# tczhangzhi/pytorch-distributed

Hardware: AMD Instinct MI355X
Metric: ImageNet images/sec (ResNet-50 train step, whole job) (higher is better)
Workload: dtype bf16; 1 GPU; model=resnet50, global_batch=3072, image_size=224, parallelism=dp1, style=ddp, hip_ext=True, hipgraph=False

## Files before the change

### amdtrain/ops/conv.py

```python

from __future__ import annotations

import os

import torch
import torch.nn as nn

from ._ext import ext_available, require_ext


def _rows(x: torch.Tensor) -> torch.Tensor:
    n, c, h, w = x.shape
    return x.permute(0, 2, 3, 1).reshape(n * h * w, c)


def _fuse_stats_enabled() -> bool:
    return os.environ.get("AMDTRAIN_FUSE_BNSTATS", "1") == "1"


def _stem_s2d_enabled() -> bool:
    return os.environ.get("AMDTRAIN_STEM_S2D", "0") == "1"


def _stem_nt64_enabled() -> bool:
    return os.environ.get("AMDTRAIN_STEM_NT64", "1") == "1"


def _s2parity_enabled() -> bool:
    return os.environ.get("AMDTRAIN_CONV3X3_S2PARITY", "1") == "1"


def _nt64_enabled() -> bool:
    return os.environ.get("AMDTRAIN_CONV3X3_NT64", "1") == "1"


def _wgrad2_enabled() -> bool:
    return os.environ.get("AMDTRAIN_WGRAD2", "1") == "1"


class GradCell:
    __slots__ = ("armed", "g", "compact_ok", "meta")

    def __init__(self):
        self.armed = False
        self.g = None
        self.compact_ok = False
        self.meta = None


def _dsgrad_compact_enabled() -> bool:
    return os.environ.get("AMDTRAIN_DSGRAD_COMPACT", "1") == "1"


class ResidualGradTap(torch.autograd.Function):

    @staticmethod
    def forward(ctx, z: torch.Tensor, cell: "GradCell"):
        ctx.cell = cell
        ctx.set_materialize_grads(False)
        return z.view_as(z)

    @staticmethod
    def backward(ctx, grad):
        if grad is None:
            return None, None
        if ctx.cell.armed:
            ctx.cell.g = grad
            ctx.cell.meta = None
            return None, None
        return grad, None


def tap_residual(x: torch.Tensor, cell: "GradCell") -> torch.Tensor:
    out = ResidualGradTap.apply(x, cell)
    out._amdtrain_tap_cell = cell
    return out


class _Conv1x1(torch.autograd.Function):

    @staticmethod
    @torch.amp.custom_fwd(device_type="cuda", cast_inputs=torch.bfloat16)
    def forward(ctx, x: torch.Tensor, weight: torch.Tensor, stride: int,
                cell=None):
        e = require_ext()
        n, cin, h, w = x.shape
        cout = weight.shape[0]
        xc = x.contiguous(memory_format=torch.channels_last)
        x2d = _rows(xc)
        w2d = weight.reshape(cout, cin)
        stats = None
        ctx.cell = cell
        if stride > 1:
            y2d = e.gemm_bt_strided(x2d, w2d, n, h, w, stride)
            ho = (h + stride - 1) // stride
            wo = (w + stride - 1) // stride
        elif _fuse_stats_enabled():
            y2d, stats = e.gemm_bt_stats(x2d, w2d)
            ho, wo = h, w
        else:
            y2d = e.gemm_bt(x2d, w2d, False)
            ho, wo = h, w
        ctx.save_for_backward(x2d, w2d)
        ctx.meta = (n, cin, h, w, stride, ho, wo, cout)
        y = y2d.view(n, ho, wo, cout).permute(0, 3, 1, 2)
        if stats is None:
            stats = torch.empty(0, device=x.device)
        ctx.mark_non_differentiable(stats)
        return y, stats

    @staticmethod
    @torch.amp.custom_bwd(device_type="cuda")
    def backward(ctx, grad_y: torch.Tensor, _grad_stats=None):
        e = require_ext()
        x2d, w2d = ctx.saved_tensors
        n, cin, h, w, stride, ho, wo, cout = ctx.meta
        gy = grad_y.contiguous(memory_format=torch.channels_last)
        gy2d = _rows(gy).to(torch.bfloat16)
        wT = e.transpose_2d(w2d)
        dx2d = e.gemm_bt(gy2d, wT, False)
        if stride > 1:
            cell = ctx.cell
            if (stride == 2 and cell is not None and cell.armed
                    and cell.compact_ok):
                cell.g = dx2d
                cell.meta = (n, h, w, ho, wo)
                dx = None
            else:
                dx = e.scatter_rows_x2(dx2d, n, h, w, ho, wo)
            dw = e.tn2_wgrad(gy2d, x2d, 1, n, h, w, stride, 1) \
                if _wgrad2_enabled() \
                else e.gemm_tn_strided(gy2d, x2d, n, h, w, stride)
        else:
            dx = dx2d.view(n, ho, wo, cin).permute(0, 3, 1, 2)
            dw = e.tn2_wgrad(gy2d, x2d) if _wgrad2_enabled() \
                else e.gemm_tn(gy2d, x2d, 0)
        return dx, dw.reshape(cout, cin, 1, 1), None, None


def conv1x1_mfma(x: torch.Tensor, weight: torch.Tensor,
                 stride: int = 1) -> torch.Tensor:
    cell = getattr(x, "_amdtrain_tap_cell", None) if stride == 2 else None
    y, stats = _Conv1x1.apply(x, weight, stride, cell)
    if stats.numel():
        y._amdtrain_bn_stats = stats
    return y


class _Conv3x3(torch.autograd.Function):

    @staticmethod
    @torch.amp.custom_fwd(device_type="cuda", cast_inputs=torch.bfloat16)
    def forward(ctx, x: torch.Tensor, weight: torch.Tensor, stride: int):
        e = require_ext()
        n, cin, h, w = x.shape
        cout = weight.shape[0]
        xc = x.contiguous(memory_format=torch.channels_last)
        x2d = _rows(xc)
        w2d = weight.contiguous(memory_format=torch.channels_last) \
            .permute(0, 2, 3, 1).reshape(cout, 9 * cin)
        nt64 = _nt64_enabled()
        if _fuse_stats_enabled():
            y2d, stats = e.conv3x3_fwd_stats(x2d, n, h, w, stride, w2d,
                                             False, nt64)
        else:
            y2d = e.conv3x3_fwd(x2d, n, h, w, stride, w2d, nt64)
            stats = torch.empty(0, device=x.device)
        ctx.save_for_backward(x2d, w2d)
        ctx.meta = (n, cin, h, w, stride, cout)
        ho = (h + 2 - 3) // stride + 1
        wo = (w + 2 - 3) // stride + 1
        y = y2d.view(n, ho, wo, cout).permute(0, 3, 1, 2)
        ctx.mark_non_differentiable(stats)
        return y, stats

    @staticmethod
    @torch.amp.custom_bwd(device_type="cuda")
    def backward(ctx, grad_y: torch.Tensor, _grad_stats=None):
        e = require_ext()
        x2d, w2d = ctx.saved_tensors
        n, cin, h, w, stride, cout = ctx.meta
        gy = grad_y.contiguous(memory_format=torch.channels_last)
        gy2d = _rows(gy).to(torch.bfloat16)
        dx2d = e.conv3x3_dgrad(gy2d, n, h, w, stride, w2d, False,
                               _s2parity_enabled(), _nt64_enabled())
        dx = dx2d.view(n, h, w, cin).permute(0, 3, 1, 2)
        dw2d = e.tn2_wgrad(gy2d, x2d, 9, n, h, w, stride, 2) \
            if _wgrad2_enabled() \
            else e.conv3x3_wgrad(gy2d, x2d, n, h, w, stride)
        dw = dw2d.view(cout, 3, 3, cin).permute(0, 3, 1, 2) \
            .contiguous(memory_format=torch.channels_last)
        return dx, dw, None


def conv3x3_mfma(x: torch.Tensor, weight: torch.Tensor,
                 stride: int = 1) -> torch.Tensor:
    y, stats = _Conv3x3.apply(x, weight, stride)
    if stats.numel():
        y._amdtrain_bn_stats = stats
    return y


class _ConvGrouped3x3(torch.autograd.Function):

    @staticmethod
    @torch.amp.custom_fwd(device_type="cuda", cast_inputs=torch.bfloat16)
    def forward(ctx, x: torch.Tensor, weight: torch.Tensor, stride: int,
                groups: int):
        e = require_ext()
        n, cin, h, w = x.shape
        cout = weight.shape[0]
        sg = cin // groups
        xc = x.contiguous(memory_format=torch.channels_last)
        x2d = _rows(xc)
        sout = cout // groups
        wg = weight.contiguous(memory_format=torch.channels_last) \
            .permute(0, 2, 3, 1).reshape(groups, sout, 3, 3, sg)
        dense = torch.zeros(groups, sout, 3, 3, groups, sg,
                            dtype=wg.dtype, device=wg.device)
        gi = torch.arange(groups, device=wg.device)
        dense[gi, :, :, :, gi, :] = wg
        w2d = dense.reshape(cout, 3, 3, cin).reshape(cout, 9 * cin)
        banded = (cin == cout and cin % 128 == 0)
        if _fuse_stats_enabled():
            y2d, stats = e.conv3x3_fwd_stats(x2d, n, h, w, stride, w2d,
                                             banded, _nt64_enabled())
        else:
            y2d = e.conv3x3_fwd(x2d, n, h, w, stride, w2d, _nt64_enabled())
            stats = torch.empty(0, device=x.device)
        ctx.save_for_backward(x2d, w2d)
        ctx.meta = (n, cin, h, w, stride, cout, groups, banded)
        ho = (h + 2 - 3) // stride + 1
        wo = (w + 2 - 3) // stride + 1
        y = y2d.view(n, ho, wo, cout).permute(0, 3, 1, 2)
        ctx.mark_non_differentiable(stats)
        return y, stats

    @staticmethod
    @torch.amp.custom_bwd(device_type="cuda")
    def backward(ctx, grad_y: torch.Tensor, _grad_stats=None):
        e = require_ext()
        x2d, w2d = ctx.saved_tensors
        n, cin, h, w, stride, cout, groups, banded = ctx.meta
        sg = cin // groups
        sout = cout // groups
        gy = grad_y.contiguous(memory_format=torch.channels_last)
        gy2d = _rows(gy).to(torch.bfloat16)
        dx2d = e.conv3x3_dgrad(gy2d, n, h, w, stride, w2d, banded,
                               _s2parity_enabled(), _nt64_enabled())
        dx = dx2d.view(n, h, w, cin).permute(0, 3, 1, 2)
        if banded and _wgrad2_enabled():
            dwb = e.tn2_wgrad_banded(gy2d, x2d, n, h, w, stride) \
                .view(cout // 128, 128 // sg, sg, 9, 128 // sg, sg)
            bi = torch.arange(cout // 128, device=dwb.device)[:, None]
            gi = torch.arange(128 // sg, device=dwb.device)[None, :]
            dw = dwb[bi, gi, :, :, gi, :].reshape(cout, 9, sg) \
                .view(cout, 3, 3, sg).permute(0, 3, 1, 2) \
                .contiguous(memory_format=torch.channels_last)
            return dx, dw, None, None
        dw2d = e.tn2_wgrad(gy2d, x2d, 9, n, h, w, stride, 2) \
            if _wgrad2_enabled() \
            else e.conv3x3_wgrad(gy2d, x2d, n, h, w, stride)
        dwd = dw2d.view(groups, sout, 3, 3, groups, sg)
        gi = torch.arange(groups, device=dwd.device)
        dw = dwd[gi, :, :, :, gi, :].permute(0, 1, 4, 2, 3) \
            .reshape(cout, sg, 3, 3) \
            .contiguous(memory_format=torch.channels_last)
        return dx, dw, None, None


def conv3x3_grouped_mfma(x: torch.Tensor, weight: torch.Tensor,
                         stride: int, groups: int) -> torch.Tensor:
    y, stats = _ConvGrouped3x3.apply(x, weight, stride, groups)
    if stats.numel():
        y._amdtrain_bn_stats = stats
    return y


def stem_s2d_input(x_nhwc: torch.Tensor) -> torch.Tensor:
    n, h, w, c = x_nhwc.shape
    assert c <= 4 and w % 2 == 0
    x4 = torch.nn.functional.pad(x_nhwc, (0, 4 - c))
    return x4.reshape(n, h, w // 2, 8)


def stem_s2d_weight(weight: torch.Tensor) -> torch.Tensor:
    cout, c, kh, kw = weight.shape
    assert c <= 4 and kh == 7 and kw == 7
    wp = torch.nn.functional.pad(weight, (1, 0, 0, 0, 0, 4 - c))
    return wp.permute(0, 2, 3, 1).reshape(cout, 7, 4, 2, 4)


def stem_s2d_dweight(dw2: torch.Tensor, cin: int) -> torch.Tensor:
    cout = dw2.shape[0]
    return dw2.reshape(cout, 7, 8, 4)[:, :, 1:, :cin].permute(0, 3, 1, 2)


def _stem_s2d_ok(weight: torch.Tensor, w: int, stride: int, pad: int) -> bool:
    return (weight.shape[1] <= 4 and tuple(weight.shape[2:]) == (7, 7)
            and stride == 2 and pad == 3 and w % 2 == 0)


class _ConvGeneric(torch.autograd.Function):

    @staticmethod
    @torch.amp.custom_fwd(device_type="cuda", cast_inputs=torch.bfloat16)
    def forward(ctx, x: torch.Tensor, weight: torch.Tensor, stride: int,
                pad: int, s2d: bool = False, nt64: bool = False):
        e = require_ext()
        n, cin, h, w = x.shape
        cout, _, kh, kw = weight.shape
        xc = x.contiguous(memory_format=torch.channels_last)
        x2d = _rows(xc)
        ho = (h + 2 * pad - kh) // stride + 1
        wo = (w + 2 * pad - kw) // stride + 1
        ctx.s2d = s2d
        if s2d:
            x8 = stem_s2d_input(x2d.view(n, h, w, cin)) \
                .view(n * h * (w // 2), 8)
            w2 = stem_s2d_weight(weight).reshape(cout, 224)
            geom = (n, h, w // 2, 7, 4, 2, 3, w2, 1, 2, ho, wo, True)
            if _fuse_stats_enabled():
                y2d, stats = e.conv_generic_fwd_stats(x8, *geom)
            else:
                y2d = e.conv_generic_fwd(x8, *geom)
                stats = torch.empty(0, device=x.device)
            ctx.save_for_backward(x8, weight)
            ctx.meta = (n, cin, h, w, kh, kw, stride, pad, cout, 224, 8)
            ctx.mark_non_differentiable(stats)
            return y2d.view(n, ho, wo, cout).permute(0, 3, 1, 2), stats
        w4 = weight.contiguous(memory_format=torch.channels_last) \
            .permute(0, 2, 3, 1)
        if cin < 8:
            x2d = torch.nn.functional.pad(x2d, (0, 8 - cin))
            w4 = torch.nn.functional.pad(w4, (0, 8 - cin))
            cin_k = 8
        else:
            cin_k = cin
        k = kh * kw * cin_k
        kpad = (k + 31) // 32 * 32
        w2 = w4.reshape(cout, k)
        if kpad != k:
            w2 = torch.nn.functional.pad(w2, (0, kpad - k))
        y2d = e.conv_generic_fwd(x2d, n, h, w, kh, kw, stride, pad, w2,
                                 0, -1, 0, 0, nt64)
        ctx.save_for_backward(x2d, weight)
        ctx.meta = (n, cin, h, w, kh, kw, stride, pad, cout, k, cin_k)
        stats = torch.empty(0, device=x.device)
        ctx.mark_non_differentiable(stats)
        return y2d.view(n, ho, wo, cout).permute(0, 3, 1, 2), stats

    @staticmethod
    @torch.amp.custom_bwd(device_type="cuda")
    def backward(ctx, grad_y: torch.Tensor, _grad_stats=None):
        e = require_ext()
        x2d, weight = ctx.saved_tensors
        n, cin, h, w, kh, kw, stride, pad, cout, k, cin_k = ctx.meta
        gy2d = _rows(grad_y.contiguous(memory_format=torch.channels_last)) \
            .to(torch.bfloat16)
        dx = None
        if ctx.needs_input_grad[0]:
            k2 = kh * kw * cout
            k2p = (k2 + 31) // 32 * 32
            w2p = weight.to(torch.bfloat16).permute(1, 2, 3, 0) \
                .reshape(cin, k2)
            if k2p != k2:
                w2p = torch.nn.functional.pad(w2p, (0, k2p - k2))
            dx2d = e.conv_generic_dgrad(gy2d, w2p.contiguous(), n, h, w,
                                        kh, kw, stride, pad)
            dx = dx2d.view(n, h, w, cin).permute(0, 3, 1, 2)
        if ctx.s2d:
            ho = (h + 2 * pad - kh) // stride + 1
            wo = (w + 2 * pad - kw) // stride + 1
            dwp = e.tn2_wgrad(gy2d, x2d, 28, n, h, w // 2, 2, 2, 7, 4, 3,
                              1, 2, ho, wo)
            dw = stem_s2d_dweight(dwp, cin) \
                .contiguous(memory_format=torch.channels_last)
        elif _wgrad2_enabled() and cout % 8 == 0:
            dwp = e.tn2_wgrad(gy2d, x2d, kh * kw, n, h, w, stride, 2,
                              kh, kw, pad)
            dw = dwp.view(cout, kh * kw, cin_k)[:, :, :cin] \
                .view(cout, kh, kw, cin).permute(0, 3, 1, 2) \
                .contiguous(memory_format=torch.channels_last)
        else:
            dw2 = e.conv_generic_wgrad(gy2d, x2d, n, h, w, kh, kw, stride,
                                       pad)
            dw = dw2[:, :k].view(cout, kh * kw, cin_k)[:, :, :cin] \
                .reshape(cout, kh, kw, cin).permute(0, 3, 1, 2) \
                .contiguous(memory_format=torch.channels_last)
        return dx, dw, None, None, None, None


def conv_stem_mfma(x: torch.Tensor, weight: torch.Tensor, stride: int,
                   pad: int) -> torch.Tensor:
    s2d = (_stem_s2d_enabled() and _wgrad2_enabled()
           and _stem_s2d_ok(weight, x.shape[3], stride, pad))
    y, stats = _ConvGeneric.apply(x, weight, stride, pad, s2d,
                                  _stem_nt64_enabled())
    if stats.numel():
        y._amdtrain_bn_stats = stats
    return y


def _conv1x1_env_default() -> str:
    return os.environ.get("AMDTRAIN_CONV1X1", "custom")


class AmdConv2d(nn.Conv2d):

    def forward(self, x: torch.Tensor) -> torch.Tensor:
        bf16_ok = (x.dtype == torch.bfloat16
                   or torch.is_autocast_enabled("cuda"))
        if (x.is_cuda and bf16_ok and ext_available()
                and self.bias is None and self.dilation == (1, 1)
                and self.groups > 1):
            if (self.kernel_size == (3, 3) and self.padding == (1, 1)
                    and self.stride[0] in (1, 2)
                    and self.in_channels % 32 == 0
                    and self.out_channels % 16 == 0
                    and self.in_channels % self.groups == 0
                    and os.environ.get("AMDTRAIN_CONV3X3G", "custom")
                    == "custom"):
                return conv3x3_grouped_mfma(x, self.weight, self.stride[0],
                                            self.groups)
            return super().forward(x)
        if (x.is_cuda and bf16_ok and ext_available()
                and self.bias is None and self.groups == 1
                and self.dilation == (1, 1)):
            ch_ok = (self.in_channels % 32 == 0
                     and self.out_channels % 16 == 0)
            if (ch_ok and self.kernel_size == (1, 1)
                    and self.padding == (0, 0)
                    and _conv1x1_env_default() == "custom"):
                return conv1x1_mfma(x, self.weight, self.stride[0])
            if (ch_ok and self.kernel_size == (3, 3)
                    and self.padding == (1, 1)
                    and self.stride[0] in (1, 2)
                    and os.environ.get("AMDTRAIN_CONV3X3", "custom")
                    == "custom"):
                return conv3x3_mfma(x, self.weight, self.stride[0])
            if (self.out_channels % 16 == 0
                    and self.stride[0] == self.stride[1]
                    and self.padding[0] == self.padding[1]
                    and os.environ.get("AMDTRAIN_CONVSTEM", "custom")
                    == "custom"):
                return conv_stem_mfma(x, self.weight, self.stride[0],
                                      self.padding[0])
        return super().forward(x)
```

### amdtrain/ops/csrc/common.h

```cpp
#pragma once

#include <torch/extension.h>
#include <ATen/cuda/CUDAContext.h>
#include <hip/hip_runtime.h>
#include <hip/hip_bf16.h>
#include <hip/hip_fp16.h>

#define AMD_WAVE 64
#define AMD_TPB 256
#define AMD_MAX_BLOCKS 2048

#define CHECK_CUDA_OK()                                                     \
  do {                                                                      \
    hipError_t e = hipGetLastError();                                       \
    TORCH_CHECK(e == hipSuccess, "HIP kernel launch failed: ",              \
                hipGetErrorString(e));                                      \
  } while (0)

static inline int amd_grid(long total, int tpb = AMD_TPB,
                           int cap = AMD_MAX_BLOCKS) {
  long g = (total + tpb - 1) / tpb;
  return (int)std::min<long>(g, cap);
}


template <typename scalar_t> struct DevT { using type = scalar_t; };
template <> struct DevT<at::BFloat16> { using type = __hip_bfloat16; };
template <> struct DevT<at::Half> { using type = __half; };

template <typename T> __device__ __forceinline__ float to_f32(T v);
template <> __device__ __forceinline__ float to_f32<float>(float v) { return v; }
template <> __device__ __forceinline__ float to_f32<__hip_bfloat16>(__hip_bfloat16 v) {
  return __bfloat162float(v);
}
template <> __device__ __forceinline__ float to_f32<__half>(__half v) {
  return __half2float(v);
}
template <> __device__ __forceinline__ float to_f32<double>(double v) {
  return (float)v;
}

template <typename T> __device__ __forceinline__ T from_f32(float v);
template <> __device__ __forceinline__ float from_f32<float>(float v) { return v; }
template <> __device__ __forceinline__ __hip_bfloat16 from_f32<__hip_bfloat16>(float v) {
  return __float2bfloat16(v);
}
template <> __device__ __forceinline__ __half from_f32<__half>(float v) {
  return __float2half(v);
}
template <> __device__ __forceinline__ double from_f32<double>(float v) {
  return (double)v;
}

template <typename T, int N> struct alignas(sizeof(T) * N) Pack {
  T v[N];
};
template <typename T> struct VecWidth {
  static constexpr int value = 16 / sizeof(T);
};


__device__ __forceinline__ float wave_reduce_sum(float v) {
#pragma unroll
  for (int off = AMD_WAVE / 2; off > 0; off >>= 1)
    v += __shfl_down(v, off, AMD_WAVE);
  return v;
}

__device__ __forceinline__ float wave_reduce_max(float v) {
#pragma unroll
  for (int off = AMD_WAVE / 2; off > 0; off >>= 1)
    v = fmaxf(v, __shfl_down(v, off, AMD_WAVE));
  return v;
}

template <int NTE = 128>
__device__ __forceinline__ void conv_epilogue_stats(
    float* __restrict__ stats, const float* acc_flat, long m0, long M,
    long n0, long N, int bm, int wm, int wn, int fr, int fq,
    void* lds_scratch) {
  constexpr int NF = NTE / 32;
  float* srow = stats + (long)bm * 2 * N;
  float s1[NF], s2[NF];
#pragma unroll
  for (int j = 0; j < NF; ++j) {
    s1[j] = 0.f;
    s2[j] = 0.f;
#pragma unroll
    for (int i = 0; i < 4; ++i)
#pragma unroll
      for (int r = 0; r < 4; ++r) {
        long row = m0 + wm + i * 16 + fq * 4 + r;
        float v = (row < M) ? acc_flat[(i * NF + j) * 4 + r] : 0.f;
        s1[j] += v;
        s2[j] += v * v;
      }
  }
#pragma unroll
  for (int j = 0; j < NF; ++j) {
#pragma unroll
    for (int off = 32; off >= 16; off >>= 1) {
      s1[j] += __shfl_down(s1[j], off, AMD_WAVE);
      s2[j] += __shfl_down(s2[j], off, AMD_WAVE);
    }
  }
  float* red = (float*)lds_scratch;
  __syncthreads();
  if (fq == 0) {
#pragma unroll
    for (int j = 0; j < NF; ++j) {
      int col = wn + j * 16 + fr;
      red[(wm ? 1 : 0) * (2 * NTE) + col * 2 + 0] = s1[j];
      red[(wm ? 1 : 0) * (2 * NTE) + col * 2 + 1] = s2[j];
    }
  }
  __syncthreads();
  const int t = threadIdx.x;
  for (int col = t; col < NTE; col += AMD_TPB) {
    long n = n0 + col;
    if (n < N) {
      srow[n] = red[col * 2] + red[2 * NTE + col * 2];
      srow[N + n] = red[col * 2 + 1] + red[2 * NTE + col * 2 + 1];
    }
  }
}


constexpr int MT_TENSORS = 24;
constexpr int MT_BLOCKS = 320;
constexpr long MT_CHUNK = 1 << 16;

struct MTMeta {
  const void* a[MT_TENSORS];
  void* b[MT_TENSORS];
  void* c[MT_TENSORS];
  long sizes[MT_TENSORS];
  short t_for_block[MT_BLOCKS];
  short chunk_for_block[MT_BLOCKS];
};

template <typename LaunchFn>
static void mt_apply(const std::vector<at::Tensor>& A,
                     const std::vector<at::Tensor>* B,
                     const std::vector<at::Tensor>* C, LaunchFn launch) {
  MTMeta meta;
  int t = 0, blk = 0;
  for (size_t i = 0; i < A.size(); ++i) {
    long n = A[i].numel();
    meta.a[t] = A[i].const_data_ptr();
    meta.b[t] = B ? (*B)[i].data_ptr() : nullptr;
    meta.c[t] = C ? (*C)[i].data_ptr() : nullptr;
    meta.sizes[t] = n;
    long nchunks = (n + MT_CHUNK - 1) / MT_CHUNK;
    for (long ch = 0; ch < nchunks; ++ch) {
      meta.t_for_block[blk] = (short)t;
      meta.chunk_for_block[blk] = (short)ch;
      ++blk;
      if (blk == MT_BLOCKS) {
        launch(meta, blk, t + 1);
        meta.a[0] = meta.a[t];
        meta.b[0] = meta.b[t];
        meta.c[0] = meta.c[t];
        meta.sizes[0] = meta.sizes[t];
        t = 0;
        blk = 0;
      }
    }
    ++t;
    if (t == MT_TENSORS && i + 1 < A.size()) {
      if (blk) launch(meta, blk, t);
      t = 0;
      blk = 0;
    }
  }
  if (blk) launch(meta, blk, t);
}
```

### amdtrain/ops/csrc/conv3x3.hip

```cpp
#include "common.h"

namespace {

using bf16 = __hip_bfloat16;
using bf16x8 = __attribute__((ext_vector_type(8))) short;
using f32x4 = __attribute__((ext_vector_type(4))) float;

constexpr int GEMM_TPB = 256;
constexpr int BK = 32;

__device__ __forceinline__ int xcd_swz(int bid, int nwg) {
  constexpr int NXCD = 8;
  if (nwg < NXCD) return bid;
  int xcd = bid % NXCD, idx = bid / NXCD;
  int q = nwg / NXCD, r = nwg % NXCD;
  return (xcd < r ? xcd * (q + 1) : r * (q + 1) + (xcd - r) * q) + idx;
}

struct ConvGeom {
  int H, W, Hout, Wout, stride;
};

__device__ __forceinline__ long fwd_gather(long m, int kh, int kw,
                                           const ConvGeom& g) {
  long t = m;
  const int wo = (int)(t % g.Wout); t /= g.Wout;
  const int ho = (int)(t % g.Hout); t /= g.Hout;
  const int h = ho * g.stride - 1 + kh;
  const int w = wo * g.stride - 1 + kw;
  if (h < 0 || h >= g.H || w < 0 || w >= g.W) return -1;
  return (t * g.H + h) * g.W + w;
}

__device__ __forceinline__ long dgrad_gather(long m, int kh, int kw,
                                             const ConvGeom& g) {
  long t = m;
  const int w = (int)(t % g.W); t /= g.W;
  const int h = (int)(t % g.H); t /= g.H;
  const int ho2 = h + 1 - kh, wo2 = w + 1 - kw;
  if (g.stride == 1) {
    if (ho2 < 0 || ho2 >= g.Hout || wo2 < 0 || wo2 >= g.Wout) return -1;
    return (t * g.Hout + ho2) * g.Wout + wo2;
  }
  if ((ho2 & 1) || (wo2 & 1)) return -1;
  const int ho = ho2 >> 1, wo = wo2 >> 1;
  if (ho < 0 || ho >= g.Hout || wo < 0 || wo >= g.Wout) return -1;
  return (t * g.Hout + ho) * g.Wout + wo;
}

struct UnitCoord {
  long n_off;
  int hb, wb;
};

template <bool DGRAD, bool PAR = false>
__device__ __forceinline__ UnitCoord decode_unit(long m, const ConvGeom& g,
                                                 int cls = 0) {
  UnitCoord u;
  long t = m;
  if (PAR) {
    const int W2 = g.W >> 1, H2 = g.H >> 1;
    const int w2 = (int)(t % W2); t /= W2;
    const int h2 = (int)(t % H2); t /= H2;
    u.n_off = t * (long)g.Hout * g.Wout;
    u.hb = 2 * h2 + (cls >> 1) + 1;
    u.wb = 2 * w2 + (cls & 1) + 1;
  } else if (DGRAD) {
    const int w = (int)(t % g.W); t /= g.W;
    const int h = (int)(t % g.H); t /= g.H;
    u.n_off = t * (long)g.Hout * g.Wout;
    u.hb = h + 1;
    u.wb = w + 1;
  } else {
    const int wo = (int)(t % g.Wout); t /= g.Wout;
    const int ho = (int)(t % g.Hout); t /= g.Hout;
    u.n_off = t * (long)g.H * g.W;
    u.hb = ho * g.stride - 1;
    u.wb = wo * g.stride - 1;
  }
  return u;
}

template <bool DGRAD, bool PAR = false>
__device__ __forceinline__ long unit_row(const UnitCoord& u, int kh, int kw,
                                         const ConvGeom& g) {
  if (DGRAD) {
    int ho2 = u.hb - kh, wo2 = u.wb - kw;
    if (PAR) {
      ho2 >>= 1;
      wo2 >>= 1;
    } else if (g.stride == 2) {
      if ((ho2 | wo2) & 1) return -1;
      ho2 >>= 1;
      wo2 >>= 1;
    }
    if (ho2 < 0 || ho2 >= g.Hout || wo2 < 0 || wo2 >= g.Wout) return -1;
    return u.n_off + (long)ho2 * g.Wout + wo2;
  }
  const int h = u.hb + kh, w = u.wb + kw;
  if (h < 0 || h >= g.H || w < 0 || w >= g.W) return -1;
  return u.n_off + (long)h * g.W + w;
}

template <bool DGRAD, int BKT, bool PAR = false>
__device__ __forceinline__ void stage_gathered(
    const bf16* __restrict__ src, int ld, const UnitCoord* uc, int c0, int kh,
    int kw, const ConvGeom& g, const bf16* __restrict__ zero_page,
    bf16* lds) {
  const int t = threadIdx.x;
  constexpr int UPR = BKT / 8;
#pragma unroll
  for (int rnd = 0; rnd < BKT / 16; ++rnd) {
    int unit = rnd * GEMM_TPB + t;
    long row = unit_row<DGRAD, PAR>(uc[rnd], kh, kw, g);
    const bf16* p = row < 0 ? zero_page
                            : src + row * (long)ld + c0 +
                                  (unit % UPR) * 8;
    __builtin_amdgcn_global_load_lds(
        (const __attribute__((address_space(1))) unsigned int*)p,
        (__attribute__((address_space(3))) unsigned int*)(lds + unit * 8), 16,
        0, 0);
  }
}

template <int BKT, int ROWS>
__device__ __forceinline__ void stage_plain_rows(
    const bf16* __restrict__ gsrc, long ld, long row0, long rows, long koff,
    bf16* lds) {
  const int t = threadIdx.x;
  constexpr int UPR = BKT / 8;
  constexpr int UNITS = ROWS * UPR;
#pragma unroll
  for (int rnd = 0; rnd < UNITS / GEMM_TPB; ++rnd) {
    int unit = rnd * GEMM_TPB + t;
    long row = row0 + unit / UPR;
    if (row >= rows) row = rows - 1;
    const bf16* src = gsrc + row * ld + koff + (unit % UPR) * 8;
    __builtin_amdgcn_global_load_lds(
        (const __attribute__((address_space(1))) unsigned int*)src,
        (__attribute__((address_space(3))) unsigned int*)(lds + unit * 8), 16,
        0, 0);
  }
}

template <int BKT>
__device__ __forceinline__ void stage_plain(
    const bf16* __restrict__ gsrc, long ld, long row0, long rows, long koff,
    bf16* lds) {
  const int t = threadIdx.x;
  constexpr int UPR = BKT / 8;
#pragma unroll
  for (int rnd = 0; rnd < BKT / 16; ++rnd) {
    int unit = rnd * GEMM_TPB + t;
    long row = row0 + unit / UPR;
    if (row >= rows) row = rows - 1;
    const bf16* src = gsrc + row * ld + koff + (unit % UPR) * 8;
    __builtin_amdgcn_global_load_lds(
        (const __attribute__((address_space(1))) unsigned int*)src,
        (__attribute__((address_space(3))) unsigned int*)(lds + unit * 8), 16,
        0, 0);
  }
}

template <bool DGRAD, int BKT = BK, bool BAND = false, int NT = 128,
          bool DB = false, bool PAR = false>
__global__ void __launch_bounds__(GEMM_TPB, 2)
conv3x3_kernel(const bf16* __restrict__ A, const bf16* __restrict__ Bw,
               bf16* __restrict__ C, long M, int AC, int NC, ConvGeom g,
               int nbm, int nbn, const bf16* __restrict__ zero_page,
               float* __restrict__ stats) {
  static_assert(!PAR || (DGRAD && !BAND), "PAR is a dense-dgrad variant");
  constexpr int STG = (128 + NT) * BKT;
  __shared__ bf16 SMEM[(DB ? 2 : 1) * STG];
  bf16* const As = SMEM;

  const int bid = xcd_swz(blockIdx.x, nbm * nbn);
  const int bm = bid / nbn, bn = bid % nbn;
  const int cls = PAR ? (bm & 3) : 0;
  const long Mr = PAR ? (M >> 2) : M;
  const long m0 = (long)(PAR ? (bm >> 2) : bm) * 128, n0 = (long)bn * NT;
  constexpr int NFR = NT / 32;

  const int t = threadIdx.x;
  const int wave = t / AMD_WAVE, lane = t % AMD_WAVE;
  const int wm = (wave >> 1) * 64, wn = (wave & 1) * (NT / 2);
  const int fr = lane & 15, fq = lane >> 4;

  f32x4 acc[4][NFR];
#pragma unroll
  for (int i = 0; i < 4; ++i)
#pragma unroll
    for (int j = 0; j < NFR; ++j) acc[i][j] = {0.f, 0.f, 0.f, 0.f};

  UnitCoord uc[BKT / 16];
#pragma unroll
  for (int rnd = 0; rnd < BKT / 16; ++rnd) {
    long m = m0 + (rnd * GEMM_TPB + t) / (BKT / 8);
    if (m >= Mr) m = Mr - 1;
    uc[rnd] = decode_unit<DGRAD, PAR>(m, g, cls);
  }

  const int ks_lo = BAND ? (int)(n0 / BKT) : 0;
  const int ks_hi = BAND ? ks_lo + NT / BKT : AC / BKT;
  const int nks = ks_hi - ks_lo;
  const int par_h = cls >> 1, par_w = cls & 1;
  const int total = (PAR ? (1 + par_h) * (1 + par_w) : 9) * nks;
  auto stage_it = [&](int it, bf16* as) {
    int tap = it / nks;
    const int ks = ks_lo + it % nks;
    if (PAR) {
      const int khi = par_w ? (tap >> 1) : tap, kwi = par_w ? (tap & 1) : 0;
      tap = (par_h ? 2 * khi : 1) * 3 + (par_w ? 2 * kwi : 1);
    }
    const int kh = tap / 3, kw = tap % 3, c0 = ks * BKT;
    stage_gathered<DGRAD, BKT, PAR>(A, AC, uc, c0, kh, kw, g, zero_page,
                                    as);
    if (NT == 128)
      stage_plain<BKT>(Bw, (long)9 * AC, n0, NC, (long)tap * AC + c0,
                       as + 128 * BKT);
    else
      stage_plain_rows<BKT, 64>(Bw, (long)9 * AC, n0, NC,
                                (long)tap * AC + c0, as + 128 * BKT);
  };
  auto compute_it = [&](const bf16* as) {
    const bf16* bs = as + 128 * BKT;
#pragma unroll
    for (int kk = 0; kk < BKT / 32; ++kk) {
      bf16x8 a[4], b[NFR];
#pragma unroll
      for (int i = 0; i < 4; ++i)
        a[i] = *(const bf16x8*)
            &as[(wm + i * 16 + fr) * BKT + kk * 32 + fq * 8];
#pragma unroll
      for (int j = 0; j < NFR; ++j)
        b[j] = *(const bf16x8*)
            &bs[(wn + j * 16 + fr) * BKT + kk * 32 + fq * 8];
#pragma unroll
      for (int i = 0; i < 4; ++i)
#pragma unroll
        for (int j = 0; j < NFR; ++j)
          acc[i][j] = __builtin_amdgcn_mfma_f32_16x16x32_bf16(
              a[i], b[j], acc[i][j], 0, 0, 0);
    }
  };
  if (DB) {
    constexpr int HB = STG;
    if (total > 0) stage_it(0, SMEM);
    for (int it = 0; it < total; ++it) {
      bf16* const as = SMEM + (it & 1) * HB;
      __syncthreads();
      if (it + 1 < total) stage_it(it + 1, SMEM + ((it + 1) & 1) * HB);
      compute_it(as);
    }
  } else {
    for (int it = 0; it < total; ++it) {
      __syncthreads();
      stage_it(it, SMEM);
      __syncthreads();
      compute_it(SMEM);
    }
  }

  if (PAR) {
    const unsigned W2 = g.W >> 1, H2 = g.H >> 1;
#pragma unroll
    for (int i = 0; i < 4; ++i) {
      const unsigned mr = (unsigned)m0 + wm + i * 16 + fq * 4;
      unsigned w2 = mr % W2, t2 = mr / W2;
      unsigned h2 = t2 % H2, n = t2 / H2;
#pragma unroll
      for (int r = 0; r < 4; ++r) {
        if ((long)mr + r < Mr) {
          const long row = ((long)n * g.H + 2 * h2 + par_h) * g.W +
                           2 * w2 + par_w;
#pragma unroll
          for (int j = 0; j < NFR; ++j) {
            long col = n0 + wn + j * 16 + fr;
            if (col < NC)
              C[row * NC + col] = __float2bfloat16(acc[i][j][r]);
          }
        }
        if (++w2 == W2) {
          w2 = 0;
          if (++h2 == H2) {
            h2 = 0;
            ++n;
          }
        }
      }
    }
    return;
  }
#pragma unroll
  for (int i = 0; i < 4; ++i)
#pragma unroll
    for (int j = 0; j < NFR; ++j)
#pragma unroll
      for (int r = 0; r < 4; ++r) {
        long row = m0 + wm + i * 16 + fq * 4 + r;
        long col = n0 + wn + j * 16 + fr;
        if (row < M && col < NC)
          C[row * NC + col] = __float2bfloat16(acc[i][j][r]);
      }
  if (stats != nullptr)
    conv_epilogue_stats<NT>(stats, (const float*)acc, m0, M, n0, NC, bm,
                            wm, wn, fr, fq, As);
}

__device__ __forceinline__ int wg_swz(int cc, int m) {
  return cc * 32 + (m ^ (((((cc >> 3) & 3) ^ ((cc >> 1) & 3))) << 3));
}

__global__ void __launch_bounds__(GEMM_TPB, 2)
conv3x3_wgrad_kernel(const bf16* __restrict__ dY, const bf16* __restrict__ X,
                     float* __restrict__ dW, long M, int Cout, int Cin,
                     ConvGeom g, int tap, int nbn, int nbk, int msplit) {
  __shared__ bf16 Ys[128 * 32];
  __shared__ bf16 Xs[128 * 32];

  const int kh = tap / 3, kw = tap % 3;
  const int tiles = nbn * nbk;
  const int tile = blockIdx.x % tiles;
  const int mpart = blockIdx.x / tiles;
  const int bn = tile / nbk, bk = tile % nbk;
  const long n0 = (long)bn * 128, k0 = (long)bk * 128;

  const long mchunks = (M + 31) / 32;
  const long cpp = (mchunks + msplit - 1) / msplit;
  const long mc0 = (long)mpart * cpp;
  const long mc1 = min(mc0 + cpp, mchunks);

  const int t = threadIdx.x;
  const int wave = t / AMD_WAVE, lane = t % AMD_WAVE;
  const int wn = (wave >> 1) * 64, wk = (wave & 1) * 64;
  const int fr = lane & 15, fq = lane >> 4;

  f32x4 acc[4][4];
#pragma unroll
  for (int i = 0; i < 4; ++i)
#pragma unroll
    for (int j = 0; j < 4; ++j) acc[i][j] = {0.f, 0.f, 0.f, 0.f};

  for (long mc = mc0; mc < mc1; ++mc) {
    const long m0 = mc * 32;
    __syncthreads();
#pragma unroll
    for (int rnd = 0; rnd < 2; ++rnd) {
      const int unit = rnd * GEMM_TPB + t;
      const long m = m0 + (unit >> 4);
      const int c0 = (unit & 15) * 8;
      const int mloc = unit >> 4;
      bf16 yv[8];
      if (m < M && n0 + c0 + 8 <= Cout) {
        uint4 raw = *(const uint4*)(dY + m * Cout + n0 + c0);
        __builtin_memcpy(yv, &raw, 16);
      } else {
#pragma unroll
        for (int j = 0; j < 8; ++j) yv[j] = bf16(0.f);
      }
#pragma unroll
      for (int j = 0; j < 8; ++j) Ys[wg_swz(c0 + j, mloc)] = yv[j];
      long xrow = m < M ? fwd_gather(m, kh, kw, g) : -1;
      bf16 xv[8];
      if (xrow >= 0 && k0 + c0 + 8 <= Cin) {
        uint4 raw = *(const uint4*)(X + xrow * (long)Cin + k0 + c0);
        __builtin_memcpy(xv, &raw, 16);
      } else {
#pragma unroll
        for (int j = 0; j < 8; ++j) xv[j] = bf16(0.f);
      }
#pragma unroll
      for (int j = 0; j < 8; ++j) Xs[wg_swz(c0 + j, mloc)] = xv[j];
    }
    __syncthreads();

    bf16x8 a[4], b[4];
#pragma unroll
    for (int i = 0; i < 4; ++i)
      a[i] = *(const bf16x8*)&Ys[wg_swz(wn + i * 16 + fr, fq * 8)];
#pragma unroll
    for (int j = 0; j < 4; ++j)
      b[j] = *(const bf16x8*)&Xs[wg_swz(wk + j * 16 + fr, fq * 8)];
#pragma unroll
    for (int i = 0; i < 4; ++i)
#pragma unroll
      for (int j = 0; j < 4; ++j)
        acc[i][j] = __builtin_amdgcn_mfma_f32_16x16x32_bf16(
            a[i], b[j], acc[i][j], 0, 0, 0);
  }

#pragma unroll
  for (int i = 0; i < 4; ++i)
#pragma unroll
    for (int j = 0; j < 4; ++j)
#pragma unroll
      for (int r = 0; r < 4; ++r) {
        long n = n0 + wn + i * 16 + fq * 4 + r;
        long k = k0 + wk + j * 16 + fr;
        if (n < Cout && k < Cin)
          atomicAdd(&dW[n * (long)(9 * Cin) + (long)tap * Cin + k],
                    acc[i][j][r]);
      }
}

__global__ void __launch_bounds__(AMD_TPB)
rotate_weight_kernel(const bf16* __restrict__ w, bf16* __restrict__ out,
                     int Cout, int Cin) {
  long total = (long)Cout * 9 * Cin;
  for (long i = (long)blockIdx.x * blockDim.x + threadIdx.x; i < total;
       i += (long)gridDim.x * blockDim.x) {
    long t = i;
    const int cin = (int)(t % Cin); t /= Cin;
    const int tap = (int)(t % 9); t /= 9;
    const int cout = (int)t;
    out[((long)cin * 9 + tap) * Cout + cout] =
        w[((long)cout * 9 + tap) * Cin + cin];
  }
}

}

static bool conv3x3_db_enabled() {
  static const bool v = []() {
    const char* e = std::getenv("AMDTRAIN_CONV3X3_DB");
    return !(e && e[0] == '0');
  }();
  return v;
}

static at::Tensor zero_page_for(const at::Tensor& like) {
  static thread_local at::Tensor zp;
  if (!zp.defined() || zp.device() != like.device())
    zp = at::zeros({16}, like.options().dtype(at::kBFloat16));
  return zp;
}

std::vector<at::Tensor> conv3x3_fwd_stats_impl(at::Tensor x2d, long Nn,
                                                long H, long W, long stride,
                                                at::Tensor w2d,
                                                bool want_stats,
                                                bool banded = false,
                                                bool nt64 = true) {
  TORCH_CHECK(x2d.is_cuda() && x2d.scalar_type() == at::kBFloat16);
  long Cin = x2d.size(1), Cout = w2d.size(0);
  TORCH_CHECK(w2d.size(1) == 9 * Cin);
  TORCH_CHECK(Cin % BK == 0, "Cin must be multiple of 32");
  long Hout = (H + 2 - 3) / stride + 1, Wout = (W + 2 - 3) / stride + 1;
  long M = Nn * Hout * Wout;
  auto y = at::empty({M, Cout}, x2d.options());
  ConvGeom g{(int)H, (int)W, (int)Hout, (int)Wout, (int)stride};
  int nbm = (int)((M + 127) / 128), nbn = (int)((Cout + 127) / 128);
  auto zp = zero_page_for(x2d);
  at::Tensor stats;
  float* stats_ptr = nullptr;
  if (want_stats) {
    stats = at::empty({nbm, 2 * Cout}, x2d.options().dtype(at::kFloat));
    stats_ptr = stats.data_ptr<float>();
  }
  auto stream = at::cuda::getCurrentCUDAStream();
  static const bool bk64 = []() {
    const char* v = std::getenv("AMDTRAIN_CONV3X3_BK64");
    return !(v && v[0] == '0');
  }();
  if (banded) {
    int nbn64 = (int)((Cout + 63) / 64);
    if (conv3x3_db_enabled())
      conv3x3_kernel<false, BK, true, 64, true>
          <<<nbm * nbn64, GEMM_TPB, 0, stream>>>(
              (const bf16*)x2d.const_data_ptr(),
              (const bf16*)w2d.const_data_ptr(), (bf16*)y.data_ptr(), M,
              (int)Cin, (int)Cout, g, nbm, nbn64,
              (const bf16*)zp.const_data_ptr(), stats_ptr);
    else
      conv3x3_kernel<false, BK, true, 64>
          <<<nbm * nbn64, GEMM_TPB, 0, stream>>>(
              (const bf16*)x2d.const_data_ptr(),
              (const bf16*)w2d.const_data_ptr(), (bf16*)y.data_ptr(), M,
              (int)Cin, (int)Cout, g, nbm, nbn64,
              (const bf16*)zp.const_data_ptr(), stats_ptr);
  } else if (nt64 && Cout <= 64 && conv3x3_db_enabled()) {
    conv3x3_kernel<false, BK, false, 64, true>
        <<<nbm, GEMM_TPB, 0, stream>>>(
            (const bf16*)x2d.const_data_ptr(),
            (const bf16*)w2d.const_data_ptr(), (bf16*)y.data_ptr(), M,
            (int)Cin, (int)Cout, g, nbm, 1,
            (const bf16*)zp.const_data_ptr(), stats_ptr);
  } else if (bk64 && Cin % 64 == 0 && Cin >= 128 && M >= 200000) {
    if (conv3x3_db_enabled())
      conv3x3_kernel<false, 64, false, 128, true>
          <<<nbm * nbn, GEMM_TPB, 0, stream>>>(
              (const bf16*)x2d.const_data_ptr(),
              (const bf16*)w2d.const_data_ptr(), (bf16*)y.data_ptr(), M,
              (int)Cin, (int)Cout, g, nbm, nbn,
              (const bf16*)zp.const_data_ptr(), stats_ptr);
    else
      conv3x3_kernel<false, 64><<<nbm * nbn, GEMM_TPB, 0, stream>>>(
          (const bf16*)x2d.const_data_ptr(),
          (const bf16*)w2d.const_data_ptr(), (bf16*)y.data_ptr(), M,
          (int)Cin, (int)Cout, g, nbm, nbn,
          (const bf16*)zp.const_data_ptr(), stats_ptr);
  } else if (conv3x3_db_enabled())
    conv3x3_kernel<false, BK, false, 128, true>
        <<<nbm * nbn, GEMM_TPB, 0, stream>>>(
            (const bf16*)x2d.const_data_ptr(),
            (const bf16*)w2d.const_data_ptr(), (bf16*)y.data_ptr(), M,
            (int)Cin, (int)Cout, g, nbm, nbn,
            (const bf16*)zp.const_data_ptr(), stats_ptr);
  else
    conv3x3_kernel<false><<<nbm * nbn, GEMM_TPB, 0, stream>>>(
        (const bf16*)x2d.const_data_ptr(), (const bf16*)w2d.const_data_ptr(),
        (bf16*)y.data_ptr(), M, (int)Cin, (int)Cout, g, nbm, nbn,
        (const bf16*)zp.const_data_ptr(), stats_ptr);
  CHECK_CUDA_OK();
  if (want_stats) return {y, stats};
  return {y};
}

at::Tensor conv3x3_fwd(at::Tensor x2d, long Nn, long H, long W, long stride,
                       at::Tensor w2d, bool nt64) {
  return conv3x3_fwd_stats_impl(x2d, Nn, H, W, stride, w2d, false, false,
                                nt64)[0];
}

std::vector<at::Tensor> conv3x3_fwd_stats(at::Tensor x2d, long Nn, long H,
                                          long W, long stride,
                                          at::Tensor w2d, bool banded,
                                          bool nt64) {
  TORCH_CHECK(!banded || (x2d.size(1) == w2d.size(0) &&
                          x2d.size(1) % 128 == 0),
              "banded conv3x3 needs Cin == Cout, both % 128");
  return conv3x3_fwd_stats_impl(x2d, Nn, H, W, stride, w2d, true, banded,
                                nt64);
}

at::Tensor conv3x3_dgrad(at::Tensor dy2d, long Nn, long H, long W,
                         long stride, at::Tensor w2d, bool banded,
                         bool s2parity, bool nt64) {
  long Cout = dy2d.size(1), Cin = w2d.size(1) / 9;
  TORCH_CHECK(w2d.size(0) == Cout && w2d.size(1) == 9 * Cin);
  TORCH_CHECK(Cout % BK == 0);
  long Hout = (H + 2 - 3) / stride + 1, Wout = (W + 2 - 3) / stride + 1;
  long M = Nn * H * W;
  auto stream = at::cuda::getCurrentCUDAStream();
  auto wrot = at::empty({Cin, 9 * Cout}, w2d.options());
  rotate_weight_kernel<<<amd_grid(Cout * 9 * Cin), AMD_TPB, 0, stream>>>(
      (const bf16*)w2d.const_data_ptr(), (bf16*)wrot.data_ptr(), (int)Cout,
      (int)Cin);
  CHECK_CUDA_OK();
  auto dx = at::empty({M, Cin}, dy2d.options());
  ConvGeom g{(int)H, (int)W, (int)Hout, (int)Wout, (int)stride};
  int nbm = (int)((M + 127) / 128), nbn = (int)((Cin + 127) / 128);
  auto zp = zero_page_for(dy2d);
  if (banded) {
    TORCH_CHECK(Cin == Cout && Cin % 128 == 0);
    int nbn64 = (int)(Cin / 64);
    if (conv3x3_db_enabled())
      conv3x3_kernel<true, BK, true, 64, true>
          <<<nbm * nbn64, GEMM_TPB, 0, stream>>>(
              (const bf16*)dy2d.const_data_ptr(),
              (const bf16*)wrot.const_data_ptr(), (bf16*)dx.data_ptr(), M,
              (int)Cout, (int)Cin, g, nbm, nbn64,
              (const bf16*)zp.const_data_ptr(), nullptr);
    else
      conv3x3_kernel<true, BK, true, 64>
          <<<nbm * nbn64, GEMM_TPB, 0, stream>>>(
              (const bf16*)dy2d.const_data_ptr(),
              (const bf16*)wrot.const_data_ptr(), (bf16*)dx.data_ptr(), M,
              (int)Cout, (int)Cin, g, nbm, nbn64,
              (const bf16*)zp.const_data_ptr(), nullptr);
    CHECK_CUDA_OK();
    return dx;
  }
  static const bool bk64d = []() {
    const char* v = std::getenv("AMDTRAIN_CONV3X3_BK64D");
    return v && v[0] == '1';
  }();
  const bool par = s2parity && stride == 2 && H % 2 == 0 && W % 2 == 0 &&
                   M < (1L << 31) && conv3x3_db_enabled();
  const bool n64 = nt64 && Cin <= 64 && conv3x3_db_enabled();
  if (par) {
    const int nbmp = 4 * (int)((M / 4 + 127) / 128);
    if (n64)
      conv3x3_kernel<true, BK, false, 64, true, true>
          <<<nbmp, GEMM_TPB, 0, stream>>>(
              (const bf16*)dy2d.const_data_ptr(),
              (const bf16*)wrot.const_data_ptr(), (bf16*)dx.data_ptr(), M,
              (int)Cout, (int)Cin, g, nbmp, 1,
              (const bf16*)zp.const_data_ptr(), nullptr);
    else
      conv3x3_kernel<true, BK, false, 128, true, true>
          <<<nbmp * nbn, GEMM_TPB, 0, stream>>>(
              (const bf16*)dy2d.const_data_ptr(),
              (const bf16*)wrot.const_data_ptr(), (bf16*)dx.data_ptr(), M,
              (int)Cout, (int)Cin, g, nbmp, nbn,
              (const bf16*)zp.const_data_ptr(), nullptr);
  } else if (n64)
    conv3x3_kernel<true, BK, false, 64, true>
        <<<nbm, GEMM_TPB, 0, stream>>>(
            (const bf16*)dy2d.const_data_ptr(),
            (const bf16*)wrot.const_data_ptr(), (bf16*)dx.data_ptr(), M,
            (int)Cout, (int)Cin, g, nbm, 1,
            (const bf16*)zp.const_data_ptr(), nullptr);
  else if (bk64d && Cout % 64 == 0)
    conv3x3_kernel<true, 64><<<nbm * nbn, GEMM_TPB, 0, stream>>>(
        (const bf16*)dy2d.const_data_ptr(),
        (const bf16*)wrot.const_data_ptr(), (bf16*)dx.data_ptr(), M,
        (int)Cout, (int)Cin, g, nbm, nbn,
        (const bf16*)zp.const_data_ptr(), nullptr);
  else if (conv3x3_db_enabled())
    conv3x3_kernel<true, BK, false, 128, true>
        <<<nbm * nbn, GEMM_TPB, 0, stream>>>(
            (const bf16*)dy2d.const_data_ptr(),
            (const bf16*)wrot.const_data_ptr(), (bf16*)dx.data_ptr(), M,
            (int)Cout, (int)Cin, g, nbm, nbn,
            (const bf16*)zp.const_data_ptr(), nullptr);
  else
    conv3x3_kernel<true><<<nbm * nbn, GEMM_TPB, 0, stream>>>(
        (const bf16*)dy2d.const_data_ptr(),
        (const bf16*)wrot.const_data_ptr(), (bf16*)dx.data_ptr(), M,
        (int)Cout, (int)Cin, g, nbm, nbn,
        (const bf16*)zp.const_data_ptr(), nullptr);
  CHECK_CUDA_OK();
  return dx;
}

at::Tensor conv3x3_wgrad(at::Tensor dy2d, at::Tensor x2d, long Nn, long H,
                         long W, long stride) {
  long Cout = dy2d.size(1), Cin = x2d.size(1);
  long Hout = (H + 2 - 3) / stride + 1, Wout = (W + 2 - 3) / stride + 1;
  long M = Nn * Hout * Wout;
  TORCH_CHECK(dy2d.size(0) == M);
  auto dW = at::zeros({Cout, 9 * Cin}, dy2d.options().dtype(at::kFloat));
  ConvGeom g{(int)H, (int)W, (int)Hout, (int)Wout, (int)stride};
  int nbn = (int)((Cout + 127) / 128), nbk = (int)((Cin + 127) / 128);
  long tiles = (long)nbn * nbk;
  const bool det = std::getenv("AMDTRAIN_DETERMINISTIC") != nullptr;
  int msplit = det ? 1
                   : (int)std::max<long>(
                         1, std::min<long>((M + 31) / 32, 512 / tiles));
  auto stream = at::cuda::getCurrentCUDAStream();
  for (int tap = 0; tap < 9; ++tap) {
    conv3x3_wgrad_kernel<<<(int)(tiles * msplit), GEMM_TPB, 0, stream>>>(
        (const bf16*)dy2d.const_data_ptr(), (const bf16*)x2d.const_data_ptr(),
        dW.data_ptr<float>(), M, (int)Cout, (int)Cin, g, tap, nbn, nbk,
        msplit);
    CHECK_CUDA_OK();
  }
  return dW;
}
```

### amdtrain/ops/csrc/conv_stem.hip

```cpp
#include "common.h"

namespace {

using bf16 = __hip_bfloat16;
using bf16x8 = __attribute__((ext_vector_type(8))) short;
using f32x4 = __attribute__((ext_vector_type(4))) float;

constexpr int GEMM_TPB = 256;
constexpr int BK = 32;

__device__ __forceinline__ int xcd_swz(int bid, int nwg) {
  constexpr int NXCD = 8;
  if (nwg < NXCD) return bid;
  int xcd = bid % NXCD, idx = bid / NXCD;
  int q = nwg / NXCD, r = nwg % NXCD;
  return (xcd < r ? xcd * (q + 1) : r * (q + 1) + (xcd - r) * q) + idx;
}

struct StemGeom {
  int H, W, Hout, Wout;
  int KH, KW, Cin;
  int stride, pad;
  int sw, pw;
  int Kpad;
};

struct StemCoord {
  long n_off;
  int hb, wb;
};

template <bool DGRAD = false>
__device__ __forceinline__ StemCoord stem_decode(long m, const StemGeom& g) {
  StemCoord u;
  long t = m;
  if (DGRAD) {
    const int w = (int)(t % g.W); t /= g.W;
    const int h = (int)(t % g.H); t /= g.H;
    u.n_off = t * (long)g.Hout * g.Wout;
    u.hb = h + g.pad;
    u.wb = w + g.pad;
    return u;
  }
  const int wo = (int)(t % g.Wout); t /= g.Wout;
  const int ho = (int)(t % g.Hout); t /= g.Hout;
  u.n_off = t * (long)g.H * g.W;
  u.hb = ho * g.stride - g.pad;
  u.wb = wo * g.sw - g.pw;
  return u;
}

__device__ __forceinline__ void col_decode(int col, const StemGeom& g,
                                           float inv_cin, float inv_kw,
                                           int& kh, int& kw, int& ci) {
  const int tap = (int)((float)col * inv_cin + 1e-4f);
  ci = col - tap * g.Cin;
  kh = (int)((float)tap * inv_kw + 1e-4f);
  kw = tap - kh * g.KW;
}

template <bool DGRAD = false>
__device__ __forceinline__ long stem_elem(const StemCoord& u, int col,
                                          const StemGeom& g, float inv_cin,
                                          float inv_kw) {
  if (col >= g.KH * g.KW * g.Cin) return -1;
  int kh, kw, ci;
  col_decode(col, g, inv_cin, inv_kw, kh, kw, ci);
  if (DGRAD) {
    int ho2 = u.hb - kh, wo2 = u.wb - kw;
    if (g.stride > 1) {
      if (ho2 % g.stride || wo2 % g.stride) return -1;
      ho2 /= g.stride;
      wo2 /= g.stride;
    }
    if (ho2 < 0 || ho2 >= g.Hout || wo2 < 0 || wo2 >= g.Wout) return -1;
    return (u.n_off + (long)ho2 * g.Wout + wo2) * g.Cin + ci;
  }
  const int h = u.hb + kh, w = u.wb + kw;
  if (h < 0 || h >= g.H || w < 0 || w >= g.W) return -1;
  return (u.n_off + (long)h * g.W + w) * g.Cin + ci;
}

template <bool DGRAD = false>
__device__ __forceinline__ void stage_im2col(
    const bf16* __restrict__ x, const StemCoord* uc, const bool* valid,
    int c0, const StemGeom& g, float inv_cin, float inv_kw, bf16* lds) {
  const int t = threadIdx.x;
#pragma unroll
  for (int rnd = 0; rnd < 2; ++rnd) {
    const int unit = rnd * GEMM_TPB + t;
    const int cc0 = c0 + (unit & 3) * 8;
    bf16 v[8];
#pragma unroll
    for (int j = 0; j < 8; ++j) {
      long idx = valid[rnd]
                     ? stem_elem<DGRAD>(uc[rnd], cc0 + j, g, inv_cin, inv_kw)
                     : -1;
      v[j] = idx < 0 ? bf16(0.f) : x[idx];
    }
    *(Pack<bf16, 8>*)(lds + unit * 8) = *(Pack<bf16, 8>*)v;
  }
}

template <int ROWS = 128>
__device__ __forceinline__ void stage_rows(
    const bf16* __restrict__ gsrc, long ld, long row0, long rows, long koff,
    bf16* lds) {
  const int t = threadIdx.x;
#pragma unroll
  for (int rnd = 0; rnd < ROWS / 64; ++rnd) {
    int unit = rnd * GEMM_TPB + t;
    long row = row0 + (unit >> 2);
    if (row >= rows) row = rows - 1;
    const bf16* src = gsrc + row * ld + koff + (unit & 3) * 8;
    __builtin_amdgcn_global_load_lds(
        (const __attribute__((address_space(1))) unsigned int*)src,
        (__attribute__((address_space(3))) unsigned int*)(lds + unit * 8), 16,
        0, 0);
  }
}


__device__ __forceinline__ void stage_im2col8(
    const bf16* __restrict__ x, const StemCoord* uc, const bool* valid,
    int c0, const StemGeom& g, const bf16* __restrict__ zp, bf16* lds) {
  const int t = threadIdx.x;
#pragma unroll
  for (int rnd = 0; rnd < 2; ++rnd) {
    const int unit = rnd * GEMM_TPB + t;
    const int tap = (c0 >> 3) + (unit & 3);
    const bf16* src = zp;
    if (valid[rnd] && tap < g.KH * g.KW) {
      const int kh = tap / g.KW, kw = tap - (tap / g.KW) * g.KW;
      const int h = uc[rnd].hb + kh, w = uc[rnd].wb + kw;
      if (h >= 0 && h < g.H && w >= 0 && w < g.W)
        src = x + (uc[rnd].n_off + (long)h * g.W + w) * 8;
    }
    __builtin_amdgcn_global_load_lds(
        (const __attribute__((address_space(1))) unsigned int*)src,
        (__attribute__((address_space(3))) unsigned int*)(lds + unit * 8), 16,
        0, 0);
  }
}

struct StemRow {
  long base;
  int hb;
  bool wok;
};

__device__ __forceinline__ void stage_row4(
    const bf16* __restrict__ x, const StemRow* ur, int ks, const StemGeom& g,
    const bf16* __restrict__ zp, bf16* lds) {
  const int t = threadIdx.x;
#pragma unroll
  for (int rnd = 0; rnd < 2; ++rnd) {
    const int unit = rnd * GEMM_TPB + t;
    const int h = ur[rnd].hb + ks;
    const bf16* src = zp;
    if (ur[rnd].wok && h >= 0 && h < g.H)
      src = x + (ur[rnd].base + (long)ks * g.W) * 8;
    __builtin_amdgcn_global_load_lds(
        (const __attribute__((address_space(1))) unsigned int*)src,
        (__attribute__((address_space(3))) unsigned int*)(lds + unit * 8), 16,
        0, 0);
  }
}

template <bool DGRAD = false, bool C8 = false, bool DB = false, int NT = 128,
          bool ROW4 = false>
__global__ void __launch_bounds__(GEMM_TPB, 2)
conv_generic_fwd_kernel(const bf16* __restrict__ x,
                        const bf16* __restrict__ W2, bf16* __restrict__ Y,
                        long M, int Cout, StemGeom g, int nbm, int nbn,
                        const bf16* __restrict__ zp,
                        float* __restrict__ stats) {
  static_assert(!ROW4 || (C8 && !DGRAD), "ROW4 is a C8 forward staging");
  constexpr int STG = (128 + NT) * BK;
  constexpr int NFR = NT / 32;
  __shared__ bf16 SMEM[(DB ? 2 : 1) * STG];
  const int bid = xcd_swz(blockIdx.x, nbm * nbn);
  const int bm = bid / nbn, bn = bid % nbn;
  const long m0 = (long)bm * 128, n0 = (long)bn * NT;
  const int t = threadIdx.x;
  const int wave = t / AMD_WAVE, lane = t % AMD_WAVE;
  const int wm = (wave >> 1) * 64, wn = (wave & 1) * (NT / 2);
  const int fr = lane & 15, fq = lane >> 4;

  f32x4 acc[4][NFR];
#pragma unroll
  for (int i = 0; i < 4; ++i)
#pragma unroll
    for (int j = 0; j < NFR; ++j) acc[i][j] = {0.f, 0.f, 0.f, 0.f};

  const float inv_cin = 1.f / g.Cin, inv_kw = 1.f / g.KW;
  StemCoord uc[2];
  bool valid[2];
#pragma unroll
  for (int rnd = 0; rnd < 2; ++rnd) {
    long m = m0 + (((rnd * GEMM_TPB) + t) >> 2);
    valid[rnd] = m < M;
    uc[rnd] = stem_decode<DGRAD>(valid[rnd] ? m : M - 1, g);
  }
  StemRow ur[2];
  if (ROW4) {
#pragma unroll
    for (int rnd = 0; rnd < 2; ++rnd) {
      const int w = uc[rnd].wb + (t & 3);
      ur[rnd].hb = uc[rnd].hb;
      ur[rnd].wok = valid[rnd] && w >= 0 && w < g.W;
      ur[rnd].base = uc[rnd].n_off + (long)uc[rnd].hb * g.W + w;
    }
  }

  const int ksteps = g.Kpad / BK;
  auto stage = [&](int ks, bf16* as) {
    if (ROW4)
      stage_row4(x, ur, ks, g, zp, as);
    else if (C8)
      stage_im2col8(x, uc, valid, ks * BK, g, zp, as);
    else
      stage_im2col<DGRAD>(x, uc, valid, ks * BK, g, inv_cin, inv_kw, as);
    stage_rows<NT>(W2, g.Kpad, n0, Cout, ks * BK, as + 128 * BK);
  };
  auto compute = [&](const bf16* as) {
    const bf16* bs = as + 128 * BK;
    bf16x8 a[4], b[NFR];
#pragma unroll
    for (int i = 0; i < 4; ++i)
      a[i] = *(const bf16x8*)&as[(wm + i * 16 + fr) * BK + fq * 8];
#pragma unroll
    for (int j = 0; j < NFR; ++j)
      b[j] = *(const bf16x8*)&bs[(wn + j * 16 + fr) * BK + fq * 8];
#pragma unroll
    for (int i = 0; i < 4; ++i)
#pragma unroll
      for (int j = 0; j < NFR; ++j)
        acc[i][j] = __builtin_amdgcn_mfma_f32_16x16x32_bf16(
            a[i], b[j], acc[i][j], 0, 0, 0);
  };
  if (DB) {
    constexpr int HB = STG;
    if (ksteps > 0) stage(0, SMEM);
    for (int ks = 0; ks < ksteps; ++ks) {
      bf16* const as = SMEM + (ks & 1) * HB;
      __syncthreads();
      if (ks + 1 < ksteps) stage(ks + 1, SMEM + ((ks + 1) & 1) * HB);
      compute(as);
    }
  } else {
    for (int ks = 0; ks < ksteps; ++ks) {
      __syncthreads();
      stage(ks, SMEM);
      __syncthreads();
      compute(SMEM);
    }
  }
#pragma unroll
  for (int i = 0; i < 4; ++i)
#pragma unroll
    for (int j = 0; j < NFR; ++j)
#pragma unroll
      for (int r = 0; r < 4; ++r) {
        long row = m0 + wm + i * 16 + fq * 4 + r;
        long col = n0 + wn + j * 16 + fr;
        if (row < M && col < Cout)
          Y[row * Cout + col] = __float2bfloat16(acc[i][j][r]);
      }
  if (stats != nullptr)
    conv_epilogue_stats<NT>(stats, (const float*)acc, m0, M, n0, Cout, bm,
                            wm, wn, fr, fq, SMEM);
}

__device__ __forceinline__ int st_swz(int c, int m) {
  return c * 32 + (m ^ (((((c >> 3) & 3) ^ ((c >> 1) & 3))) << 3));
}

__global__ void __launch_bounds__(GEMM_TPB, 2)
conv_generic_wgrad_kernel(const bf16* __restrict__ dY,
                          const bf16* __restrict__ x, float* __restrict__ dW2,
                          long M, int Cout, StemGeom g, int nbn, int nbk,
                          int msplit) {
  __shared__ bf16 Ys[128 * 32];
  __shared__ bf16 Xs[128 * 32];
  const int tiles = nbn * nbk;
  const int tile = blockIdx.x % tiles;
  const int mpart = blockIdx.x / tiles;
  const int bn = tile / nbk, bk = tile % nbk;
  const long n0 = (long)bn * 128, k0 = (long)bk * 128;

  const long mchunks = (M + 31) / 32;
  const long cpp = (mchunks + msplit - 1) / msplit;
  const long mc0 = (long)mpart * cpp;
  const long mc1 = min(mc0 + cpp, mchunks);

  const int t = threadIdx.x;
  const int wave = t / AMD_WAVE, lane = t % AMD_WAVE;
  const int wn = (wave >> 1) * 64, wk = (wave & 1) * 64;
  const int fr = lane & 15, fq = lane >> 4;

  f32x4 acc[4][4];
#pragma unroll
  for (int i = 0; i < 4; ++i)
#pragma unroll
    for (int j = 0; j < 4; ++j) acc[i][j] = {0.f, 0.f, 0.f, 0.f};

  const float inv_cin = 1.f / g.Cin, inv_kw = 1.f / g.KW;
  const int K = g.KH * g.KW * g.Cin;
  int ckh[2][8], ckw[2][8], cci[2][8];
  bool cok[2][8];
#pragma unroll
  for (int rnd = 0; rnd < 2; ++rnd) {
    const int unit = rnd * GEMM_TPB + t;
    const int c0 = (unit & 15) * 8;
#pragma unroll
    for (int j = 0; j < 8; ++j) {
      const int col = (int)(k0 + c0 + j);
      cok[rnd][j] = col < K;
      col_decode(cok[rnd][j] ? col : 0, g, inv_cin, inv_kw, ckh[rnd][j],
                 ckw[rnd][j], cci[rnd][j]);
    }
  }

  for (long mc = mc0; mc < mc1; ++mc) {
    const long m0 = mc * 32;
    __syncthreads();
#pragma unroll
    for (int rnd = 0; rnd < 2; ++rnd) {
      const int unit = rnd * GEMM_TPB + t;
      const long m = m0 + (unit >> 4);
      const int c0 = (unit & 15) * 8;
      const int mloc = unit >> 4;
      bf16 yv[8];
      if (m < M && n0 + c0 + 8 <= Cout) {
        uint4 raw = *(const uint4*)(dY + m * Cout + n0 + c0);
        __builtin_memcpy(yv, &raw, 16);
      } else {
#pragma unroll
        for (int j = 0; j < 8; ++j) yv[j] = bf16(0.f);
      }
#pragma unroll
      for (int j = 0; j < 8; ++j) Ys[st_swz(c0 + j, mloc)] = yv[j];
      bf16 xv[8];
      StemCoord u = stem_decode(m < M ? m : 0, g);
#pragma unroll
      for (int j = 0; j < 8; ++j) {
        const int h = u.hb + ckh[rnd][j], w = u.wb + ckw[rnd][j];
        const bool ok = (m < M) && cok[rnd][j] && h >= 0 && h < g.H &&
                        w >= 0 && w < g.W;
        long idx = (u.n_off + (long)h * g.W + w) * g.Cin + cci[rnd][j];
        xv[j] = ok ? x[idx] : bf16(0.f);
      }
#pragma unroll
      for (int j = 0; j < 8; ++j) Xs[st_swz(c0 + j, mloc)] = xv[j];
    }
    __syncthreads();

    bf16x8 a[4], b[4];
#pragma unroll
    for (int i = 0; i < 4; ++i)
      a[i] = *(const bf16x8*)&Ys[st_swz(wn + i * 16 + fr, fq * 8)];
#pragma unroll
    for (int j = 0; j < 4; ++j)
      b[j] = *(const bf16x8*)&Xs[st_swz(wk + j * 16 + fr, fq * 8)];
#pragma unroll
    for (int i = 0; i < 4; ++i)
#pragma unroll
      for (int j = 0; j < 4; ++j)
        acc[i][j] = __builtin_amdgcn_mfma_f32_16x16x32_bf16(
            a[i], b[j], acc[i][j], 0, 0, 0);
  }
#pragma unroll
  for (int i = 0; i < 4; ++i)
#pragma unroll
    for (int j = 0; j < 4; ++j)
#pragma unroll
      for (int r = 0; r < 4; ++r) {
        long n = n0 + wn + i * 16 + fq * 4 + r;
        long k = k0 + wk + j * 16 + fr;
        if (n < Cout && k < g.Kpad)
          atomicAdd(&dW2[n * (long)g.Kpad + k], acc[i][j][r]);
      }
}

static StemGeom make_geom(long H, long W, long KH, long KW, long Cin,
                          long stride, long pad, long stride_w = 0,
                          long pad_w = -1, long Hout = 0, long Wout = 0) {
  StemGeom g;
  g.H = (int)H; g.W = (int)W;
  g.sw = (int)(stride_w > 0 ? stride_w : stride);
  g.pw = (int)(pad_w >= 0 ? pad_w : pad);
  g.Hout = (int)(Hout > 0 ? Hout : (H + 2 * pad - KH) / stride + 1);
  g.Wout = (int)(Wout > 0 ? Wout : (W + 2 * g.pw - KW) / g.sw + 1);
  g.KH = (int)KH; g.KW = (int)KW; g.Cin = (int)Cin;
  g.stride = (int)stride; g.pad = (int)pad;
  int K = (int)(KH * KW * Cin);
  g.Kpad = (K + 31) / 32 * 32;
  return g;
}

template <bool DGRAD, bool C8, bool DBUF, int NT = 128, bool ROW4 = false>
static void stem_launch(int grid, hipStream_t stream, const bf16* x,
                        const bf16* w2, bf16* y, long M, int Cout,
                        const StemGeom& g, int nbm, int nbn, const bf16* zp,
                        float* stats) {
  conv_generic_fwd_kernel<DGRAD, C8, DBUF, NT, ROW4>
      <<<grid, GEMM_TPB, 0, stream>>>(x, w2, y, M, Cout, g, nbm, nbn, zp,
                                      stats);
}

static at::Tensor stem_zero_page(const at::Tensor& like) {
  static thread_local at::Tensor zp;
  if (!zp.defined() || zp.device() != like.device())
    zp = at::zeros({16}, like.options().dtype(at::kBFloat16));
  return zp;
}

}


static bool stem_db_enabled() {
  static const bool v = []() {
    const char* e = std::getenv("AMDTRAIN_STEM_DB");
    return !(e && e[0] == '0');
  }();
  return v;
}

static std::vector<at::Tensor> conv_generic_fwd_impl(
    at::Tensor x2d, long Nn, long H, long W, long KH, long KW, long stride,
    long pad, at::Tensor w2, long stride_w, long pad_w, long Hout, long Wout,
    bool want_stats, bool tile64) {
  TORCH_CHECK(x2d.is_cuda() && x2d.scalar_type() == at::kBFloat16);
  TORCH_CHECK(x2d.is_contiguous() && w2.is_contiguous());
  long Cin = x2d.size(1), Cout = w2.size(0);
  TORCH_CHECK(x2d.size(0) == Nn * H * W);
  auto g = make_geom(H, W, KH, KW, Cin, stride, pad, stride_w, pad_w, Hout,
                     Wout);
  TORCH_CHECK(w2.size(1) == g.Kpad, "weight must be K-padded to ", g.Kpad);
  long M = Nn * g.Hout * g.Wout;
  auto y = at::empty({M, Cout}, x2d.options());
  int nbm = (int)((M + 127) / 128), nbn = (int)((Cout + 127) / 128);
  auto stream = at::cuda::getCurrentCUDAStream();
  auto zp = stem_zero_page(x2d);
  const bool db = stem_db_enabled();
  const bool c8 = Cin == 8 && g.Kpad == (KH * KW * 8 + 31) / 32 * 32;
  const bool row4 = c8 && KW == 4 && g.Kpad == KH * 32;
  const bool t64 = tile64 && Cout <= 64;
  TORCH_CHECK(!want_stats || c8, "conv_generic stats need the C8 kernel");
  at::Tensor stats;
  float* sp = nullptr;
  if (want_stats) {
    stats = at::empty({nbm, 2 * Cout}, x2d.options().dtype(at::kFloat));
    sp = stats.data_ptr<float>();
  }
  const bf16* xp = (const bf16*)x2d.const_data_ptr();
  const bf16* wp = (const bf16*)w2.const_data_ptr();
  const bf16* zpp = (const bf16*)zp.const_data_ptr();
  bf16* yp = (bf16*)y.data_ptr();
  const int grid = nbm * nbn, co = (int)Cout;
  if (c8 && row4 && t64 && db)
    stem_launch<false, true, true, 64, true>(grid, stream, xp, wp, yp, M, co,
                                             g, nbm, nbn, zpp, sp);
  else if (c8 && row4 && t64)
    stem_launch<false, true, false, 64, true>(grid, stream, xp, wp, yp, M, co,
                                              g, nbm, nbn, zpp, sp);
  else if (c8 && t64 && db)
    stem_launch<false, true, true, 64>(grid, stream, xp, wp, yp, M, co, g,
                                       nbm, nbn, zpp, sp);
  else if (c8 && t64)
    stem_launch<false, true, false, 64>(grid, stream, xp, wp, yp, M, co, g,
                                        nbm, nbn, zpp, sp);
  else if (c8 && db)
    stem_launch<false, true, true>(grid, stream, xp, wp, yp, M, co, g, nbm,
                                   nbn, zpp, sp);
  else if (c8)
    stem_launch<false, true, false>(grid, stream, xp, wp, yp, M, co, g, nbm,
                                    nbn, zpp, sp);
  else if (db)
    stem_launch<false, false, true>(grid, stream, xp, wp, yp, M, co, g, nbm,
                                    nbn, zpp, sp);
  else
    stem_launch<false, false, false>(grid, stream, xp, wp, yp, M, co, g, nbm,
                                     nbn, zpp, sp);
  CHECK_CUDA_OK();
  if (want_stats) return {y, stats};
  return {y};
}

at::Tensor conv_generic_fwd(at::Tensor x2d, long Nn, long H, long W,
                            long KH, long KW, long stride, long pad,
                            at::Tensor w2, long stride_w, long pad_w,
                            long Hout, long Wout, bool tile64) {
  return conv_generic_fwd_impl(x2d, Nn, H, W, KH, KW, stride, pad, w2,
                               stride_w, pad_w, Hout, Wout, false, tile64)[0];
}

std::vector<at::Tensor> conv_generic_fwd_stats(
    at::Tensor x2d, long Nn, long H, long W, long KH, long KW, long stride,
    long pad, at::Tensor w2, long stride_w, long pad_w, long Hout, long Wout,
    bool tile64) {
  return conv_generic_fwd_impl(x2d, Nn, H, W, KH, KW, stride, pad, w2,
                               stride_w, pad_w, Hout, Wout, true, tile64);
}

at::Tensor conv_generic_dgrad(at::Tensor dy2d, at::Tensor w2p, long Nn,
                              long H, long W, long KH, long KW, long stride,
                              long pad) {
  TORCH_CHECK(dy2d.is_cuda() && dy2d.scalar_type() == at::kBFloat16);
  long Cout = dy2d.size(1), Cin = w2p.size(0);
  auto g = make_geom(H, W, KH, KW, Cout, stride, pad);
  TORCH_CHECK(w2p.size(1) == g.Kpad, "w2p must be K-padded to ", g.Kpad);
  TORCH_CHECK(dy2d.size(0) == Nn * g.Hout * g.Wout);
  long M = Nn * H * W;
  auto dx = at::empty({M, Cin}, dy2d.options());
  int nbm = (int)((M + 127) / 128), nbn = (int)((Cin + 127) / 128);
  auto stream = at::cuda::getCurrentCUDAStream();
  auto zp = stem_zero_page(dy2d);
  if (stem_db_enabled())
    conv_generic_fwd_kernel<true, false, true>
        <<<nbm * nbn, GEMM_TPB, 0, stream>>>(
            (const bf16*)dy2d.const_data_ptr(),
            (const bf16*)w2p.const_data_ptr(), (bf16*)dx.data_ptr(), M,
            (int)Cin, g, nbm, nbn, (const bf16*)zp.const_data_ptr(),
            nullptr);
  else
    conv_generic_fwd_kernel<true><<<nbm * nbn, GEMM_TPB, 0, stream>>>(
        (const bf16*)dy2d.const_data_ptr(),
        (const bf16*)w2p.const_data_ptr(), (bf16*)dx.data_ptr(), M,
        (int)Cin, g, nbm, nbn, (const bf16*)zp.const_data_ptr(), nullptr);
  CHECK_CUDA_OK();
  return dx;
}

at::Tensor conv_generic_wgrad(at::Tensor dy2d, at::Tensor x2d, long Nn,
                              long H, long W, long KH, long KW, long stride,
                              long pad) {
  long Cin = x2d.size(1), Cout = dy2d.size(1);
  auto g = make_geom(H, W, KH, KW, Cin, stride, pad);
  long M = Nn * g.Hout * g.Wout;
  TORCH_CHECK(dy2d.size(0) == M);
  auto dW2 = at::zeros({Cout, g.Kpad}, dy2d.options().dtype(at::kFloat));
  int nbn = (int)((Cout + 127) / 128), nbk = (int)((g.Kpad + 127) / 128);
  long tiles = (long)nbn * nbk;
  const bool det = std::getenv("AMDTRAIN_DETERMINISTIC") != nullptr;
  int msplit = det ? 1
                   : (int)std::max<long>(
                         1, std::min<long>((M + 31) / 32, 512 / tiles));
  auto stream = at::cuda::getCurrentCUDAStream();
  conv_generic_wgrad_kernel<<<(int)(tiles * msplit), GEMM_TPB, 0, stream>>>(
      (const bf16*)dy2d.const_data_ptr(), (const bf16*)x2d.const_data_ptr(),
      dW2.data_ptr<float>(), M, (int)Cout, g, nbn, nbk, msplit);
  CHECK_CUDA_OK();
  return dW2;
}
```

### amdtrain/ops/csrc/ext.cpp

```cpp
#include <torch/extension.h>

#include <optional>
#include <vector>

void multi_tensor_sgd(std::vector<at::Tensor> params,
                      std::vector<at::Tensor> grads,
                      std::vector<at::Tensor> momenta, double lr,
                      double momentum, double weight_decay, bool nesterov,
                      bool first, bool zero_grad);

std::vector<at::Tensor> cross_entropy_fwd(at::Tensor logits, at::Tensor target);
at::Tensor cross_entropy_bwd(at::Tensor logits, at::Tensor target,
                             at::Tensor lse, at::Tensor upstream);

at::Tensor normalize_u8(at::Tensor x, std::vector<double> mean,
                        std::vector<double> std_, long dtype_code);
at::Tensor topk_ranks(at::Tensor logits, at::Tensor target);
at::Tensor scatter_rows_x2(at::Tensor src2d, long Nn, long H, long W,
                           long Hs, long Ws);
void multi_tensor_scale_check(std::vector<at::Tensor> tensors, double scale,
                              at::Tensor found_inf);
void multi_tensor_cast(std::vector<at::Tensor> src,
                       std::vector<at::Tensor> dst);

std::vector<at::Tensor> batch_norm_fwd_train(
    at::Tensor x, at::Tensor weight, at::Tensor bias, at::Tensor running_mean,
    at::Tensor running_var, double momentum, double eps, bool relu,
    std::optional<at::Tensor> addend);
std::vector<at::Tensor> batch_norm_fwd_train_from_parts(
    at::Tensor x, at::Tensor parts, at::Tensor weight, at::Tensor bias,
    at::Tensor running_mean, at::Tensor running_var, double momentum,
    double eps, bool relu, std::optional<at::Tensor> addend);
at::Tensor batch_norm_fwd_eval(at::Tensor x, at::Tensor weight,
                               at::Tensor bias, at::Tensor running_mean,
                               at::Tensor running_var, double eps, bool relu,
                               std::optional<at::Tensor> addend);
std::vector<at::Tensor> batch_norm_train_stats(
    at::Tensor x, std::optional<at::Tensor> parts, at::Tensor weight,
    at::Tensor bias, at::Tensor running_mean, at::Tensor running_var,
    double momentum, double eps);
std::vector<at::Tensor> batch_norm_dual_fwd_train(
    at::Tensor x3, at::Tensor x_d, std::optional<at::Tensor> parts3,
    std::optional<at::Tensor> parts_d, at::Tensor weight3, at::Tensor bias3,
    at::Tensor running_mean3, at::Tensor running_var3, double momentum3,
    double eps3, at::Tensor weight_d, at::Tensor bias_d,
    at::Tensor running_mean_d, at::Tensor running_var_d, double momentum_d,
    double eps_d);
std::vector<at::Tensor> batch_norm_dual_bwd(
    at::Tensor x3, at::Tensor x_d, at::Tensor grad_out,
    std::optional<at::Tensor> grad_out2, at::Tensor relu_mask,
    at::Tensor weight3, at::Tensor mean3, at::Tensor invstd3,
    at::Tensor weight_d, at::Tensor mean_d, at::Tensor invstd_d);
std::vector<at::Tensor> batch_norm_bwd(at::Tensor x, at::Tensor grad_out,
                                       std::optional<at::Tensor> y,
                                       at::Tensor weight,
                                       at::Tensor mean, at::Tensor invstd,
                                       bool relu, bool need_ghat,
                                       std::optional<at::Tensor> scale,
                                       std::optional<at::Tensor> shift,
                                       std::optional<at::Tensor> grad_out2,
                                       std::optional<at::Tensor> relu_mask,
                                       bool grad_out2_compact);
std::vector<at::Tensor> batch_norm_bwd_pool(
    at::Tensor x, at::Tensor grad_pool, std::optional<at::Tensor> grad_pool2,
    at::Tensor idx, at::Tensor weight, at::Tensor mean, at::Tensor invstd,
    at::Tensor scale, at::Tensor shift);

at::Tensor gemm_bt(at::Tensor A, at::Tensor B, bool f32_out,
                   std::optional<at::Tensor> addend,
                   std::optional<at::Tensor> bias);
at::Tensor gemm_tn(at::Tensor dY, at::Tensor X, long msplit);
at::Tensor gemm_bt_strided(at::Tensor A, at::Tensor B, long Nn, long H,
                           long W, long stride);
at::Tensor gemm_tn_strided(at::Tensor dY, at::Tensor X, long Nn, long H,
                           long W, long stride);
at::Tensor transpose_2d(at::Tensor x);

at::Tensor conv3x3_fwd(at::Tensor x2d, long Nn, long H, long W, long stride,
                       at::Tensor w2d, bool nt64);
std::vector<at::Tensor> conv3x3_fwd_stats(at::Tensor x2d, long Nn, long H,
                                          long W, long stride,
                                          at::Tensor w2d, bool banded,
                                          bool nt64);
std::vector<at::Tensor> gemm_bt_stats(at::Tensor A, at::Tensor B);

at::Tensor gemm_bt_8p(at::Tensor A, at::Tensor B);
at::Tensor gemm_bt_8p3(at::Tensor A, at::Tensor B);
at::Tensor conv3x3_8p(at::Tensor A2d, long Nn, long H, long W, long stride,
                      at::Tensor w2d, bool dgrad);
at::Tensor conv3x3_dgrad(at::Tensor dy2d, long Nn, long H, long W,
                         long stride, at::Tensor w2d, bool banded,
                         bool s2parity, bool nt64);
at::Tensor conv3x3_wgrad(at::Tensor dy2d, at::Tensor x2d, long Nn, long H,
                         long W, long stride);

at::Tensor tn2_wgrad(at::Tensor dY, at::Tensor X, long taps, long Nn, long H,
                     long W, long stride, long gmode, long kh, long kw,
                     long pad, long stride_w, long pad_w, long Hout,
                     long Wout);
at::Tensor tn2_wgrad_banded(at::Tensor dY, at::Tensor X, long Nn, long H,
                            long W, long stride);
at::Tensor tr16_probe(at::Tensor in);

at::Tensor conv_generic_fwd(at::Tensor x2d, long Nn, long H, long W, long KH,
                            long KW, long stride, long pad, at::Tensor w2,
                            long stride_w, long pad_w, long Hout, long Wout,
                            bool tile64);
std::vector<at::Tensor> conv_generic_fwd_stats(
    at::Tensor x2d, long Nn, long H, long W, long KH, long KW, long stride,
    long pad, at::Tensor w2, long stride_w, long pad_w, long Hout, long Wout,
    bool tile64);
at::Tensor conv_generic_wgrad(at::Tensor dy2d, at::Tensor x2d, long Nn,
                              long H, long W, long KH, long KW, long stride,
                              long pad);
at::Tensor conv_generic_dgrad(at::Tensor dy2d, at::Tensor w2p, long Nn,
                              long H, long W, long KH, long KW, long stride,
                              long pad);

std::vector<at::Tensor> max_pool_3x3_s2_fwd(at::Tensor x,
                                            std::optional<at::Tensor> scale,
                                            std::optional<at::Tensor> shift);
at::Tensor max_pool_3x3_s2_bwd(at::Tensor grad_y, at::Tensor idx, long H,
                               long W);
at::Tensor global_avg_pool_fwd(at::Tensor x);
at::Tensor global_avg_pool_bwd(at::Tensor grad_y, long H, long W);

PYBIND11_MODULE(TORCH_EXTENSION_NAME, m) {
  m.doc() = "amdtrain hand-written gfx950 (CDNA4) HIP kernels";
  m.def("multi_tensor_sgd", &multi_tensor_sgd, "fused multi-tensor SGD");
  m.def("cross_entropy_fwd", &cross_entropy_fwd);
  m.def("cross_entropy_bwd", &cross_entropy_bwd);
  m.def("normalize_u8", &normalize_u8);
  m.def("topk_ranks", &topk_ranks);
  m.def("scatter_rows_x2", &scatter_rows_x2);
  m.def("multi_tensor_scale_check", &multi_tensor_scale_check);
  m.def("multi_tensor_cast", &multi_tensor_cast);
  m.def("batch_norm_fwd_train", &batch_norm_fwd_train,
        py::arg("x"), py::arg("weight"), py::arg("bias"),
        py::arg("running_mean"), py::arg("running_var"), py::arg("momentum"),
        py::arg("eps"), py::arg("relu"),
        py::arg("addend") = std::nullopt);
  m.def("batch_norm_fwd_train_from_parts", &batch_norm_fwd_train_from_parts,
        py::arg("x"), py::arg("parts"), py::arg("weight"), py::arg("bias"),
        py::arg("running_mean"), py::arg("running_var"), py::arg("momentum"),
        py::arg("eps"), py::arg("relu"), py::arg("addend") = std::nullopt);
  m.def("batch_norm_fwd_eval", &batch_norm_fwd_eval,
        py::arg("x"), py::arg("weight"), py::arg("bias"),
        py::arg("running_mean"), py::arg("running_var"), py::arg("eps"),
        py::arg("relu"), py::arg("addend") = std::nullopt);
  m.def("batch_norm_train_stats", &batch_norm_train_stats);
  m.def("batch_norm_dual_fwd_train", &batch_norm_dual_fwd_train);
  m.def("batch_norm_dual_bwd", &batch_norm_dual_bwd);
  m.def("batch_norm_bwd", &batch_norm_bwd, py::arg("x"), py::arg("grad_out"),
        py::arg("y"), py::arg("weight"), py::arg("mean"), py::arg("invstd"),
        py::arg("relu"), py::arg("need_ghat"),
        py::arg("scale") = std::nullopt, py::arg("shift") = std::nullopt,
        py::arg("grad_out2") = std::nullopt,
        py::arg("relu_mask") = std::nullopt,
        py::arg("grad_out2_compact") = false);
  m.def("batch_norm_bwd_pool", &batch_norm_bwd_pool, py::arg("x"),
        py::arg("grad_pool"), py::arg("grad_pool2"), py::arg("idx"),
        py::arg("weight"), py::arg("mean"), py::arg("invstd"),
        py::arg("scale"), py::arg("shift"));
  m.def("gemm_bt", &gemm_bt, py::arg("A"), py::arg("B"),
        py::arg("f32_out") = false, py::arg("addend") = std::nullopt,
        py::arg("bias") = std::nullopt);
  m.def("gemm_tn", &gemm_tn, py::arg("dY"), py::arg("X"),
        py::arg("msplit") = 0);
  m.def("gemm_bt_strided", &gemm_bt_strided);
  m.def("gemm_tn_strided", &gemm_tn_strided);
  m.def("transpose_2d", &transpose_2d);
  m.def("conv3x3_fwd", &conv3x3_fwd, py::arg("x2d"), py::arg("Nn"),
        py::arg("H"), py::arg("W"), py::arg("stride"), py::arg("w2d"),
        py::arg("nt64") = true);
  m.def("conv3x3_fwd_stats", &conv3x3_fwd_stats, py::arg("x2d"),
        py::arg("Nn"), py::arg("H"), py::arg("W"), py::arg("stride"),
        py::arg("w2d"), py::arg("banded") = false, py::arg("nt64") = true);
  m.def("gemm_bt_stats", &gemm_bt_stats);
  m.def("gemm_bt_8p", &gemm_bt_8p);
  m.def("gemm_bt_8p3", &gemm_bt_8p3);
  m.def("conv3x3_8p", &conv3x3_8p);
  m.def("conv3x3_dgrad", &conv3x3_dgrad, py::arg("dy2d"), py::arg("Nn"),
        py::arg("H"), py::arg("W"), py::arg("stride"), py::arg("w2d"),
        py::arg("banded") = false, py::arg("s2parity") = true,
        py::arg("nt64") = true);
  m.def("conv3x3_wgrad", &conv3x3_wgrad);
  m.def("tn2_wgrad", &tn2_wgrad, py::arg("dY"), py::arg("X"),
        py::arg("taps") = 1, py::arg("Nn") = 0, py::arg("H") = 0,
        py::arg("W") = 0, py::arg("stride") = 1, py::arg("gmode") = 0,
        py::arg("kh") = 3, py::arg("kw") = 3, py::arg("pad") = 1,
        py::arg("stride_w") = 0, py::arg("pad_w") = -1, py::arg("Hout") = 0,
        py::arg("Wout") = 0);
  m.def("tn2_wgrad_banded", &tn2_wgrad_banded);
  m.def("tr16_probe", &tr16_probe);
  m.def("conv_generic_fwd", &conv_generic_fwd, py::arg("x2d"),
        py::arg("Nn"), py::arg("H"), py::arg("W"), py::arg("KH"),
        py::arg("KW"), py::arg("stride"), py::arg("pad"), py::arg("w2"),
        py::arg("stride_w") = 0, py::arg("pad_w") = -1, py::arg("Hout") = 0,
        py::arg("Wout") = 0, py::arg("tile64") = false);
  m.def("conv_generic_fwd_stats", &conv_generic_fwd_stats, py::arg("x2d"),
        py::arg("Nn"), py::arg("H"), py::arg("W"), py::arg("KH"),
        py::arg("KW"), py::arg("stride"), py::arg("pad"), py::arg("w2"),
        py::arg("stride_w") = 0, py::arg("pad_w") = -1, py::arg("Hout") = 0,
        py::arg("Wout") = 0, py::arg("tile64") = false);
  m.def("conv_generic_wgrad", &conv_generic_wgrad);
  m.def("conv_generic_dgrad", &conv_generic_dgrad);
  m.def("max_pool_3x3_s2_fwd", &max_pool_3x3_s2_fwd, py::arg("x"),
        py::arg("scale") = std::nullopt, py::arg("shift") = std::nullopt);
  m.def("max_pool_3x3_s2_bwd", &max_pool_3x3_s2_bwd);
  m.def("global_avg_pool_fwd", &global_avg_pool_fwd);
  m.def("global_avg_pool_bwd", &global_avg_pool_bwd);
}
```

### amdtrain/ops/csrc/gemm.hip

```cpp
#include "common.h"

namespace {

using bf16 = __hip_bfloat16;
using bf16x8 = __attribute__((ext_vector_type(8))) short;
using f32x4 = __attribute__((ext_vector_type(4))) float;

constexpr int BM = 128, BN = 128, BK = 32;
constexpr int GEMM_TPB = 256;

__device__ __forceinline__ short bf16_bits(bf16 v) {
  short s;
  __builtin_memcpy(&s, &v, 2);
  return s;
}

__device__ __forceinline__ int xcd_swizzle(int bid, int nwg) {
  constexpr int NXCD = 8;
  if (nwg < NXCD) return bid;
  int xcd = bid % NXCD, idx = bid / NXCD;
  int q = nwg / NXCD, r = nwg % NXCD;
  return (xcd < r ? xcd * (q + 1) : r * (q + 1) + (xcd - r) * q) + idx;
}

__device__ __forceinline__ void stage_tile_128x32(
    const bf16* __restrict__ g, long ld, long row0, long rows, long k0,
    bf16* lds) {
  const int t = threadIdx.x;
#pragma unroll
  for (int rnd = 0; rnd < 2; ++rnd) {
    int unit = rnd * GEMM_TPB + t;
    long row = row0 + (unit >> 2);
    if (row >= rows) row = rows - 1;
    int koff = (unit & 3) * 8;
    const bf16* src = g + row * ld + k0 + koff;
    __builtin_amdgcn_global_load_lds(
        (const __attribute__((address_space(1))) unsigned int*)src,
        (__attribute__((address_space(3))) unsigned int*)(lds + unit * 8), 16,
        0, 0);
  }
}

__device__ __forceinline__ void stage_tile_rows(
    const bf16* __restrict__ g, long ld, const long* arow, long k0,
    bf16* lds) {
  const int t = threadIdx.x;
#pragma unroll
  for (int rnd = 0; rnd < 2; ++rnd) {
    int unit = rnd * GEMM_TPB + t;
    int koff = (unit & 3) * 8;
    const bf16* src = g + arow[rnd] * ld + k0 + koff;
    __builtin_amdgcn_global_load_lds(
        (const __attribute__((address_space(1))) unsigned int*)src,
        (__attribute__((address_space(3))) unsigned int*)(lds + unit * 8), 16,
        0, 0);
  }
}

constexpr long GEMM_DB_KMAX = 1024;
inline bool gemm_adir_enabled() {
  static const bool v = []() {
    const char* e = std::getenv("AMDTRAIN_GEMM_ADIR");
    return e && e[0] == '1';
  }();
  return v;
}
inline bool gemm_db_enabled(long K) {
  static const int v = []() {
    const char* e = std::getenv("AMDTRAIN_GEMM_DB");
    return e ? (e[0] == '1' ? 1 : 0) : -1;
  }();
  if (v >= 0) return v == 1;
  return K <= GEMM_DB_KMAX;
}

struct StrideMap {
  int H, W, Hout, Wout, stride;
};

__device__ __forceinline__ long stride_row(long m, const StrideMap& sm) {
  long t = m;
  const int wo = (int)(t % sm.Wout); t /= sm.Wout;
  const int ho = (int)(t % sm.Hout); t /= sm.Hout;
  return (t * sm.H + (long)ho * sm.stride) * sm.W + (long)wo * sm.stride;
}


template <int NFRAG>
__device__ __forceinline__ void epilogue_stats(
    float* __restrict__ stats, const float* acc_flat, long m0, long M,
    long n0, long N, int bm, int wm, int wn, int fr, int fq, int nbm,
    bf16* lds_scratch) {
  float* srow = stats + (long)bm * 2 * N;
  float s1[NFRAG], s2[NFRAG];
#pragma unroll
  for (int j = 0; j < NFRAG; ++j) {
    s1[j] = 0.f;
    s2[j] = 0.f;
#pragma unroll
    for (int i = 0; i < 4; ++i)
#pragma unroll
      for (int r = 0; r < 4; ++r) {
        long row = m0 + wm + i * 16 + fq * 4 + r;
        float v = (row < M) ? acc_flat[(i * NFRAG + j) * 4 + r] : 0.f;
        s1[j] += v;
        s2[j] += v * v;
      }
  }
#pragma unroll
  for (int j = 0; j < NFRAG; ++j) {
#pragma unroll
    for (int off = 32; off >= 16; off >>= 1) {
      s1[j] += __shfl_down(s1[j], off, AMD_WAVE);
      s2[j] += __shfl_down(s2[j], off, AMD_WAVE);
    }
  }
  float* red = (float*)lds_scratch;
  __syncthreads();
  if (fq == 0) {
#pragma unroll
    for (int j = 0; j < NFRAG; ++j) {
      int col = wn + j * 16 + fr;
      red[(wm ? 1 : 0) * 256 + col * 2 + 0] = s1[j];
      red[(wm ? 1 : 0) * 256 + col * 2 + 1] = s2[j];
    }
  }
  __syncthreads();
  const int t = threadIdx.x;
  for (int col = t; col < 128; col += GEMM_TPB) {
    long n = n0 + col;
    if (n < N) {
      srow[n] = red[col * 2] + red[256 + col * 2];
      srow[N + n] = red[col * 2 + 1] + red[256 + col * 2 + 1];
    }
  }
}

template <bool F32OUT, bool STRIDED, bool NT = false, bool LDSE = false,
          bool DB = false, bool ADIR = false>
__global__ void __launch_bounds__(GEMM_TPB, 2)
gemm_bt_kernel(const bf16* __restrict__ A, const bf16* __restrict__ B,
               void* __restrict__ C, long M, long N, long K, int nbm,
               int nbn, StrideMap sm, float* __restrict__ stats) {
  __shared__ bf16 SMEM[(DB ? 2 : 1) *
                       ((ADIR ? 0 : BM) + BN) * BK];
  bf16* const As = SMEM;
  bf16* const Bs = SMEM + (ADIR ? 0 : BM * BK);

  const int nwg = nbm * nbn;
  const int bid = xcd_swizzle(blockIdx.x, nwg);
  const int bm = bid / nbn, bn = bid % nbn;
  const long m0 = (long)bm * BM, n0 = (long)bn * BN;

  const int t = threadIdx.x;
  const int wave = t / AMD_WAVE;
  const int lane = t % AMD_WAVE;
  const int wm = (wave >> 1) * 64;
  const int wn = (wave & 1) * 64;
  const int fr = lane & 15;
  const int fq = lane >> 4;

  f32x4 acc[4][4];
#pragma unroll
  for (int i = 0; i < 4; ++i)
#pragma unroll
    for (int j = 0; j < 4; ++j) acc[i][j] = {0.f, 0.f, 0.f, 0.f};

  long arow[2];
  if (STRIDED) {
#pragma unroll
    for (int rnd = 0; rnd < 2; ++rnd) {
      long m = m0 + (((rnd * GEMM_TPB) + t) >> 2);
      if (m >= M) m = M - 1;
      arow[rnd] = stride_row(m, sm);
    }
  }

  const bf16* Ap[4];
  if (ADIR) {
#pragma unroll
    for (int i = 0; i < 4; ++i) {
      long row = m0 + wm + i * 16 + fr;
      if (row >= M) row = M - 1;
      Ap[i] = A + row * K + fq * 8;
    }
  }
  const long ksteps = K / BK;
  auto stage = [&](long kt, bf16* as) {
    if (!ADIR) {
      if (STRIDED)
        stage_tile_rows(A, K, arow, kt * BK, as);
      else
        stage_tile_128x32(A, K, m0, M, kt * BK, as);
    }
    stage_tile_128x32(B, K, n0, N, kt * BK,
                      as + (ADIR ? 0 : BM * BK));
  };
  auto compute = [&](const bf16* as, long kt) {
    const bf16* bs = as + (ADIR ? 0 : BM * BK);
    bf16x8 a[4], b[4];
#pragma unroll
    for (int i = 0; i < 4; ++i)
      a[i] = ADIR ? *(const bf16x8*)(Ap[i] + kt * BK)
                  : *(const bf16x8*)&as[(wm + i * 16 + fr) * BK + fq * 8];
#pragma unroll
    for (int j = 0; j < 4; ++j)
      b[j] = *(const bf16x8*)&bs[(wn + j * 16 + fr) * BK + fq * 8];
#pragma unroll
    for (int i = 0; i < 4; ++i)
#pragma unroll
      for (int j = 0; j < 4; ++j)
        acc[i][j] = __builtin_amdgcn_mfma_f32_16x16x32_bf16(
            a[i], b[j], acc[i][j], 0, 0, 0);
  };
  if (DB) {
    constexpr int HB = ((ADIR ? 0 : BM) + BN) * BK;
    if (ksteps > 0) stage(0, SMEM);
    for (long kt = 0; kt < ksteps; ++kt) {
      bf16* const as = SMEM + (kt & 1) * HB;
      __syncthreads();
      if (kt + 1 < ksteps) stage(kt + 1, SMEM + ((kt + 1) & 1) * HB);
      compute(as, kt);
    }
  } else {
    for (long kt = 0; kt < ksteps; ++kt) {
      __syncthreads();
      stage(kt, SMEM);
      __syncthreads();
      compute(SMEM, kt);
    }
  }

  if (LDSE && !F32OUT && n0 + 128 <= N) {
#pragma unroll
    for (int h = 0; h < 2; ++h) {
      __syncthreads();
      if (wm == h * 64) {
#pragma unroll
        for (int i = 0; i < 4; ++i)
#pragma unroll
          for (int j = 0; j < 4; ++j)
#pragma unroll
            for (int r = 0; r < 4; ++r)
              SMEM[(i * 16 + fq * 4 + r) * 128 + wn + j * 16 + fr] =
                  __float2bfloat16(acc[i][j][r]);
      }
      __syncthreads();
      for (int u2 = t; u2 < 1024; u2 += GEMM_TPB) {
        const int row_l = u2 >> 3;
        const long row = m0 + h * 64 + row_l;
        if (row < M)
          *(uint4*)((bf16*)C + row * N + n0 + (u2 & 7) * 16) =
              ((const uint4*)SMEM)[u2];
      }
    }
  } else {
#pragma unroll
    for (int i = 0; i < 4; ++i) {
#pragma unroll
      for (int j = 0; j < 4; ++j) {
#pragma unroll
        for (int r = 0; r < 4; ++r) {
          long row = m0 + wm + i * 16 + fq * 4 + r;
          long col = n0 + wn + j * 16 + fr;
          if (row < M && col < N) {
            if (F32OUT) {
              ((float*)C)[row * N + col] = acc[i][j][r];
            } else if (NT) {
              bf16 v = __float2bfloat16(acc[i][j][r]);
              short b;
              __builtin_memcpy(&b, &v, 2);
              __builtin_nontemporal_store(b, (short*)C + row * N + col);
            } else {
              ((bf16*)C)[row * N + col] = __float2bfloat16(acc[i][j][r]);
            }
          }
        }
      }
    }
  }
  if (stats != nullptr)
    epilogue_stats<4>(stats, (const float*)acc, m0, M, n0, N, bm, wm, wn,
                      fr, fq, nbm, As);
}

template <bool DB = false>
__global__ void __launch_bounds__(GEMM_TPB, 2)
gemm_bt_n2_kernel(const bf16* __restrict__ A, const bf16* __restrict__ B,
                  bf16* __restrict__ C, long M, long N, long K, int nbm,
                  int nbn2, float* __restrict__ stats, int nbm_stats) {
  __shared__ bf16 SMEM[(DB ? 2 : 1) * (BM + 256) * BK];
  bf16* const As = SMEM;
  bf16* const Bs = SMEM + BM * BK;

  const int bid = xcd_swizzle(blockIdx.x, nbm * nbn2);
  const int bm = bid / nbn2, bn = bid % nbn2;
  const long m0 = (long)bm * BM, n0 = (long)bn * 256;

  const int t = threadIdx.x;
  const int wave = t / AMD_WAVE;
  const int lane = t % AMD_WAVE;
  const int wm = (wave >> 1) * 64;
  const int wn = (wave & 1) * 64;
  const int fr = lane & 15;
  const int fq = lane >> 4;

  f32x4 acc[4][8];
#pragma unroll
  for (int i = 0; i < 4; ++i)
#pragma unroll
    for (int j = 0; j < 8; ++j) acc[i][j] = {0.f, 0.f, 0.f, 0.f};

  const long ksteps = K / BK;
  auto stage = [&](long kt, bf16* as) {
    bf16* bs = as + BM * BK;
    stage_tile_128x32(A, K, m0, M, kt * BK, as);
    stage_tile_128x32(B, K, n0, N, kt * BK, bs);
    stage_tile_128x32(B, K, n0 + 128, N, kt * BK, bs + 128 * BK);
  };
  auto compute = [&](const bf16* as) {
    const bf16* bs = as + BM * BK;
    bf16x8 a[4], b[8];
#pragma unroll
    for (int i = 0; i < 4; ++i)
      a[i] = *(const bf16x8*)&as[(wm + i * 16 + fr) * BK + fq * 8];
#pragma unroll
    for (int j = 0; j < 8; ++j) {
      const int jn = (j < 4) ? wn + j * 16 : 128 + wn + (j - 4) * 16;
      b[j] = *(const bf16x8*)&bs[(jn + fr) * BK + fq * 8];
    }
#pragma unroll
    for (int i = 0; i < 4; ++i)
#pragma unroll
      for (int j = 0; j < 8; ++j)
        acc[i][j] = __builtin_amdgcn_mfma_f32_16x16x32_bf16(
            a[i], b[j], acc[i][j], 0, 0, 0);
  };
  if (DB) {
    constexpr int HB = (BM + 256) * BK;
    if (ksteps > 0) stage(0, SMEM);
    for (long kt = 0; kt < ksteps; ++kt) {
      bf16* const as = SMEM + (kt & 1) * HB;
      __syncthreads();
      if (kt + 1 < ksteps) stage(kt + 1, SMEM + ((kt + 1) & 1) * HB);
      compute(as);
    }
  } else {
    for (long kt = 0; kt < ksteps; ++kt) {
      __syncthreads();
      stage(kt, SMEM);
      __syncthreads();
      compute(SMEM);
    }
  }

#pragma unroll
  for (int i = 0; i < 4; ++i)
#pragma unroll
    for (int j = 0; j < 8; ++j)
#pragma unroll
      for (int r = 0; r < 4; ++r) {
        long row = m0 + wm + i * 16 + fq * 4 + r;
        long col = n0 + ((j < 4) ? wn + j * 16 : 128 + wn + (j - 4) * 16)
                   + fr;
        if (row < M && col < N)
          C[row * N + col] = __float2bfloat16(acc[i][j][r]);
      }
  if (stats != nullptr) {
    float accl[4][4][4], acch[4][4][4];
#pragma unroll
    for (int i = 0; i < 4; ++i)
#pragma unroll
      for (int j = 0; j < 4; ++j)
#pragma unroll
        for (int r = 0; r < 4; ++r) {
          accl[i][j][r] = acc[i][j][r];
          acch[i][j][r] = acc[i][j + 4][r];
        }
    epilogue_stats<4>(stats, (const float*)accl, m0, M, n0, N, bm, wm, wn,
                      fr, fq, nbm_stats, As);
    __syncthreads();
    epilogue_stats<4>(stats, (const float*)acch, m0, M, n0 + 128, N, bm,
                      wm, wn, fr, fq, nbm_stats, As);
  }
}

__global__ void __launch_bounds__(GEMM_TPB, 2)
gemm_bt_ks_kernel(const bf16* __restrict__ A, const bf16* __restrict__ B,
                  float* __restrict__ parts, long M, long N, long K, int nbm,
                  int nbn, int ksplit) {
  __shared__ bf16 As[BM * BK];
  __shared__ bf16 Bs[BN * BK];

  const int tiles = nbm * nbn;
  const int bid = xcd_swizzle(blockIdx.x, tiles * ksplit);
  const int tile = bid % tiles;
  const int kp = bid / tiles;
  const int bm = tile / nbn, bn = tile % nbn;
  const long m0 = (long)bm * BM, n0 = (long)bn * BN;

  const long ksteps = K / BK;
  const long kper = (ksteps + ksplit - 1) / ksplit;
  const long kt0 = kp * kper;
  const long kt1 = min(kt0 + kper, ksteps);

  const int t = threadIdx.x;
  const int wave = t / AMD_WAVE;
  const int lane = t % AMD_WAVE;
  const int wm = (wave >> 1) * 64;
  const int wn = (wave & 1) * 64;
  const int fr = lane & 15;
  const int fq = lane >> 4;

  f32x4 acc[4][4];
#pragma unroll
  for (int i = 0; i < 4; ++i)
#pragma unroll
    for (int j = 0; j < 4; ++j) acc[i][j] = {0.f, 0.f, 0.f, 0.f};

  for (long kt = kt0; kt < kt1; ++kt) {
    __syncthreads();
    stage_tile_128x32(A, K, m0, M, kt * BK, As);
    stage_tile_128x32(B, K, n0, N, kt * BK, Bs);
    __syncthreads();
    bf16x8 a[4], b[4];
#pragma unroll
    for (int i = 0; i < 4; ++i)
      a[i] = *(const bf16x8*)&As[(wm + i * 16 + fr) * BK + fq * 8];
#pragma unroll
    for (int j = 0; j < 4; ++j)
      b[j] = *(const bf16x8*)&Bs[(wn + j * 16 + fr) * BK + fq * 8];
#pragma unroll
    for (int i = 0; i < 4; ++i)
#pragma unroll
      for (int j = 0; j < 4; ++j)
        acc[i][j] = __builtin_amdgcn_mfma_f32_16x16x32_bf16(
            a[i], b[j], acc[i][j], 0, 0, 0);
  }

  float* out = parts + (long)kp * M * N;
#pragma unroll
  for (int i = 0; i < 4; ++i)
#pragma unroll
    for (int j = 0; j < 4; ++j)
#pragma unroll
      for (int r = 0; r < 4; ++r) {
        long row = m0 + wm + i * 16 + fq * 4 + r;
        long col = n0 + wn + j * 16 + fr;
        if (row < M && col < N) out[row * N + col] = acc[i][j][r];
      }
}

__global__ void __launch_bounds__(AMD_TPB)
gemm_ks_collapse_kernel(const float* __restrict__ parts,
                        bf16* __restrict__ out, int ksplit, long MN, long N,
                        const float* __restrict__ bias,
                        const bf16* __restrict__ gadd) {
  for (long i = (long)blockIdx.x * blockDim.x + threadIdx.x; i < MN;
       i += (long)gridDim.x * blockDim.x) {
    float v = parts[i];
    for (int p = 1; p < ksplit; ++p) v += parts[(long)p * MN + i];
    if (bias != nullptr) v += bias[i % N];
    if (gadd != nullptr) v += __bfloat162float(gadd[i]);
    out[i] = __float2bfloat16(v);
  }
}

__device__ __forceinline__ int tn_swz(int c, int m) {
  return c * 32 + (m ^ (((((c >> 3) & 3) ^ ((c >> 1) & 3))) << 3));
}

__device__ __forceinline__ void tn_stage(const bf16* __restrict__ g, long ld,
                                         long m0, long M, long col0,
                                         bf16* lds) {
  const int t = threadIdx.x;
#pragma unroll
  for (int rnd = 0; rnd < 2; ++rnd) {
    const int unit = rnd * GEMM_TPB + t;
    const long m = m0 + (unit >> 4);
    const int c0 = (unit & 15) * 8;
    bf16 vals[8];
    if (m < M && col0 + c0 + 8 <= ld) {
      uint4 raw = *(const uint4*)(g + m * ld + col0 + c0);
      __builtin_memcpy(vals, &raw, 16);
    } else if (m < M && col0 + c0 < ld) {
#pragma unroll
      for (int j = 0; j < 8; ++j)
        vals[j] = (col0 + c0 + j < ld) ? g[m * ld + col0 + c0 + j]
                                       : bf16(0.f);
    } else {
#pragma unroll
      for (int j = 0; j < 8; ++j) vals[j] = bf16(0.f);
    }
    const int mloc = unit >> 4;
#pragma unroll
    for (int j = 0; j < 8; ++j) lds[tn_swz(c0 + j, mloc)] = vals[j];
  }
}

__device__ __forceinline__ void tn_stage_strided(
    const bf16* __restrict__ g, long ld, long m0, long M, long col0,
    const StrideMap& sm, bf16* lds) {
  const int t = threadIdx.x;
#pragma unroll
  for (int rnd = 0; rnd < 2; ++rnd) {
    const int unit = rnd * GEMM_TPB + t;
    const long m = m0 + (unit >> 4);
    const int c0 = (unit & 15) * 8;
    bf16 vals[8];
    if (m < M && col0 + c0 + 8 <= ld) {
      const long row = stride_row(m, sm);
      uint4 raw = *(const uint4*)(g + row * ld + col0 + c0);
      __builtin_memcpy(vals, &raw, 16);
    } else {
#pragma unroll
      for (int j = 0; j < 8; ++j) vals[j] = bf16(0.f);
    }
    const int mloc = unit >> 4;
#pragma unroll
    for (int j = 0; j < 8; ++j) lds[tn_swz(c0 + j, mloc)] = vals[j];
  }
}

template <bool STRIDED>
__global__ void __launch_bounds__(GEMM_TPB, 2)
gemm_tn_kernel(const bf16* __restrict__ dY, const bf16* __restrict__ X,
               float* __restrict__ dW, long M, long N, long K, int nbn,
               int nbk, int msplit, StrideMap sm) {
  __shared__ bf16 Ys[128 * 32];
  __shared__ bf16 Xs[128 * 32];

  const int tiles = nbn * nbk;
  const int tile = blockIdx.x % tiles;
  const int mpart = blockIdx.x / tiles;
  const int bn = tile / nbk, bk = tile % nbk;
  const long n0 = (long)bn * BM, k0 = (long)bk * BN;

  const long mchunks = (M + 31) / 32;
  const long chunks_per_part = (mchunks + msplit - 1) / msplit;
  const long mc0 = (long)mpart * chunks_per_part;
  const long mc1 = min(mc0 + chunks_per_part, mchunks);

  const int t = threadIdx.x;
  const int wave = t / AMD_WAVE;
  const int lane = t % AMD_WAVE;
  const int wn = (wave >> 1) * 64;
  const int wk = (wave & 1) * 64;
  const int fr = lane & 15;
  const int fq = lane >> 4;

  f32x4 acc[4][4];
#pragma unroll
  for (int i = 0; i < 4; ++i)
#pragma unroll
    for (int j = 0; j < 4; ++j) acc[i][j] = {0.f, 0.f, 0.f, 0.f};

  for (long mc = mc0; mc < mc1; ++mc) {
    const long m0 = mc * 32;
    __syncthreads();
    tn_stage(dY, N, m0, M, n0, Ys);
    if (STRIDED)
      tn_stage_strided(X, K, m0, M, k0, sm, Xs);
    else
      tn_stage(X, K, m0, M, k0, Xs);
    __syncthreads();

    bf16x8 a[4], b[4];
#pragma unroll
    for (int i = 0; i < 4; ++i)
      a[i] = *(const bf16x8*)&Ys[tn_swz(wn + i * 16 + fr, fq * 8)];
#pragma unroll
    for (int j = 0; j < 4; ++j)
      b[j] = *(const bf16x8*)&Xs[tn_swz(wk + j * 16 + fr, fq * 8)];
#pragma unroll
    for (int i = 0; i < 4; ++i)
#pragma unroll
      for (int j = 0; j < 4; ++j)
        acc[i][j] = __builtin_amdgcn_mfma_f32_16x16x32_bf16(
            a[i], b[j], acc[i][j], 0, 0, 0);
  }

#pragma unroll
  for (int i = 0; i < 4; ++i)
#pragma unroll
    for (int j = 0; j < 4; ++j)
#pragma unroll
      for (int r = 0; r < 4; ++r) {
        long n = n0 + wn + i * 16 + fq * 4 + r;
        long k = k0 + wk + j * 16 + fr;
        if (n < N && k < K) atomicAdd(&dW[n * K + k], acc[i][j][r]);
      }
}

__global__ void __launch_bounds__(AMD_TPB)
transpose_2d_kernel(const bf16* __restrict__ in, bf16* __restrict__ out,
                    int R, int Ccols) {
  __shared__ bf16 tile[32][33];
  const int bx = blockIdx.x % ((Ccols + 31) / 32);
  const int by = blockIdx.x / ((Ccols + 31) / 32);
  const int c0 = bx * 32, r0 = by * 32;
  const int tx = threadIdx.x % 32, ty = threadIdx.x / 32;
  for (int dy = 0; dy < 32; dy += 8) {
    int r = r0 + ty + dy, c = c0 + tx;
    if (r < R && c < Ccols) tile[ty + dy][tx] = in[(long)r * Ccols + c];
  }
  __syncthreads();
  for (int dy = 0; dy < 32; dy += 8) {
    int c = c0 + ty + dy, r = r0 + tx;
    if (r < R && c < Ccols) out[(long)c * R + r] = tile[tx][ty + dy];
  }
}

}

at::Tensor gemm_bt(at::Tensor A, at::Tensor B, bool f32_out,
                   std::optional<at::Tensor> addend,
                   std::optional<at::Tensor> bias) {
  TORCH_CHECK(A.is_cuda() && A.dim() == 2 && B.dim() == 2);
  TORCH_CHECK(A.scalar_type() == at::kBFloat16 &&
              B.scalar_type() == at::kBFloat16,
              "gemm_bt expects bf16 inputs");
  auto Ac = A.contiguous();
  auto Bc = B.contiguous();
  long M = Ac.size(0), K = Ac.size(1), N = Bc.size(0);
  TORCH_CHECK(Bc.size(1) == K, "K mismatch");
  TORCH_CHECK(K % BK == 0, "K must be a multiple of ", BK);
  auto C = at::empty({M, N},
                     Ac.options().dtype(f32_out ? at::kFloat : at::kBFloat16));
  int nbm = (int)((M + BM - 1) / BM), nbn = (int)((N + BN - 1) / BN);
  auto stream = at::cuda::getCurrentCUDAStream();
  StrideMap sm{0, 0, 0, 0, 1};
  const bf16* gadd = nullptr;
  at::Tensor ac, bc2;
  if (addend) {
    ac = addend->contiguous();
    TORCH_CHECK(ac.scalar_type() == at::kBFloat16 &&
                ac.numel() == M * N, "addend must be bf16 [M,N]");
    gadd = (const bf16*)ac.const_data_ptr();
  }
  const float* biasp = nullptr;
  if (bias) {
    bc2 = bias->to(at::kFloat).contiguous();
    TORCH_CHECK(bc2.numel() == N, "bias must be [N]");
    biasp = (const float*)bc2.const_data_ptr();
  }
  const long tiles = (long)nbm * nbn;
  const long ksteps = K / BK;
  if (!f32_out && !addend && !bias && N % 256 == 0 && K <= 256 &&
      (long)nbm * (nbn / 2) >= 256) {
    int nbn2 = nbn / 2;
    if (gemm_db_enabled(K))
      gemm_bt_n2_kernel<true><<<nbm * nbn2, GEMM_TPB, 0, stream>>>(
          (const bf16*)Ac.const_data_ptr(),
          (const bf16*)Bc.const_data_ptr(), (bf16*)C.data_ptr(), M, N, K,
          nbm, nbn2, nullptr, nbm);
    else
      gemm_bt_n2_kernel<<<nbm * nbn2, GEMM_TPB, 0, stream>>>(
          (const bf16*)Ac.const_data_ptr(),
          (const bf16*)Bc.const_data_ptr(), (bf16*)C.data_ptr(), M, N, K,
          nbm, nbn2, nullptr, nbm);
    CHECK_CUDA_OK();
    return C;
  }
  if (!f32_out && tiles <= 128 && ksteps >= 2 && 512 / tiles >= 2) {
    const int ksplit = (int)std::min<long>(ksteps, 512 / tiles);
    auto parts = at::empty({ksplit, M * N},
                           Ac.options().dtype(at::kFloat));
    gemm_bt_ks_kernel<<<(int)(tiles * ksplit), GEMM_TPB, 0, stream>>>(
        (const bf16*)Ac.const_data_ptr(), (const bf16*)Bc.const_data_ptr(),
        parts.data_ptr<float>(), M, N, K, nbm, nbn, ksplit);
    CHECK_CUDA_OK();
    gemm_ks_collapse_kernel<<<amd_grid(M * N), AMD_TPB, 0, stream>>>(
        (const float*)parts.const_data_ptr(), (bf16*)C.data_ptr(), ksplit,
        M * N, N, biasp, gadd);
    CHECK_CUDA_OK();
    return C;
  }
  static const bool use_nt = []() {
    const char* v = std::getenv("AMDTRAIN_GEMM_NT");
    return v && v[0] == '1';
  }();
  const bool use_db = gemm_db_enabled(K);
  static const bool use_ldse = []() {
    const char* v = std::getenv("AMDTRAIN_GEMM_LDSE");
    return v && v[0] == '1';
  }();
  if (f32_out)
    gemm_bt_kernel<true, false><<<nbm * nbn, GEMM_TPB, 0, stream>>>(
        (const bf16*)Ac.const_data_ptr(), (const bf16*)Bc.const_data_ptr(),
        C.data_ptr(), M, N, K, nbm, nbn, sm, nullptr);
  else if (use_ldse && N % 8 == 0)
    gemm_bt_kernel<false, false, false, true>
        <<<nbm * nbn, GEMM_TPB, 0, stream>>>(
            (const bf16*)Ac.const_data_ptr(),
            (const bf16*)Bc.const_data_ptr(), C.data_ptr(), M, N, K, nbm,
            nbn, sm, nullptr);
  else if (use_nt)
    gemm_bt_kernel<false, false, true><<<nbm * nbn, GEMM_TPB, 0, stream>>>(
        (const bf16*)Ac.const_data_ptr(), (const bf16*)Bc.const_data_ptr(),
        C.data_ptr(), M, N, K, nbm, nbn, sm, nullptr);
  else if (gemm_adir_enabled())
    gemm_bt_kernel<false, false, false, false, true, true>
        <<<nbm * nbn, GEMM_TPB, 0, stream>>>(
            (const bf16*)Ac.const_data_ptr(),
            (const bf16*)Bc.const_data_ptr(), C.data_ptr(), M, N, K, nbm,
            nbn, sm, nullptr);
  else if (use_db)
    gemm_bt_kernel<false, false, false, false, true>
        <<<nbm * nbn, GEMM_TPB, 0, stream>>>(
            (const bf16*)Ac.const_data_ptr(),
            (const bf16*)Bc.const_data_ptr(), C.data_ptr(), M, N, K, nbm,
            nbn, sm, nullptr);
  else
    gemm_bt_kernel<false, false><<<nbm * nbn, GEMM_TPB, 0, stream>>>(
        (const bf16*)Ac.const_data_ptr(), (const bf16*)Bc.const_data_ptr(),
        C.data_ptr(), M, N, K, nbm, nbn, sm, nullptr);
  CHECK_CUDA_OK();
  if (biasp) C.add_(*bias);
  if (gadd) C.add_(ac);
  return C;
}

std::vector<at::Tensor> gemm_bt_stats(at::Tensor A, at::Tensor B) {
  TORCH_CHECK(A.is_cuda() && A.scalar_type() == at::kBFloat16 &&
              B.scalar_type() == at::kBFloat16);
  auto Ac = A.contiguous();
  auto Bc = B.contiguous();
  long M = Ac.size(0), K = Ac.size(1), N = Bc.size(0);
  TORCH_CHECK(Bc.size(1) == K && K % BK == 0);
  auto C = at::empty({M, N}, Ac.options());
  int nbm = (int)((M + BM - 1) / BM), nbn = (int)((N + BN - 1) / BN);
  auto stats = at::empty({nbm, 2 * N}, Ac.options().dtype(at::kFloat));
  StrideMap sm{0, 0, 0, 0, 1};
  auto stream = at::cuda::getCurrentCUDAStream();
  const bool use_db = gemm_db_enabled(K);
  if (N % 256 == 0 && K <= 256 && (long)nbm * (nbn / 2) >= 256) {
    int nbn2 = nbn / 2;
    if (use_db)
      gemm_bt_n2_kernel<true><<<nbm * nbn2, GEMM_TPB, 0, stream>>>(
          (const bf16*)Ac.const_data_ptr(),
          (const bf16*)Bc.const_data_ptr(), (bf16*)C.data_ptr(), M, N, K,
          nbm, nbn2, stats.data_ptr<float>(), nbm);
    else
      gemm_bt_n2_kernel<<<nbm * nbn2, GEMM_TPB, 0, stream>>>(
          (const bf16*)Ac.const_data_ptr(),
          (const bf16*)Bc.const_data_ptr(), (bf16*)C.data_ptr(), M, N, K,
          nbm, nbn2, stats.data_ptr<float>(), nbm);
  } else if (gemm_adir_enabled()) {
    gemm_bt_kernel<false, false, false, false, true, true>
        <<<nbm * nbn, GEMM_TPB, 0, stream>>>(
            (const bf16*)Ac.const_data_ptr(),
            (const bf16*)Bc.const_data_ptr(), C.data_ptr(), M, N, K, nbm,
            nbn, sm, stats.data_ptr<float>());
  } else if (use_db) {
    gemm_bt_kernel<false, false, false, false, true>
        <<<nbm * nbn, GEMM_TPB, 0, stream>>>(
            (const bf16*)Ac.const_data_ptr(),
            (const bf16*)Bc.const_data_ptr(), C.data_ptr(), M, N, K, nbm,
            nbn, sm, stats.data_ptr<float>());
  } else {
    gemm_bt_kernel<false, false><<<nbm * nbn, GEMM_TPB, 0, stream>>>(
        (const bf16*)Ac.const_data_ptr(), (const bf16*)Bc.const_data_ptr(),
        C.data_ptr(), M, N, K, nbm, nbn, sm, stats.data_ptr<float>());
  }
  CHECK_CUDA_OK();
  return {C, stats};
}

at::Tensor gemm_bt_strided(at::Tensor A, at::Tensor B, long Nn, long H,
                           long W, long stride) {
  TORCH_CHECK(A.is_cuda() && A.scalar_type() == at::kBFloat16 &&
              B.scalar_type() == at::kBFloat16);
  auto Ac = A.contiguous();
  auto Bc = B.contiguous();
  long K = Ac.size(1), N = Bc.size(0);
  TORCH_CHECK(Bc.size(1) == K && K % BK == 0);
  long Hout = (H + stride - 1) / stride, Wout = (W + stride - 1) / stride;
  long M = Nn * Hout * Wout;
  auto C = at::empty({M, N}, Ac.options());
  int nbm = (int)((M + BM - 1) / BM), nbn = (int)((N + BN - 1) / BN);
  StrideMap sm{(int)H, (int)W, (int)Hout, (int)Wout, (int)stride};
  auto stream = at::cuda::getCurrentCUDAStream();
  if (gemm_db_enabled(K))
    gemm_bt_kernel<false, true, false, false, true>
        <<<nbm * nbn, GEMM_TPB, 0, stream>>>(
            (const bf16*)Ac.const_data_ptr(),
            (const bf16*)Bc.const_data_ptr(), C.data_ptr(), M, N, K, nbm,
            nbn, sm, nullptr);
  else
    gemm_bt_kernel<false, true><<<nbm * nbn, GEMM_TPB, 0, stream>>>(
        (const bf16*)Ac.const_data_ptr(), (const bf16*)Bc.const_data_ptr(),
        C.data_ptr(), M, N, K, nbm, nbn, sm, nullptr);
  CHECK_CUDA_OK();
  return C;
}

at::Tensor gemm_tn(at::Tensor dY, at::Tensor X, long msplit) {
  TORCH_CHECK(dY.is_cuda() && dY.dim() == 2 && X.dim() == 2);
  TORCH_CHECK(dY.scalar_type() == at::kBFloat16 &&
              X.scalar_type() == at::kBFloat16);
  auto Yc = dY.contiguous();
  auto Xc = X.contiguous();
  long M = Yc.size(0), N = Yc.size(1), K = Xc.size(1);
  TORCH_CHECK(Xc.size(0) == M, "M mismatch");
  TORCH_CHECK(N % 8 == 0 && K % 8 == 0, "N,K must be multiples of 8");
  auto dW = at::zeros({N, K}, Yc.options().dtype(at::kFloat));
  int nbn = (int)((N + 127) / 128), nbk = (int)((K + 127) / 128);
  long tiles = (long)nbn * nbk;
  const bool det = std::getenv("AMDTRAIN_DETERMINISTIC") != nullptr;
  if (det)
    msplit = 1;
  else if (msplit <= 0)
    msplit = std::max<long>(1, std::min<long>((M + 31) / 32, 512 / tiles));
  auto stream = at::cuda::getCurrentCUDAStream();
  StrideMap sm{0, 0, 0, 0, 1};
  gemm_tn_kernel<false><<<(int)(tiles * msplit), GEMM_TPB, 0, stream>>>(
      (const bf16*)Yc.const_data_ptr(), (const bf16*)Xc.const_data_ptr(),
      dW.data_ptr<float>(), M, N, K, nbn, nbk, (int)msplit, sm);
  CHECK_CUDA_OK();
  return dW;
}

at::Tensor gemm_tn_strided(at::Tensor dY, at::Tensor X, long Nn, long H,
                           long W, long stride) {
  auto Yc = dY.contiguous();
  auto Xc = X.contiguous();
  long M = Yc.size(0), N = Yc.size(1), K = Xc.size(1);
  TORCH_CHECK(N % 8 == 0 && K % 8 == 0);
  long Hout = (H + stride - 1) / stride, Wout = (W + stride - 1) / stride;
  TORCH_CHECK(M == Nn * Hout * Wout, "M mismatch for strided wgrad");
  auto dW = at::zeros({N, K}, Yc.options().dtype(at::kFloat));
  int nbn = (int)((N + 127) / 128), nbk = (int)((K + 127) / 128);
  long tiles = (long)nbn * nbk;
  const bool det2 = std::getenv("AMDTRAIN_DETERMINISTIC") != nullptr;
  long msplit = det2 ? 1 : std::max<long>(
      1, std::min<long>((M + 31) / 32, 512 / tiles));
  StrideMap sm{(int)H, (int)W, (int)Hout, (int)Wout, (int)stride};
  auto stream = at::cuda::getCurrentCUDAStream();
  gemm_tn_kernel<true><<<(int)(tiles * msplit), GEMM_TPB, 0, stream>>>(
      (const bf16*)Yc.const_data_ptr(), (const bf16*)Xc.const_data_ptr(),
      dW.data_ptr<float>(), M, N, K, nbn, nbk, (int)msplit, sm);
  CHECK_CUDA_OK();
  return dW;
}

at::Tensor transpose_2d(at::Tensor x) {
  TORCH_CHECK(x.is_cuda() && x.dim() == 2 &&
              x.scalar_type() == at::kBFloat16);
  auto xc = x.contiguous();
  int R = (int)xc.size(0), C = (int)xc.size(1);
  auto out = at::empty({C, R}, xc.options());
  int gx = (C + 31) / 32, gy = (R + 31) / 32;
  auto stream = at::cuda::getCurrentCUDAStream();
  transpose_2d_kernel<<<gx * gy, AMD_TPB, 0, stream>>>(
      (const bf16*)xc.const_data_ptr(), (bf16*)out.data_ptr(), R, C);
  CHECK_CUDA_OK();
  return out;
}
```

Measured before the change: 10900 images/sec.

## Add vectorized wide bf16 epilogue with DPP quad transpose for conv and GEMM kernels

Adds a selectable epilogue mode to the conv3x3, 1x1 GEMM and generic conv kernels. The wide mode permutes the B-fragment column mapping and uses DPP lane swaps plus byte permutes to gather contiguous 8-element bf16 runs, so each lane writes 16-byte stores instead of scattered 2-byte stores. A middle mode keeps the old layout but drops per-element bounds checks on interior tiles. This targets the cost of uncoalesced output writes, at the price of extra cross-lane shuffles and more kernel template instantiations.

```diff
diff --git a/amdtrain/ops/conv.py b/amdtrain/ops/conv.py
--- a/amdtrain/ops/conv.py
+++ b/amdtrain/ops/conv.py
@@ -32,6 +32,16 @@
 
 def _nt64_enabled() -> bool:
     return os.environ.get("AMDTRAIN_CONV3X3_NT64", "1") == "1"
+
+
+def _epilogue_mode() -> int:
+    v = os.environ.get("AMDTRAIN_EPILOGUE")
+    if v is None or v == "":
+        return -1
+    mode = int(v)
+    if mode not in (0, 1, 2):
+        raise ValueError(f"AMDTRAIN_EPILOGUE must be 0, 1 or 2, got {v!r}")
+    return mode
 
 
 def _wgrad2_enabled() -> bool:
@@ -92,14 +102,16 @@
         stats = None
         ctx.cell = cell
         if stride > 1:
-            y2d = e.gemm_bt_strided(x2d, w2d, n, h, w, stride)
+            y2d = e.gemm_bt_strided(x2d, w2d, n, h, w, stride,
+                                    _epilogue_mode())
             ho = (h + stride - 1) // stride
             wo = (w + stride - 1) // stride
         elif _fuse_stats_enabled():
-            y2d, stats = e.gemm_bt_stats(x2d, w2d)
+            y2d, stats = e.gemm_bt_stats(x2d, w2d, _epilogue_mode())
             ho, wo = h, w
         else:
-            y2d = e.gemm_bt(x2d, w2d, False)
+            y2d = e.gemm_bt(x2d, w2d, False, None, None,
+                            _epilogue_mode())
             ho, wo = h, w
         ctx.save_for_backward(x2d, w2d)
         ctx.meta = (n, cin, h, w, stride, ho, wo, cout)
@@ -118,7 +130,8 @@
         gy = grad_y.contiguous(memory_format=torch.channels_last)
         gy2d = _rows(gy).to(torch.bfloat16)
         wT = e.transpose_2d(w2d)
-        dx2d = e.gemm_bt(gy2d, wT, False)
+        dx2d = e.gemm_bt(gy2d, wT, False, None, None,
+                         _epilogue_mode())
         if stride > 1:
             cell = ctx.cell
             if (stride == 2 and cell is not None and cell.armed
@@ -162,9 +175,11 @@
         nt64 = _nt64_enabled()
         if _fuse_stats_enabled():
             y2d, stats = e.conv3x3_fwd_stats(x2d, n, h, w, stride, w2d,
-                                             False, nt64)
-        else:
-            y2d = e.conv3x3_fwd(x2d, n, h, w, stride, w2d, nt64)
+                                             False, nt64,
+                                             _epilogue_mode())
+        else:
+            y2d = e.conv3x3_fwd(x2d, n, h, w, stride, w2d, nt64,
+                                _epilogue_mode())
             stats = torch.empty(0, device=x.device)
         ctx.save_for_backward(x2d, w2d)
         ctx.meta = (n, cin, h, w, stride, cout)
@@ -183,7 +198,8 @@
         gy = grad_y.contiguous(memory_format=torch.channels_last)
         gy2d = _rows(gy).to(torch.bfloat16)
         dx2d = e.conv3x3_dgrad(gy2d, n, h, w, stride, w2d, False,
-                               _s2parity_enabled(), _nt64_enabled())
+                               _s2parity_enabled(), _nt64_enabled(),
+                               _epilogue_mode())
         dx = dx2d.view(n, h, w, cin).permute(0, 3, 1, 2)
         dw2d = e.tn2_wgrad(gy2d, x2d, 9, n, h, w, stride, 2) \
             if _wgrad2_enabled() \
@@ -224,9 +240,11 @@
         banded = (cin == cout and cin % 128 == 0)
         if _fuse_stats_enabled():
             y2d, stats = e.conv3x3_fwd_stats(x2d, n, h, w, stride, w2d,
-                                             banded, _nt64_enabled())
-        else:
-            y2d = e.conv3x3_fwd(x2d, n, h, w, stride, w2d, _nt64_enabled())
+                                             banded, _nt64_enabled(),
+                                             _epilogue_mode())
+        else:
+            y2d = e.conv3x3_fwd(x2d, n, h, w, stride, w2d, _nt64_enabled(),
+                                _epilogue_mode())
             stats = torch.empty(0, device=x.device)
         ctx.save_for_backward(x2d, w2d)
         ctx.meta = (n, cin, h, w, stride, cout, groups, banded)
@@ -247,7 +265,8 @@
         gy = grad_y.contiguous(memory_format=torch.channels_last)
         gy2d = _rows(gy).to(torch.bfloat16)
         dx2d = e.conv3x3_dgrad(gy2d, n, h, w, stride, w2d, banded,
-                               _s2parity_enabled(), _nt64_enabled())
+                               _s2parity_enabled(), _nt64_enabled(),
+                               _epilogue_mode())
         dx = dx2d.view(n, h, w, cin).permute(0, 3, 1, 2)
         if banded and _wgrad2_enabled():
             dwb = e.tn2_wgrad_banded(gy2d, x2d, n, h, w, stride) \
@@ -319,7 +338,8 @@
             x8 = stem_s2d_input(x2d.view(n, h, w, cin)) \
                 .view(n * h * (w // 2), 8)
             w2 = stem_s2d_weight(weight).reshape(cout, 224)
-            geom = (n, h, w // 2, 7, 4, 2, 3, w2, 1, 2, ho, wo, True)
+            geom = (n, h, w // 2, 7, 4, 2, 3, w2, 1, 2, ho, wo, True,
+                    _epilogue_mode())
             if _fuse_stats_enabled():
                 y2d, stats = e.conv_generic_fwd_stats(x8, *geom)
             else:
@@ -343,7 +363,7 @@
         if kpad != k:
             w2 = torch.nn.functional.pad(w2, (0, kpad - k))
         y2d = e.conv_generic_fwd(x2d, n, h, w, kh, kw, stride, pad, w2,
-                                 0, -1, 0, 0, nt64)
+                                 0, -1, 0, 0, nt64, _epilogue_mode())
         ctx.save_for_backward(x2d, weight)
         ctx.meta = (n, cin, h, w, kh, kw, stride, pad, cout, k, cin_k)
         stats = torch.empty(0, device=x.device)
diff --git a/amdtrain/ops/csrc/common.h b/amdtrain/ops/csrc/common.h
--- a/amdtrain/ops/csrc/common.h
+++ b/amdtrain/ops/csrc/common.h
@@ -74,7 +74,113 @@
   return v;
 }
 
-template <int NTE = 128>
+static inline int epi_mode(long epi, int kernel_default) {
+  return epi < 0 ? kernel_default : (int)epi;
+}
+typedef float epi_f32x4 __attribute__((ext_vector_type(4)));
+typedef float epi_f32x2 __attribute__((ext_vector_type(2)));
+typedef __bf16 epi_bf16x2 __attribute__((ext_vector_type(2)));
+
+template <bool WIDE>
+__device__ __forceinline__ constexpr int epi_col(int j, int fr) {
+  return WIDE ? (j >> 1) * 32 + (fr >> 2) * 8 + (j & 1) * 4 + (fr & 3)
+              : j * 16 + fr;
+}
+
+__device__ __forceinline__ unsigned epi_pack_bf16(float lo, float hi) {
+  epi_f32x2 f = {lo, hi};
+  epi_bf16x2 b = __builtin_convertvector(f, epi_bf16x2);
+  unsigned u;
+  __builtin_memcpy(&u, &b, 4);
+  return u;
+}
+
+template <int NF>
+__device__ __forceinline__ void epi_quad_transpose(const epi_f32x4* a,
+                                                   uint4* run, int fr) {
+  const bool odd = fr & 1, low = !(fr & 2);
+  const unsigned sel = odd ? 0x03020706u : 0x05040100u;
+  unsigned d[NF][2];
+#pragma unroll
+  for (int j = 0; j < NF; ++j) {
+    const unsigned p01 = epi_pack_bf16(a[j][0], a[j][1]);
+    const unsigned p23 = epi_pack_bf16(a[j][2], a[j][3]);
+    const unsigned x01 = __builtin_amdgcn_update_dpp(0, (int)p01, 0xB1, 0xF,
+                                                     0xF, true);
+    const unsigned x23 = __builtin_amdgcn_update_dpp(0, (int)p23, 0xB1, 0xF,
+                                                     0xF, true);
+    const unsigned q01 = __builtin_amdgcn_perm(x01, p01, sel);
+    const unsigned q23 = __builtin_amdgcn_perm(x23, p23, sel);
+    const unsigned send = low ? q23 : q01;
+    const unsigned recv = __builtin_amdgcn_update_dpp(0, (int)send, 0x4E,
+                                                      0xF, 0xF, true);
+    d[j][0] = low ? q01 : recv;
+    d[j][1] = low ? recv : q23;
+  }
+#pragma unroll
+  for (int h = 0; h < NF / 2; ++h)
+    run[h] = make_uint4(d[2 * h][0], d[2 * h][1], d[2 * h + 1][0],
+                        d[2 * h + 1][1]);
+}
+
+template <int NF, int ACCLD, bool WIDE>
+__device__ __forceinline__ void epi_store_bf16(
+    __hip_bfloat16* __restrict__ C, long ld, long m0, long M, long n0,
+    long N, int wm, int wn, int fr, int fq, const epi_f32x4* acc, int epi) {
+  const bool inside = __builtin_amdgcn_readfirstlane(
+      (int)(m0 + wm + 64 <= M && n0 + wn + NF * 16 <= N));
+  char* const blk = (char*)(C + m0 * ld + n0);
+  const unsigned ld2 = (unsigned)ld * 2;
+  if constexpr (WIDE) {
+    const unsigned lrow = wm + fq * 4 + (fr & 3), lcol = wn + (fr >> 2) * 8;
+    const unsigned off = lrow * ld2 + lcol * 2;
+    auto rows = [&](auto pred) {
+#pragma unroll
+      for (int i = 0; i < 4; ++i) {
+        uint4 run[NF / 2];
+        epi_quad_transpose<NF>(acc + i * ACCLD, run, fr);
+        if (!pred.value || m0 + lrow + i * 16 < M) {
+#pragma unroll
+          for (int h = 0; h < NF / 2; ++h)
+            if (!pred.value || n0 + lcol + h * 32 + 8 <= N)
+              *(uint4*)(blk + (off + i * 16 * ld2 + h * 64)) = run[h];
+        }
+      }
+    };
+    if (inside)
+      rows(std::false_type{});
+    else
+      rows(std::true_type{});
+    return;
+  }
+  if (inside && epi >= 1) {
+    const unsigned off = (wm + fq * 4) * ld2 + (wn + fr) * 2;
+#pragma unroll
+    for (int i = 0; i < 4; ++i)
+#pragma unroll
+      for (int r = 0; r < 4; ++r) {
+        const unsigned roff = off + (i * 16 + r) * ld2;
+#pragma unroll
+        for (int j = 0; j < NF; ++j)
+          *(__hip_bfloat16*)(blk + (roff + j * 32)) =
+              __float2bfloat16(acc[i * ACCLD + j][r]);
+      }
+    return;
+  }
+#pragma unroll
+  for (int i = 0; i < 4; ++i)
+#pragma unroll
+    for (int j = 0; j < NF; ++j)
+#pragma unroll
+      for (int r = 0; r < 4; ++r) {
+        long row = m0 + wm + i * 16 + fq * 4 + r;
+        long col = n0 + wn + j * 16 + fr;
+        if (row < M && col < N)
+          C[row * ld + col] = __float2bfloat16(acc[i * ACCLD + j][r]);
+      }
+}
+
+template <int NTE = 128, bool WIDE = false>
 __device__ __forceinline__ void conv_epilogue_stats(
     float* __restrict__ stats, const float* acc_flat, long m0, long M,
     long n0, long N, int bm, int wm, int wn, int fr, int fq,
@@ -109,7 +215,7 @@
   if (fq == 0) {
 #pragma unroll
     for (int j = 0; j < NF; ++j) {
-      int col = wn + j * 16 + fr;
+      int col = wn + epi_col<WIDE>(j, fr);
       red[(wm ? 1 : 0) * (2 * NTE) + col * 2 + 0] = s1[j];
       red[(wm ? 1 : 0) * (2 * NTE) + col * 2 + 1] = s2[j];
     }
diff --git a/amdtrain/ops/csrc/conv3x3.hip b/amdtrain/ops/csrc/conv3x3.hip
--- a/amdtrain/ops/csrc/conv3x3.hip
+++ b/amdtrain/ops/csrc/conv3x3.hip
@@ -163,12 +163,12 @@
 }
 
 template <bool DGRAD, int BKT = BK, bool BAND = false, int NT = 128,
-          bool DB = false, bool PAR = false>
+          bool DB = false, bool PAR = false, bool WIDE = false>
 __global__ void __launch_bounds__(GEMM_TPB, 2)
 conv3x3_kernel(const bf16* __restrict__ A, const bf16* __restrict__ Bw,
                bf16* __restrict__ C, long M, int AC, int NC, ConvGeom g,
                int nbm, int nbn, const bf16* __restrict__ zero_page,
-               float* __restrict__ stats) {
+               float* __restrict__ stats, int epi) {
   static_assert(!PAR || (DGRAD && !BAND), "PAR is a dense-dgrad variant");
   constexpr int STG = (128 + NT) * BKT;
   __shared__ bf16 SMEM[(DB ? 2 : 1) * STG];
@@ -234,7 +234,7 @@
 #pragma unroll
       for (int j = 0; j < NFR; ++j)
         b[j] = *(const bf16x8*)
-            &bs[(wn + j * 16 + fr) * BKT + kk * 32 + fq * 8];
+            &bs[(wn + epi_col<WIDE>(j, fr)) * BKT + kk * 32 + fq * 8];
 #pragma unroll
       for (int i = 0; i < 4; ++i)
 #pragma unroll
@@ -261,6 +261,27 @@
     }
   }
 
+  if (PAR && WIDE) {
+    const unsigned W2 = g.W >> 1, H2 = g.H >> 1;
+    const long lcol = n0 + wn + (fr >> 2) * 8;
+#pragma unroll
+    for (int i = 0; i < 4; ++i) {
+      uint4 run[NFR / 2];
+      epi_quad_transpose<NFR>(&acc[i][0], run, fr);
+      const unsigned mr = (unsigned)m0 + wm + i * 16 + fq * 4 + (fr & 3);
+      if ((long)mr < Mr) {
+        const unsigned w2 = mr % W2, t2 = mr / W2;
+        const unsigned h2 = t2 % H2, n = t2 / H2;
+        const long row = ((long)n * g.H + 2 * h2 + par_h) * g.W + 2 * w2 +
+                         par_w;
+#pragma unroll
+        for (int h = 0; h < NFR / 2; ++h)
+          if (lcol + h * 32 + 8 <= NC)
+            *(uint4*)(C + row * NC + lcol + h * 32) = run[h];
+      }
+    }
+    return;
+  }
   if (PAR) {
     const unsigned W2 = g.W >> 1, H2 = g.H >> 1;
 #pragma unroll
@@ -291,20 +312,11 @@
     }
     return;
   }
-#pragma unroll
-  for (int i = 0; i < 4; ++i)
-#pragma unroll
-    for (int j = 0; j < NFR; ++j)
-#pragma unroll
-      for (int r = 0; r < 4; ++r) {
-        long row = m0 + wm + i * 16 + fq * 4 + r;
-        long col = n0 + wn + j * 16 + fr;
-        if (row < M && col < NC)
-          C[row * NC + col] = __float2bfloat16(acc[i][j][r]);
-      }
+  epi_store_bf16<NFR, NFR, WIDE>(C, NC, m0, M, n0, NC, wm, wn, fr, fq,
+                                 &acc[0][0], epi);
   if (stats != nullptr)
-    conv_epilogue_stats<NT>(stats, (const float*)acc, m0, M, n0, NC, bm,
-                            wm, wn, fr, fq, As);
+    conv_epilogue_stats<NT, WIDE>(stats, (const float*)acc, m0, M, n0, NC,
+                                  bm, wm, wn, fr, fq, As);
 }
 
 __device__ __forceinline__ int wg_swz(int cc, int m) {
@@ -435,12 +447,31 @@
   return zp;
 }
 
+template <bool DGRAD, int BKT, bool BAND, int NT, bool DB, bool PAR = false>
+static void launch_c3(bool wide, int grid, hipStream_t stream, const bf16* A,
+                      const bf16* Bw, bf16* C, long M, int AC, int NC,
+                      const ConvGeom& g, int nbm, int nbn, const bf16* zp,
+                      float* stats, int epi) {
+  if constexpr (DB && !BAND) {
+    if (wide) {
+      conv3x3_kernel<DGRAD, BKT, BAND, NT, DB, PAR, true>
+          <<<grid, GEMM_TPB, 0, stream>>>(A, Bw, C, M, AC, NC, g, nbm, nbn,
+                                          zp, stats, epi);
+      return;
+    }
+  }
+  conv3x3_kernel<DGRAD, BKT, BAND, NT, DB, PAR, false>
+      <<<grid, GEMM_TPB, 0, stream>>>(A, Bw, C, M, AC, NC, g, nbm, nbn, zp,
+                                      stats, epi);
+}
+
 std::vector<at::Tensor> conv3x3_fwd_stats_impl(at::Tensor x2d, long Nn,
                                                 long H, long W, long stride,
                                                 at::Tensor w2d,
                                                 bool want_stats,
                                                 bool banded = false,
-                                                bool nt64 = true) {
+                                                bool nt64 = true,
+                                                long epi = -1) {
   TORCH_CHECK(x2d.is_cuda() && x2d.scalar_type() == at::kBFloat16);
   long Cin = x2d.size(1), Cout = w2d.size(0);
   TORCH_CHECK(w2d.size(1) == 9 * Cin);
@@ -452,90 +483,78 @@
   int nbm = (int)((M + 127) / 128), nbn = (int)((Cout + 127) / 128);
   auto zp = zero_page_for(x2d);
   at::Tensor stats;
-  float* stats_ptr = nullptr;
+  float* sp = nullptr;
   if (want_stats) {
     stats = at::empty({nbm, 2 * Cout}, x2d.options().dtype(at::kFloat));
-    stats_ptr = stats.data_ptr<float>();
+    sp = stats.data_ptr<float>();
   }
   auto stream = at::cuda::getCurrentCUDAStream();
   static const bool bk64 = []() {
     const char* v = std::getenv("AMDTRAIN_CONV3X3_BK64");
     return !(v && v[0] == '0');
   }();
+  const bf16* xp = (const bf16*)x2d.const_data_ptr();
+  const bf16* wp = (const bf16*)w2d.const_data_ptr();
+  const bf16* zpp = (const bf16*)zp.const_data_ptr();
+  bf16* yp = (bf16*)y.data_ptr();
+  const int ci = (int)Cin, co = (int)Cout, ep = epi_mode(epi, 2);
+  const bool wide = ep >= 2 && Cout % 8 == 0;
+  const bool db = conv3x3_db_enabled();
   if (banded) {
     int nbn64 = (int)((Cout + 63) / 64);
-    if (conv3x3_db_enabled())
-      conv3x3_kernel<false, BK, true, 64, true>
-          <<<nbm * nbn64, GEMM_TPB, 0, stream>>>(
-              (const bf16*)x2d.const_data_ptr(),
-              (const bf16*)w2d.const_data_ptr(), (bf16*)y.data_ptr(), M,
-              (int)Cin, (int)Cout, g, nbm, nbn64,
-              (const bf16*)zp.const_data_ptr(), stats_ptr);
+    if (db)
+      launch_c3<false, BK, true, 64, true>(wide, nbm * nbn64, stream, xp, wp,
+                                           yp, M, ci, co, g, nbm, nbn64, zpp,
+                                           sp, ep);
     else
-      conv3x3_kernel<false, BK, true, 64>
-          <<<nbm * nbn64, GEMM_TPB, 0, stream>>>(
-              (const bf16*)x2d.const_data_ptr(),
-              (const bf16*)w2d.const_data_ptr(), (bf16*)y.data_ptr(), M,
-              (int)Cin, (int)Cout, g, nbm, nbn64,
-              (const bf16*)zp.const_data_ptr(), stats_ptr);
-  } else if (nt64 && Cout <= 64 && conv3x3_db_enabled()) {
-    conv3x3_kernel<false, BK, false, 64, true>
-        <<<nbm, GEMM_TPB, 0, stream>>>(
-            (const bf16*)x2d.const_data_ptr(),
-            (const bf16*)w2d.const_data_ptr(), (bf16*)y.data_ptr(), M,
-            (int)Cin, (int)Cout, g, nbm, 1,
-            (const bf16*)zp.const_data_ptr(), stats_ptr);
+      launch_c3<false, BK, true, 64, false>(wide, nbm * nbn64, stream, xp,
+                                            wp, yp, M, ci, co, g, nbm, nbn64,
+                                            zpp, sp, ep);
+  } else if (nt64 && Cout <= 64 && db) {
+    launch_c3<false, BK, false, 64, true>(wide, nbm, stream, xp, wp, yp, M,
+                                          ci, co, g, nbm, 1, zpp, sp, ep);
   } else if (bk64 && Cin % 64 == 0 && Cin >= 128 && M >= 200000) {
-    if (conv3x3_db_enabled())
-      conv3x3_kernel<false, 64, false, 128, true>
-          <<<nbm * nbn, GEMM_TPB, 0, stream>>>(
-              (const bf16*)x2d.const_data_ptr(),
-              (const bf16*)w2d.const_data_ptr(), (bf16*)y.data_ptr(), M,
-              (int)Cin, (int)Cout, g, nbm, nbn,
-              (const bf16*)zp.const_data_ptr(), stats_ptr);
+    if (db)
+      launch_c3<false, 64, false, 128, true>(wide, nbm * nbn, stream, xp, wp,
+                                             yp, M, ci, co, g, nbm, nbn, zpp,
+                                             sp, ep);
     else
-      conv3x3_kernel<false, 64><<<nbm * nbn, GEMM_TPB, 0, stream>>>(
-          (const bf16*)x2d.const_data_ptr(),
-          (const bf16*)w2d.const_data_ptr(), (bf16*)y.data_ptr(), M,
-          (int)Cin, (int)Cout, g, nbm, nbn,
-          (const bf16*)zp.const_data_ptr(), stats_ptr);
-  } else if (conv3x3_db_enabled())
-    conv3x3_kernel<false, BK, false, 128, true>
-        <<<nbm * nbn, GEMM_TPB, 0, stream>>>(
-            (const bf16*)x2d.const_data_ptr(),
-            (const bf16*)w2d.const_data_ptr(), (bf16*)y.data_ptr(), M,
-            (int)Cin, (int)Cout, g, nbm, nbn,
-            (const bf16*)zp.const_data_ptr(), stats_ptr);
+      launch_c3<false, 64, false, 128, false>(wide, nbm * nbn, stream, xp,
+                                              wp, yp, M, ci, co, g, nbm, nbn,
+                                              zpp, sp, ep);
+  } else if (db)
+    launch_c3<false, BK, false, 128, true>(wide, nbm * nbn, stream, xp, wp,
+                                           yp, M, ci, co, g, nbm, nbn, zpp,
+                                           sp, ep);
   else
-    conv3x3_kernel<false><<<nbm * nbn, GEMM_TPB, 0, stream>>>(
-        (const bf16*)x2d.const_data_ptr(), (const bf16*)w2d.const_data_ptr(),
-        (bf16*)y.data_ptr(), M, (int)Cin, (int)Cout, g, nbm, nbn,
-        (const bf16*)zp.const_data_ptr(), stats_ptr);
+    launch_c3<false, BK, false, 128, false>(wide, nbm * nbn, stream, xp, wp,
+                                            yp, M, ci, co, g, nbm, nbn, zpp,
+                                            sp, ep);
   CHECK_CUDA_OK();
   if (want_stats) return {y, stats};
   return {y};
 }
 
 at::Tensor conv3x3_fwd(at::Tensor x2d, long Nn, long H, long W, long stride,
-                       at::Tensor w2d, bool nt64) {
+                       at::Tensor w2d, bool nt64, long epi) {
   return conv3x3_fwd_stats_impl(x2d, Nn, H, W, stride, w2d, false, false,
-                                nt64)[0];
+                                nt64, epi)[0];
 }
 
 std::vector<at::Tensor> conv3x3_fwd_stats(at::Tensor x2d, long Nn, long H,
                                           long W, long stride,
                                           at::Tensor w2d, bool banded,
-                                          bool nt64) {
+                                          bool nt64, long epi) {
   TORCH_CHECK(!banded || (x2d.size(1) == w2d.size(0) &&
                           x2d.size(1) % 128 == 0),
               "banded conv3x3 needs Cin == Cout, both % 128");
   return conv3x3_fwd_stats_impl(x2d, Nn, H, W, stride, w2d, true, banded,
-                                nt64);
+                                nt64, epi);
 }
 
 at::Tensor conv3x3_dgrad(at::Tensor dy2d, long Nn, long H, long W,
                          long stride, at::Tensor w2d, bool banded,
-                         bool s2parity, bool nt64) {
+                         bool s2parity, bool nt64, long epi) {
   long Cout = dy2d.size(1), Cin = w2d.size(1) / 9;
   TORCH_CHECK(w2d.size(0) == Cout && w2d.size(1) == 9 * Cin);
   TORCH_CHECK(Cout % BK == 0);
@@ -551,23 +570,24 @@
   ConvGeom g{(int)H, (int)W, (int)Hout, (int)Wout, (int)stride};
   int nbm = (int)((M + 127) / 128), nbn = (int)((Cin + 127) / 128);
   auto zp = zero_page_for(dy2d);
+  const bf16* yp = (const bf16*)dy2d.const_data_ptr();
+  const bf16* wp = (const bf16*)wrot.const_data_ptr();
+  const bf16* zpp = (const bf16*)zp.const_data_ptr();
+  bf16* xp = (bf16*)dx.data_ptr();
+  const int ci = (int)Cin, co = (int)Cout, ep = epi_mode(epi, 2);
+  const bool wide = ep >= 2 && Cin % 8 == 0;
+  const bool db = conv3x3_db_enabled();
   if (banded) {
     TORCH_CHECK(Cin == Cout && Cin % 128 == 0);
     int nbn64 = (int)(Cin / 64);
-    if (conv3x3_db_enabled())
-      conv3x3_kernel<true, BK, true, 64, true>
-          <<<nbm * nbn64, GEMM_TPB, 0, stream>>>(
-              (const bf16*)dy2d.const_data_ptr(),
-              (const bf16*)wrot.const_data_ptr(), (bf16*)dx.data_ptr(), M,
-              (int)Cout, (int)Cin, g, nbm, nbn64,
-              (const bf16*)zp.const_data_ptr(), nullptr);
+    if (db)
+      launch_c3<true, BK, true, 64, true>(wide, nbm * nbn64, stream, yp, wp,
+                                          xp, M, co, ci, g, nbm, nbn64, zpp,
+                                          nullptr, ep);
     else
-      conv3x3_kernel<true, BK, true, 64>
-          <<<nbm * nbn64, GEMM_TPB, 0, stream>>>(
-              (const bf16*)dy2d.const_data_ptr(),
-              (const bf16*)wrot.const_data_ptr(), (bf16*)dx.data_ptr(), M,
-              (int)Cout, (int)Cin, g, nbm, nbn64,
-              (const bf16*)zp.const_data_ptr(), nullptr);
+      launch_c3<true, BK, true, 64, false>(wide, nbm * nbn64, stream, yp, wp,
+                                           xp, M, co, ci, g, nbm, nbn64, zpp,
+                                           nullptr, ep);
     CHECK_CUDA_OK();
     return dx;
   }
@@ -576,50 +596,35 @@
     return v && v[0] == '1';
   }();
   const bool par = s2parity && stride == 2 && H % 2 == 0 && W % 2 == 0 &&
-                   M < (1L << 31) && conv3x3_db_enabled();
-  const bool n64 = nt64 && Cin <= 64 && conv3x3_db_enabled();
+                   M < (1L << 31) && db;
+  const bool n64 = nt64 && Cin <= 64 && db;
   if (par) {
     const int nbmp = 4 * (int)((M / 4 + 127) / 128);
     if (n64)
-      conv3x3_kernel<true, BK, false, 64, true, true>
-          <<<nbmp, GEMM_TPB, 0, stream>>>(
-              (const bf16*)dy2d.const_data_ptr(),
-              (const bf16*)wrot.const_data_ptr(), (bf16*)dx.data_ptr(), M,
-              (int)Cout, (int)Cin, g, nbmp, 1,
-              (const bf16*)zp.const_data_ptr(), nullptr);
+      launch_c3<true, BK, false, 64, true, true>(wide, nbmp, stream, yp, wp,
+                                                 xp, M, co, ci, g, nbmp, 1,
+                                                 zpp, nullptr, ep);
     else
-      conv3x3_kernel<true, BK, false, 128, true, true>
-          <<<nbmp * nbn, GEMM_TPB, 0, stream>>>(
-              (const bf16*)dy2d.const_data_ptr(),
-              (const bf16*)wrot.const_data_ptr(), (bf16*)dx.data_ptr(), M,
-              (int)Cout, (int)Cin, g, nbmp, nbn,
-              (const bf16*)zp.const_data_ptr(), nullptr);
+      launch_c3<true, BK, false, 128, true, true>(wide, nbmp * nbn, stream,
+                                                  yp, wp, xp, M, co, ci, g,
+                                                  nbmp, nbn, zpp, nullptr,
+                                                  ep);
   } else if (n64)
-    conv3x3_kernel<true, BK, false, 64, true>
-        <<<nbm, GEMM_TPB, 0, stream>>>(
-            (const bf16*)dy2d.const_data_ptr(),
-            (const bf16*)wrot.const_data_ptr(), (bf16*)dx.data_ptr(), M,
-            (int)Cout, (int)Cin, g, nbm, 1,
-            (const bf16*)zp.const_data_ptr(), nullptr);
+    launch_c3<true, BK, false, 64, true>(wide, nbm, stream, yp, wp, xp, M,
+                                         co, ci, g, nbm, 1, zpp, nullptr,
+                                         ep);
   else if (bk64d && Cout % 64 == 0)
-    conv3x3_kernel<true, 64><<<nbm * nbn, GEMM_TPB, 0, stream>>>(
-        (const bf16*)dy2d.const_data_ptr(),
-        (const bf16*)wrot.const_data_ptr(), (bf16*)dx.data_ptr(), M,
-        (int)Cout, (int)Cin, g, nbm, nbn,
-        (const bf16*)zp.const_data_ptr(), nullptr);
-  else if (conv3x3_db_enabled())
-    conv3x3_kernel<true, BK, false, 128, true>
-        <<<nbm * nbn, GEMM_TPB, 0, stream>>>(
-            (const bf16*)dy2d.const_data_ptr(),
-            (const bf16*)wrot.const_data_ptr(), (bf16*)dx.data_ptr(), M,
-            (int)Cout, (int)Cin, g, nbm, nbn,
-            (const bf16*)zp.const_data_ptr(), nullptr);
+    launch_c3<true, 64, false, 128, false>(wide, nbm * nbn, stream, yp, wp,
+                                           xp, M, co, ci, g, nbm, nbn, zpp,
+                                           nullptr, ep);
+  else if (db)
+    launch_c3<true, BK, false, 128, true>(wide, nbm * nbn, stream, yp, wp,
+                                          xp, M, co, ci, g, nbm, nbn, zpp,
+                                          nullptr, ep);
   else
-    conv3x3_kernel<true><<<nbm * nbn, GEMM_TPB, 0, stream>>>(
-        (const bf16*)dy2d.const_data_ptr(),
-        (const bf16*)wrot.const_data_ptr(), (bf16*)dx.data_ptr(), M,
-        (int)Cout, (int)Cin, g, nbm, nbn,
-        (const bf16*)zp.const_data_ptr(), nullptr);
+    launch_c3<true, BK, false, 128, false>(wide, nbm * nbn, stream, yp, wp,
+                                           xp, M, co, ci, g, nbm, nbn, zpp,
+                                           nullptr, ep);
   CHECK_CUDA_OK();
   return dx;
 }
diff --git a/amdtrain/ops/csrc/conv_stem.hip b/amdtrain/ops/csrc/conv_stem.hip
--- a/amdtrain/ops/csrc/conv_stem.hip
+++ b/amdtrain/ops/csrc/conv_stem.hip
@@ -168,13 +168,13 @@
 }
 
 template <bool DGRAD = false, bool C8 = false, bool DB = false, int NT = 128,
-          bool ROW4 = false>
+          bool ROW4 = false, bool WIDE = false>
 __global__ void __launch_bounds__(GEMM_TPB, 2)
 conv_generic_fwd_kernel(const bf16* __restrict__ x,
                         const bf16* __restrict__ W2, bf16* __restrict__ Y,
                         long M, int Cout, StemGeom g, int nbm, int nbn,
                         const bf16* __restrict__ zp,
-                        float* __restrict__ stats) {
+                        float* __restrict__ stats, int epi) {
   static_assert(!ROW4 || (C8 && !DGRAD), "ROW4 is a C8 forward staging");
   constexpr int STG = (128 + NT) * BK;
   constexpr int NFR = NT / 32;
@@ -231,7 +231,8 @@
       a[i] = *(const bf16x8*)&as[(wm + i * 16 + fr) * BK + fq * 8];
 #pragma unroll
     for (int j = 0; j < NFR; ++j)
-      b[j] = *(const bf16x8*)&bs[(wn + j * 16 + fr) * BK + fq * 8];
+      b[j] = *(const bf16x8*)
+          &bs[(wn + epi_col<WIDE>(j, fr)) * BK + fq * 8];
 #pragma unroll
     for (int i = 0; i < 4; ++i)
 #pragma unroll
@@ -256,20 +257,11 @@
       compute(SMEM);
     }
   }
-#pragma unroll
-  for (int i = 0; i < 4; ++i)
-#pragma unroll
-    for (int j = 0; j < NFR; ++j)
-#pragma unroll
-      for (int r = 0; r < 4; ++r) {
-        long row = m0 + wm + i * 16 + fq * 4 + r;
-        long col = n0 + wn + j * 16 + fr;
-        if (row < M && col < Cout)
-          Y[row * Cout + col] = __float2bfloat16(acc[i][j][r]);
-      }
+  epi_store_bf16<NFR, NFR, WIDE>(Y, Cout, m0, M, n0, Cout, wm, wn, fr, fq,
+                                 &acc[0][0], epi);
   if (stats != nullptr)
-    conv_epilogue_stats<NT>(stats, (const float*)acc, m0, M, n0, Cout, bm,
-                            wm, wn, fr, fq, SMEM);
+    conv_epilogue_stats<NT, WIDE>(stats, (const float*)acc, m0, M, n0, Cout,
+                                  bm, wm, wn, fr, fq, SMEM);
 }
 
 __device__ __forceinline__ int st_swz(int c, int m) {
@@ -403,10 +395,18 @@
 static void stem_launch(int grid, hipStream_t stream, const bf16* x,
                         const bf16* w2, bf16* y, long M, int Cout,
                         const StemGeom& g, int nbm, int nbn, const bf16* zp,
-                        float* stats) {
-  conv_generic_fwd_kernel<DGRAD, C8, DBUF, NT, ROW4>
+                        float* stats, bool wide, int epi) {
+  if constexpr (C8 && DBUF && !DGRAD) {
+    if (wide) {
+      conv_generic_fwd_kernel<DGRAD, C8, DBUF, NT, ROW4, true>
+          <<<grid, GEMM_TPB, 0, stream>>>(x, w2, y, M, Cout, g, nbm, nbn, zp,
+                                          stats, epi);
+      return;
+    }
+  }
+  conv_generic_fwd_kernel<DGRAD, C8, DBUF, NT, ROW4, false>
       <<<grid, GEMM_TPB, 0, stream>>>(x, w2, y, M, Cout, g, nbm, nbn, zp,
-                                      stats);
+                                      stats, epi);
 }
 
 static at::Tensor stem_zero_page(const at::Tensor& like) {
@@ -430,7 +430,7 @@
 static std::vector<at::Tensor> conv_generic_fwd_impl(
     at::Tensor x2d, long Nn, long H, long W, long KH, long KW, long stride,
     long pad, at::Tensor w2, long stride_w, long pad_w, long Hout, long Wout,
-    bool want_stats, bool tile64) {
+    bool want_stats, bool tile64, long epi) {
   TORCH_CHECK(x2d.is_cuda() && x2d.scalar_type() == at::kBFloat16);
   TORCH_CHECK(x2d.is_contiguous() && w2.is_contiguous());
   long Cin = x2d.size(1), Cout = w2.size(0);
@@ -458,31 +458,32 @@
   const bf16* wp = (const bf16*)w2.const_data_ptr();
   const bf16* zpp = (const bf16*)zp.const_data_ptr();
   bf16* yp = (bf16*)y.data_ptr();
-  const int grid = nbm * nbn, co = (int)Cout;
+  const int grid = nbm * nbn, co = (int)Cout, ep = epi_mode(epi, 2);
+  const bool wide = ep >= 2 && Cout % 8 == 0;
   if (c8 && row4 && t64 && db)
     stem_launch<false, true, true, 64, true>(grid, stream, xp, wp, yp, M, co,
-                                             g, nbm, nbn, zpp, sp);
+                                             g, nbm, nbn, zpp, sp, wide, ep);
   else if (c8 && row4 && t64)
     stem_launch<false, true, false, 64, true>(grid, stream, xp, wp, yp, M, co,
-                                              g, nbm, nbn, zpp, sp);
+                                              g, nbm, nbn, zpp, sp, wide, ep);
   else if (c8 && t64 && db)
     stem_launch<false, true, true, 64>(grid, stream, xp, wp, yp, M, co, g,
-                                       nbm, nbn, zpp, sp);
+                                       nbm, nbn, zpp, sp, wide, ep);
   else if (c8 && t64)
     stem_launch<false, true, false, 64>(grid, stream, xp, wp, yp, M, co, g,
-                                        nbm, nbn, zpp, sp);
+                                        nbm, nbn, zpp, sp, wide, ep);
   else if (c8 && db)
     stem_launch<false, true, true>(grid, stream, xp, wp, yp, M, co, g, nbm,
-                                   nbn, zpp, sp);
+                                   nbn, zpp, sp, wide, ep);
   else if (c8)
     stem_launch<false, true, false>(grid, stream, xp, wp, yp, M, co, g, nbm,
-                                    nbn, zpp, sp);
+                                    nbn, zpp, sp, wide, ep);
   else if (db)
     stem_launch<false, false, true>(grid, stream, xp, wp, yp, M, co, g, nbm,
-                                    nbn, zpp, sp);
+                                    nbn, zpp, sp, wide, ep);
   else
     stem_launch<false, false, false>(grid, stream, xp, wp, yp, M, co, g, nbm,
-                                     nbn, zpp, sp);
+                                     nbn, zpp, sp, wide, ep);
   CHECK_CUDA_OK();
   if (want_stats) return {y, stats};
   return {y};
@@ -491,17 +492,19 @@
 at::Tensor conv_generic_fwd(at::Tensor x2d, long Nn, long H, long W,
                             long KH, long KW, long stride, long pad,
                             at::Tensor w2, long stride_w, long pad_w,
-                            long Hout, long Wout, bool tile64) {
+                            long Hout, long Wout, bool tile64, long epi) {
   return conv_generic_fwd_impl(x2d, Nn, H, W, KH, KW, stride, pad, w2,
-                               stride_w, pad_w, Hout, Wout, false, tile64)[0];
+                               stride_w, pad_w, Hout, Wout, false, tile64,
+                               epi)[0];
 }
 
 std::vector<at::Tensor> conv_generic_fwd_stats(
     at::Tensor x2d, long Nn, long H, long W, long KH, long KW, long stride,
     long pad, at::Tensor w2, long stride_w, long pad_w, long Hout, long Wout,
-    bool tile64) {
+    bool tile64, long epi) {
   return conv_generic_fwd_impl(x2d, Nn, H, W, KH, KW, stride, pad, w2,
-                               stride_w, pad_w, Hout, Wout, true, tile64);
+                               stride_w, pad_w, Hout, Wout, true, tile64,
+                               epi);
 }
 
 at::Tensor conv_generic_dgrad(at::Tensor dy2d, at::Tensor w2p, long Nn,
@@ -523,12 +526,13 @@
             (const bf16*)dy2d.const_data_ptr(),
             (const bf16*)w2p.const_data_ptr(), (bf16*)dx.data_ptr(), M,
             (int)Cin, g, nbm, nbn, (const bf16*)zp.const_data_ptr(),
-            nullptr);
+            nullptr, 0);
   else
     conv_generic_fwd_kernel<true><<<nbm * nbn, GEMM_TPB, 0, stream>>>(
         (const bf16*)dy2d.const_data_ptr(),
         (const bf16*)w2p.const_data_ptr(), (bf16*)dx.data_ptr(), M,
-        (int)Cin, g, nbm, nbn, (const bf16*)zp.const_data_ptr(), nullptr);
+        (int)Cin, g, nbm, nbn, (const bf16*)zp.const_data_ptr(), nullptr,
+        0);
   CHECK_CUDA_OK();
   return dx;
 }
diff --git a/amdtrain/ops/csrc/ext.cpp b/amdtrain/ops/csrc/ext.cpp
--- a/amdtrain/ops/csrc/ext.cpp
+++ b/amdtrain/ops/csrc/ext.cpp
@@ -68,21 +68,21 @@
 
 at::Tensor gemm_bt(at::Tensor A, at::Tensor B, bool f32_out,
                    std::optional<at::Tensor> addend,
-                   std::optional<at::Tensor> bias);
+                   std::optional<at::Tensor> bias, long epi);
 at::Tensor gemm_tn(at::Tensor dY, at::Tensor X, long msplit);
 at::Tensor gemm_bt_strided(at::Tensor A, at::Tensor B, long Nn, long H,
-                           long W, long stride);
+                           long W, long stride, long epi);
 at::Tensor gemm_tn_strided(at::Tensor dY, at::Tensor X, long Nn, long H,
                            long W, long stride);
 at::Tensor transpose_2d(at::Tensor x);
 
 at::Tensor conv3x3_fwd(at::Tensor x2d, long Nn, long H, long W, long stride,
-                       at::Tensor w2d, bool nt64);
+                       at::Tensor w2d, bool nt64, long epi);
 std::vector<at::Tensor> conv3x3_fwd_stats(at::Tensor x2d, long Nn, long H,
                                           long W, long stride,
                                           at::Tensor w2d, bool banded,
-                                          bool nt64);
-std::vector<at::Tensor> gemm_bt_stats(at::Tensor A, at::Tensor B);
+                                          bool nt64, long epi);
+std::vector<at::Tensor> gemm_bt_stats(at::Tensor A, at::Tensor B, long epi);
 
 at::Tensor gemm_bt_8p(at::Tensor A, at::Tensor B);
 at::Tensor gemm_bt_8p3(at::Tensor A, at::Tensor B);
@@ -90,7 +90,7 @@
                       at::Tensor w2d, bool dgrad);
 at::Tensor conv3x3_dgrad(at::Tensor dy2d, long Nn, long H, long W,
                          long stride, at::Tensor w2d, bool banded,
-                         bool s2parity, bool nt64);
+                         bool s2parity, bool nt64, long epi);
 at::Tensor conv3x3_wgrad(at::Tensor dy2d, at::Tensor x2d, long Nn, long H,
                          long W, long stride);
 
@@ -105,11 +105,11 @@
 at::Tensor conv_generic_fwd(at::Tensor x2d, long Nn, long H, long W, long KH,
                             long KW, long stride, long pad, at::Tensor w2,
                             long stride_w, long pad_w, long Hout, long Wout,
-                            bool tile64);
+                            bool tile64, long epi);
 std::vector<at::Tensor> conv_generic_fwd_stats(
     at::Tensor x2d, long Nn, long H, long W, long KH, long KW, long stride,
     long pad, at::Tensor w2, long stride_w, long pad_w, long Hout, long Wout,
-    bool tile64);
+    bool tile64, long epi);
 at::Tensor conv_generic_wgrad(at::Tensor dy2d, at::Tensor x2d, long Nn,
                               long H, long W, long KH, long KW, long stride,
                               long pad);
@@ -164,26 +164,30 @@
         py::arg("scale"), py::arg("shift"));
   m.def("gemm_bt", &gemm_bt, py::arg("A"), py::arg("B"),
         py::arg("f32_out") = false, py::arg("addend") = std::nullopt,
-        py::arg("bias") = std::nullopt);
+        py::arg("bias") = std::nullopt, py::arg("epi") = -1);
   m.def("gemm_tn", &gemm_tn, py::arg("dY"), py::arg("X"),
         py::arg("msplit") = 0);
-  m.def("gemm_bt_strided", &gemm_bt_strided);
+  m.def("gemm_bt_strided", &gemm_bt_strided, py::arg("A"), py::arg("B"),
+        py::arg("Nn"), py::arg("H"), py::arg("W"), py::arg("stride"),
+        py::arg("epi") = -1);
   m.def("gemm_tn_strided", &gemm_tn_strided);
   m.def("transpose_2d", &transpose_2d);
   m.def("conv3x3_fwd", &conv3x3_fwd, py::arg("x2d"), py::arg("Nn"),
         py::arg("H"), py::arg("W"), py::arg("stride"), py::arg("w2d"),
-        py::arg("nt64") = true);
+        py::arg("nt64") = true, py::arg("epi") = -1);
   m.def("conv3x3_fwd_stats", &conv3x3_fwd_stats, py::arg("x2d"),
         py::arg("Nn"), py::arg("H"), py::arg("W"), py::arg("stride"),
-        py::arg("w2d"), py::arg("banded") = false, py::arg("nt64") = true);
-  m.def("gemm_bt_stats", &gemm_bt_stats);
+        py::arg("w2d"), py::arg("banded") = false, py::arg("nt64") = true,
+        py::arg("epi") = -1);
+  m.def("gemm_bt_stats", &gemm_bt_stats, py::arg("A"), py::arg("B"),
+        py::arg("epi") = -1);
   m.def("gemm_bt_8p", &gemm_bt_8p);
   m.def("gemm_bt_8p3", &gemm_bt_8p3);
   m.def("conv3x3_8p", &conv3x3_8p);
   m.def("conv3x3_dgrad", &conv3x3_dgrad, py::arg("dy2d"), py::arg("Nn"),
         py::arg("H"), py::arg("W"), py::arg("stride"), py::arg("w2d"),
         py::arg("banded") = false, py::arg("s2parity") = true,
-        py::arg("nt64") = true);
+        py::arg("nt64") = true, py::arg("epi") = -1);
   m.def("conv3x3_wgrad", &conv3x3_wgrad);
   m.def("tn2_wgrad", &tn2_wgrad, py::arg("dY"), py::arg("X"),
         py::arg("taps") = 1, py::arg("Nn") = 0, py::arg("H") = 0,
@@ -197,12 +201,14 @@
         py::arg("Nn"), py::arg("H"), py::arg("W"), py::arg("KH"),
         py::arg("KW"), py::arg("stride"), py::arg("pad"), py::arg("w2"),
         py::arg("stride_w") = 0, py::arg("pad_w") = -1, py::arg("Hout") = 0,
-        py::arg("Wout") = 0, py::arg("tile64") = false);
+        py::arg("Wout") = 0, py::arg("tile64") = false,
+        py::arg("epi") = -1);
   m.def("conv_generic_fwd_stats", &conv_generic_fwd_stats, py::arg("x2d"),
         py::arg("Nn"), py::arg("H"), py::arg("W"), py::arg("KH"),
         py::arg("KW"), py::arg("stride"), py::arg("pad"), py::arg("w2"),
         py::arg("stride_w") = 0, py::arg("pad_w") = -1, py::arg("Hout") = 0,
-        py::arg("Wout") = 0, py::arg("tile64") = false);
+        py::arg("Wout") = 0, py::arg("tile64") = false,
+        py::arg("epi") = -1);
   m.def("conv_generic_wgrad", &conv_generic_wgrad);
   m.def("conv_generic_dgrad", &conv_generic_dgrad);
   m.def("max_pool_3x3_s2_fwd", &max_pool_3x3_s2_fwd, py::arg("x"),
diff --git a/amdtrain/ops/csrc/gemm.hip b/amdtrain/ops/csrc/gemm.hip
--- a/amdtrain/ops/csrc/gemm.hip
+++ b/amdtrain/ops/csrc/gemm.hip
@@ -86,7 +86,7 @@
 }
 
 
-template <int NFRAG>
+template <int NFRAG, bool WIDE = false>
 __device__ __forceinline__ void epilogue_stats(
     float* __restrict__ stats, const float* acc_flat, long m0, long M,
     long n0, long N, int bm, int wm, int wn, int fr, int fq, int nbm,
@@ -120,7 +120,7 @@
   if (fq == 0) {
 #pragma unroll
     for (int j = 0; j < NFRAG; ++j) {
-      int col = wn + j * 16 + fr;
+      int col = wn + epi_col<WIDE>(j, fr);
       red[(wm ? 1 : 0) * 256 + col * 2 + 0] = s1[j];
       red[(wm ? 1 : 0) * 256 + col * 2 + 1] = s2[j];
     }
@@ -137,11 +137,12 @@
 }
 
 template <bool F32OUT, bool STRIDED, bool NT = false, bool LDSE = false,
-          bool DB = false, bool ADIR = false>
+          bool DB = false, bool ADIR = false, bool WIDE = false>
 __global__ void __launch_bounds__(GEMM_TPB, 2)
 gemm_bt_kernel(const bf16* __restrict__ A, const bf16* __restrict__ B,
                void* __restrict__ C, long M, long N, long K, int nbm,
-               int nbn, StrideMap sm, float* __restrict__ stats) {
+               int nbn, StrideMap sm, float* __restrict__ stats, int epi) {
+  static_assert(!WIDE || !(F32OUT || NT || LDSE), "WIDE is a bf16 epilogue");
   __shared__ bf16 SMEM[(DB ? 2 : 1) *
                        ((ADIR ? 0 : BM) + BN) * BK];
   bf16* const As = SMEM;
@@ -205,7 +206,8 @@
                   : *(const bf16x8*)&as[(wm + i * 16 + fr) * BK + fq * 8];
 #pragma unroll
     for (int j = 0; j < 4; ++j)
-      b[j] = *(const bf16x8*)&bs[(wn + j * 16 + fr) * BK + fq * 8];
+      b[j] = *(const bf16x8*)
+          &bs[(wn + epi_col<WIDE>(j, fr)) * BK + fq * 8];
 #pragma unroll
     for (int i = 0; i < 4; ++i)
 #pragma unroll
@@ -254,7 +256,7 @@
               ((const uint4*)SMEM)[u2];
       }
     }
-  } else {
+  } else if (F32OUT || NT) {
 #pragma unroll
     for (int i = 0; i < 4; ++i) {
 #pragma unroll
@@ -266,29 +268,31 @@
           if (row < M && col < N) {
             if (F32OUT) {
               ((float*)C)[row * N + col] = acc[i][j][r];
-            } else if (NT) {
+            } else {
               bf16 v = __float2bfloat16(acc[i][j][r]);
               short b;
               __builtin_memcpy(&b, &v, 2);
               __builtin_nontemporal_store(b, (short*)C + row * N + col);
-            } else {
-              ((bf16*)C)[row * N + col] = __float2bfloat16(acc[i][j][r]);
             }
           }
         }
       }
     }
+  } else {
+    epi_store_bf16<4, 4, WIDE>((bf16*)C, N, m0, M, n0, N, wm, wn, fr, fq,
+                               &acc[0][0], epi);
   }
   if (stats != nullptr)
-    epilogue_stats<4>(stats, (const float*)acc, m0, M, n0, N, bm, wm, wn,
-                      fr, fq, nbm, As);
-}
-
-template <bool DB = false>
+    epilogue_stats<4, WIDE>(stats, (const float*)acc, m0, M, n0, N, bm, wm,
+                            wn, fr, fq, nbm, As);
+}
+
+template <bool DB = false, bool WIDE = false>
 __global__ void __launch_bounds__(GEMM_TPB, 2)
 gemm_bt_n2_kernel(const bf16* __restrict__ A, const bf16* __restrict__ B,
                   bf16* __restrict__ C, long M, long N, long K, int nbm,
-                  int nbn2, float* __restrict__ stats, int nbm_stats) {
+                  int nbn2, float* __restrict__ stats, int nbm_stats,
+                  int epi) {
   __shared__ bf16 SMEM[(DB ? 2 : 1) * (BM + 256) * BK];
   bf16* const As = SMEM;
   bf16* const Bs = SMEM + BM * BK;
@@ -326,8 +330,8 @@
       a[i] = *(const bf16x8*)&as[(wm + i * 16 + fr) * BK + fq * 8];
 #pragma unroll
     for (int j = 0; j < 8; ++j) {
-      const int jn = (j < 4) ? wn + j * 16 : 128 + wn + (j - 4) * 16;
-      b[j] = *(const bf16x8*)&bs[(jn + fr) * BK + fq * 8];
+      const int jn = (j < 4 ? 0 : 128) + wn + epi_col<WIDE>(j & 3, fr);
+      b[j] = *(const bf16x8*)&bs[jn * BK + fq * 8];
     }
 #pragma unroll
     for (int i = 0; i < 4; ++i)
@@ -354,18 +358,10 @@
     }
   }
 
-#pragma unroll
-  for (int i = 0; i < 4; ++i)
-#pragma unroll
-    for (int j = 0; j < 8; ++j)
-#pragma unroll
-      for (int r = 0; r < 4; ++r) {
-        long row = m0 + wm + i * 16 + fq * 4 + r;
-        long col = n0 + ((j < 4) ? wn + j * 16 : 128 + wn + (j - 4) * 16)
-                   + fr;
-        if (row < M && col < N)
-          C[row * N + col] = __float2bfloat16(acc[i][j][r]);
-      }
+  epi_store_bf16<4, 8, WIDE>(C, N, m0, M, n0, N, wm, wn, fr, fq,
+                             &acc[0][0], epi);
+  epi_store_bf16<4, 8, WIDE>(C, N, m0, M, n0, N, wm, 128 + wn, fr, fq,
+                             &acc[0][4], epi);
   if (stats != nullptr) {
     float accl[4][4][4], acch[4][4][4];
 #pragma unroll
@@ -377,11 +373,11 @@
           accl[i][j][r] = acc[i][j][r];
           acch[i][j][r] = acc[i][j + 4][r];
         }
-    epilogue_stats<4>(stats, (const float*)accl, m0, M, n0, N, bm, wm, wn,
-                      fr, fq, nbm_stats, As);
+    epilogue_stats<4, WIDE>(stats, (const float*)accl, m0, M, n0, N, bm, wm,
+                            wn, fr, fq, nbm_stats, As);
     __syncthreads();
-    epilogue_stats<4>(stats, (const float*)acch, m0, M, n0 + 128, N, bm,
-                      wm, wn, fr, fq, nbm_stats, As);
+    epilogue_stats<4, WIDE>(stats, (const float*)acch, m0, M, n0 + 128, N,
+                            bm, wm, wn, fr, fq, nbm_stats, As);
   }
 }
 
@@ -613,9 +609,44 @@
 
 }
 
+constexpr int EPI_DEFAULT_BT = 2, EPI_DEFAULT_N2 = 1;
+static inline bool epi_wide(int epi, long N) {
+  return epi >= 2 && N % 8 == 0;
+}
+
+template <bool STRIDED>
+static void launch_bt(bool db, bool wide, int grid, hipStream_t stream,
+                      const bf16* A, const bf16* B, void* C, long M, long N,
+                      long K, int nbm, int nbn, const StrideMap& sm,
+                      float* stats, int epi) {
+#define AMDTRAIN_BT(DBV, WV)                                                \
+  gemm_bt_kernel<false, STRIDED, false, false, DBV, false, WV>              \
+      <<<grid, GEMM_TPB, 0, stream>>>(A, B, C, M, N, K, nbm, nbn, sm,       \
+                                      stats, epi)
+  if (db && wide) AMDTRAIN_BT(true, true);
+  else if (db) AMDTRAIN_BT(true, false);
+  else if (wide) AMDTRAIN_BT(false, true);
+  else AMDTRAIN_BT(false, false);
+#undef AMDTRAIN_BT
+}
+
+static void launch_bt_n2(bool db, bool wide, int grid, hipStream_t stream,
+                         const bf16* A, const bf16* B, bf16* C, long M,
+                         long N, long K, int nbm, int nbn2, float* stats,
+                         int epi) {
+#define AMDTRAIN_N2(DBV, WV)                                                \
+  gemm_bt_n2_kernel<DBV, WV><<<grid, GEMM_TPB, 0, stream>>>(                \
+      A, B, C, M, N, K, nbm, nbn2, stats, nbm, epi)
+  if (db && wide) AMDTRAIN_N2(true, true);
+  else if (db) AMDTRAIN_N2(true, false);
+  else if (wide) AMDTRAIN_N2(false, true);
+  else AMDTRAIN_N2(false, false);
+#undef AMDTRAIN_N2
+}
+
 at::Tensor gemm_bt(at::Tensor A, at::Tensor B, bool f32_out,
                    std::optional<at::Tensor> addend,
-                   std::optional<at::Tensor> bias) {
+                   std::optional<at::Tensor> bias, long epi) {
   TORCH_CHECK(A.is_cuda() && A.dim() == 2 && B.dim() == 2);
   TORCH_CHECK(A.scalar_type() == at::kBFloat16 &&
               B.scalar_type() == at::kBFloat16,
@@ -646,19 +677,15 @@
   }
   const long tiles = (long)nbm * nbn;
   const long ksteps = K / BK;
+  const bf16* Ap = (const bf16*)Ac.const_data_ptr();
+  const bf16* Bp = (const bf16*)Bc.const_data_ptr();
   if (!f32_out && !addend && !bias && N % 256 == 0 && K <= 256 &&
       (long)nbm * (nbn / 2) >= 256) {
     int nbn2 = nbn / 2;
-    if (gemm_db_enabled(K))
-      gemm_bt_n2_kernel<true><<<nbm * nbn2, GEMM_TPB, 0, stream>>>(
-          (const bf16*)Ac.const_data_ptr(),
-          (const bf16*)Bc.const_data_ptr(), (bf16*)C.data_ptr(), M, N, K,
-          nbm, nbn2, nullptr, nbm);
-    else
-      gemm_bt_n2_kernel<<<nbm * nbn2, GEMM_TPB, 0, stream>>>(
-          (const bf16*)Ac.const_data_ptr(),
-          (const bf16*)Bc.const_data_ptr(), (bf16*)C.data_ptr(), M, N, K,
-          nbm, nbn2, nullptr, nbm);
+    const int ep2 = epi_mode(epi, EPI_DEFAULT_N2);
+    launch_bt_n2(gemm_db_enabled(K), epi_wide(ep2, N), nbm * nbn2, stream,
+                 Ap, Bp, (bf16*)C.data_ptr(), M, N, K, nbm, nbn2, nullptr,
+                 ep2);
     CHECK_CUDA_OK();
     return C;
   }
@@ -667,8 +694,7 @@
     auto parts = at::empty({ksplit, M * N},
                            Ac.options().dtype(at::kFloat));
     gemm_bt_ks_kernel<<<(int)(tiles * ksplit), GEMM_TPB, 0, stream>>>(
-        (const bf16*)Ac.const_data_ptr(), (const bf16*)Bc.const_data_ptr(),
-        parts.data_ptr<float>(), M, N, K, nbm, nbn, ksplit);
+        Ap, Bp, parts.data_ptr<float>(), M, N, K, nbm, nbn, ksplit);
     CHECK_CUDA_OK();
     gemm_ks_collapse_kernel<<<amd_grid(M * N), AMD_TPB, 0, stream>>>(
         (const float*)parts.const_data_ptr(), (bf16*)C.data_ptr(), ksplit,
@@ -685,43 +711,32 @@
     const char* v = std::getenv("AMDTRAIN_GEMM_LDSE");
     return v && v[0] == '1';
   }();
+  const int grid = nbm * nbn, ep = epi_mode(epi, EPI_DEFAULT_BT);
+  const bool wide = epi_wide(ep, N);
   if (f32_out)
-    gemm_bt_kernel<true, false><<<nbm * nbn, GEMM_TPB, 0, stream>>>(
-        (const bf16*)Ac.const_data_ptr(), (const bf16*)Bc.const_data_ptr(),
-        C.data_ptr(), M, N, K, nbm, nbn, sm, nullptr);
+    gemm_bt_kernel<true, false><<<grid, GEMM_TPB, 0, stream>>>(
+        Ap, Bp, C.data_ptr(), M, N, K, nbm, nbn, sm, nullptr, ep);
   else if (use_ldse && N % 8 == 0)
     gemm_bt_kernel<false, false, false, true>
-        <<<nbm * nbn, GEMM_TPB, 0, stream>>>(
-            (const bf16*)Ac.const_data_ptr(),
-            (const bf16*)Bc.const_data_ptr(), C.data_ptr(), M, N, K, nbm,
-            nbn, sm, nullptr);
+        <<<grid, GEMM_TPB, 0, stream>>>(Ap, Bp, C.data_ptr(), M, N, K, nbm,
+                                        nbn, sm, nullptr, ep);
   else if (use_nt)
-    gemm_bt_kernel<false, false, true><<<nbm * nbn, GEMM_TPB, 0, stream>>>(
-        (const bf16*)Ac.const_data_ptr(), (const bf16*)Bc.const_data_ptr(),
-        C.data_ptr(), M, N, K, nbm, nbn, sm, nullptr);
+    gemm_bt_kernel<false, false, true><<<grid, GEMM_TPB, 0, stream>>>(
+        Ap, Bp, C.data_ptr(), M, N, K, nbm, nbn, sm, nullptr, ep);
   else if (gemm_adir_enabled())
     gemm_bt_kernel<false, false, false, false, true, true>
-        <<<nbm * nbn, GEMM_TPB, 0, stream>>>(
-            (const bf16*)Ac.const_data_ptr(),
-            (const bf16*)Bc.const_data_ptr(), C.data_ptr(), M, N, K, nbm,
-            nbn, sm, nullptr);
-  else if (use_db)
-    gemm_bt_kernel<false, false, false, false, true>
-        <<<nbm * nbn, GEMM_TPB, 0, stream>>>(
-            (const bf16*)Ac.const_data_ptr(),
-            (const bf16*)Bc.const_data_ptr(), C.data_ptr(), M, N, K, nbm,
-            nbn, sm, nullptr);
+        <<<grid, GEMM_TPB, 0, stream>>>(Ap, Bp, C.data_ptr(), M, N, K, nbm,
+                                        nbn, sm, nullptr, ep);
   else
-    gemm_bt_kernel<false, false><<<nbm * nbn, GEMM_TPB, 0, stream>>>(
-        (const bf16*)Ac.const_data_ptr(), (const bf16*)Bc.const_data_ptr(),
-        C.data_ptr(), M, N, K, nbm, nbn, sm, nullptr);
+    launch_bt<false>(use_db, wide, grid, stream, Ap, Bp, C.data_ptr(), M, N,
+                     K, nbm, nbn, sm, nullptr, ep);
   CHECK_CUDA_OK();
   if (biasp) C.add_(*bias);
   if (gadd) C.add_(ac);
   return C;
 }
 
-std::vector<at::Tensor> gemm_bt_stats(at::Tensor A, at::Tensor B) {
+std::vector<at::Tensor> gemm_bt_stats(at::Tensor A, at::Tensor B, long epi) {
   TORCH_CHECK(A.is_cuda() && A.scalar_type() == at::kBFloat16 &&
               B.scalar_type() == at::kBFloat16);
   auto Ac = A.contiguous();
@@ -734,41 +749,31 @@
   StrideMap sm{0, 0, 0, 0, 1};
   auto stream = at::cuda::getCurrentCUDAStream();
   const bool use_db = gemm_db_enabled(K);
+  const int ep = epi_mode(epi, EPI_DEFAULT_BT);
+  const bf16* Ap = (const bf16*)Ac.const_data_ptr();
+  const bf16* Bp = (const bf16*)Bc.const_data_ptr();
   if (N % 256 == 0 && K <= 256 && (long)nbm * (nbn / 2) >= 256) {
     int nbn2 = nbn / 2;
-    if (use_db)
-      gemm_bt_n2_kernel<true><<<nbm * nbn2, GEMM_TPB, 0, stream>>>(
-          (const bf16*)Ac.const_data_ptr(),
-          (const bf16*)Bc.const_data_ptr(), (bf16*)C.data_ptr(), M, N, K,
-          nbm, nbn2, stats.data_ptr<float>(), nbm);
-    else
-      gemm_bt_n2_kernel<<<nbm * nbn2, GEMM_TPB, 0, stream>>>(
-          (const bf16*)Ac.const_data_ptr(),
-          (const bf16*)Bc.const_data_ptr(), (bf16*)C.data_ptr(), M, N, K,
-          nbm, nbn2, stats.data_ptr<float>(), nbm);
+    const int ep2 = epi_mode(epi, EPI_DEFAULT_N2);
+    launch_bt_n2(use_db, epi_wide(ep2, N), nbm * nbn2, stream, Ap, Bp,
+                 (bf16*)C.data_ptr(), M, N, K, nbm, nbn2,
+                 stats.data_ptr<float>(), ep2);
   } else if (gemm_adir_enabled()) {
     gemm_bt_kernel<false, false, false, false, true, true>
         <<<nbm * nbn, GEMM_TPB, 0, stream>>>(
-            (const bf16*)Ac.const_data_ptr(),
-            (const bf16*)Bc.const_data_ptr(), C.data_ptr(), M, N, K, nbm,
-            nbn, sm, stats.data_ptr<float>());
-  } else if (use_db) {
-    gemm_bt_kernel<false, false, false, false, true>
-        <<<nbm * nbn, GEMM_TPB, 0, stream>>>(
-            (const bf16*)Ac.const_data_ptr(),
-            (const bf16*)Bc.const_data_ptr(), C.data_ptr(), M, N, K, nbm,
-            nbn, sm, stats.data_ptr<float>());
+            Ap, Bp, C.data_ptr(), M, N, K, nbm, nbn, sm,
+            stats.data_ptr<float>(), ep);
   } else {
-    gemm_bt_kernel<false, false><<<nbm * nbn, GEMM_TPB, 0, stream>>>(
-        (const bf16*)Ac.const_data_ptr(), (const bf16*)Bc.const_data_ptr(),
-        C.data_ptr(), M, N, K, nbm, nbn, sm, stats.data_ptr<float>());
+    launch_bt<false>(use_db, epi_wide(ep, N), nbm * nbn, stream, Ap, Bp,
+                     C.data_ptr(), M, N, K, nbm, nbn, sm,
+                     stats.data_ptr<float>(), ep);
   }
   CHECK_CUDA_OK();
   return {C, stats};
 }
 
 at::Tensor gemm_bt_strided(at::Tensor A, at::Tensor B, long Nn, long H,
-                           long W, long stride) {
+                           long W, long stride, long epi) {
   TORCH_CHECK(A.is_cuda() && A.scalar_type() == at::kBFloat16 &&
               B.scalar_type() == at::kBFloat16);
   auto Ac = A.contiguous();
@@ -781,16 +786,11 @@
   int nbm = (int)((M + BM - 1) / BM), nbn = (int)((N + BN - 1) / BN);
   StrideMap sm{(int)H, (int)W, (int)Hout, (int)Wout, (int)stride};
   auto stream = at::cuda::getCurrentCUDAStream();
-  if (gemm_db_enabled(K))
-    gemm_bt_kernel<false, true, false, false, true>
-        <<<nbm * nbn, GEMM_TPB, 0, stream>>>(
-            (const bf16*)Ac.const_data_ptr(),
-            (const bf16*)Bc.const_data_ptr(), C.data_ptr(), M, N, K, nbm,
-            nbn, sm, nullptr);
-  else
-    gemm_bt_kernel<false, true><<<nbm * nbn, GEMM_TPB, 0, stream>>>(
-        (const bf16*)Ac.const_data_ptr(), (const bf16*)Bc.const_data_ptr(),
-        C.data_ptr(), M, N, K, nbm, nbn, sm, nullptr);
+  const int ep = epi_mode(epi, EPI_DEFAULT_BT);
+  launch_bt<true>(gemm_db_enabled(K), epi_wide(ep, N), nbm * nbn, stream,
+                  (const bf16*)Ac.const_data_ptr(),
+                  (const bf16*)Bc.const_data_ptr(), C.data_ptr(), M, N, K,
+                  nbm, nbn, sm, nullptr, ep);
   CHECK_CUDA_OK();
   return C;
 }
```

Result: faster. 11130 images/sec (median of 6 runs) (+2.1%).
